# clovaai/assembled-cnn

Hardware: AMD Instinct MI355X
Metric: images/sec Assemble-ResNet-50 224^2 bf16 train (higher is better)
Workload: dtype bf16; 1 GPU; Assemble-ResNet-50 (BigLittle + SK + anti_alias sconv k=3 + resnet_d) bf16 train; per_gpu_batch=256, global_batch=256, image=224x224x3, num_classes=1001, parallelism=dp1

## Files before the change

### assembled_cnn_amd/csrc/sk_fused.hip

```cpp
#include "common.h"
#include "blur3s2.h"

namespace {

__device__ __forceinline__ u32x4 ldv(const bf16_t* p, size_t off) { return *reinterpret_cast<const u32x4*>(p + off); }
__device__ __forceinline__ float rbf(float x) { return bf2f(f2bf(x)); }

struct Coef8 {
  float sc[8], sh[8];
};
__device__ __forceinline__ void load_coef(const float* __restrict__ scale, const float* __restrict__ shift, int ch0, Coef8& k) {
  const f32x4 s0 = *reinterpret_cast<const f32x4*>(scale + ch0), s1 = *reinterpret_cast<const f32x4*>(scale + ch0 + 4);
  const f32x4 h0 = *reinterpret_cast<const f32x4*>(shift + ch0), h1 = *reinterpret_cast<const f32x4*>(shift + ch0 + 4);
#pragma unroll
  for (int e = 0; e < 4; ++e) {
    k.sc[e] = s0[e]; k.sc[e + 4] = s1[e];
    k.sh[e] = h0[e]; k.sh[e + 4] = h1[e];
  }
}
template <class K>
__device__ __forceinline__ void bnrelu8(const u32x4& vy, const K& k, float* f) {
  float y[8];
  unpack8(vy, y);
#pragma unroll
  for (int e = 0; e < 8; ++e) f[e] = rbf(fmaxf(y[e] * k.sc[e] + k.sh[e], 0.f));
}

__device__ __forceinline__ void gate8(const float* __restrict__ att, int n, int F, int c0, float* a0) {
#pragma unroll
  for (int e = 0; e < 8; ++e) {
    const float l0 = att[(size_t)n * 2 * F + c0 + e];
    const float l1 = att[(size_t)n * 2 * F + F + c0 + e];
    a0[e] = 1.0f / (1.0f + __expf(l1 - l0));
  }
}

template <int NT>
__device__ __forceinline__ void lane_sum8(float (*red)[9], const float* v, float* out, int vcb, int vcl, int nrl, bool leader) {
  if ((vcb & (vcb - 1)) == 0 && vcb <= 64) {
    float w[8];
#pragma unroll
    for (int e = 0; e < 8; ++e) w[e] = v[e];
    for (int off = vcb; off < 64; off <<= 1) {
#pragma unroll
      for (int e = 0; e < 8; ++e) w[e] += __shfl_xor(w[e], off, 64);
    }
    const int wave = threadIdx.x >> 6, lane = threadIdx.x & 63;
    __syncthreads();
    if (lane < vcb) {
#pragma unroll
      for (int e = 0; e < 8; ++e) red[wave * vcb + lane][e] = w[e];
    }
    __syncthreads();
    if (leader) {
#pragma unroll
      for (int e = 0; e < 8; ++e) {
        float t = 0.f;
#pragma unroll
        for (int r = 0; r < NT / 64; ++r) t += red[r * vcb + vcl][e];
        out[e] = t;
      }
    }
    return;
  }
  __syncthreads();
#pragma unroll
  for (int e = 0; e < 8; ++e) red[threadIdx.x][e] = v[e];
  __syncthreads();
  if (leader) {
#pragma unroll
    for (int e = 0; e < 8; ++e) {
      float t = 0.f;
      for (int r = 0; r < nrl; ++r) t += red[r * vcb + vcl][e];
      out[e] = t;
    }
  }
}

struct CoefLds {
  const float* sc;
  const float* sh;
};
template <class K>
__device__ __forceinline__ void bnrelu8m(const u32x4& vy, const K& k, float* f, float* m, float* my) {
  float y[8];
  unpack8(vy, y);
#pragma unroll
  for (int e = 0; e < 8; ++e) {
    const float t = y[e] * k.sc[e] + k.sh[e];
    f[e] = rbf(fmaxf(t, 0.f));
    m[e] = t > 0.f ? 1.f : 0.f;
    my[e] = t > 0.f ? y[e] : 0.f;
  }
}

template <int NT, bool ST>
__global__ __launch_bounds__(NT, NT == 256 ? 4 : 1) void sk_gap_bn_kernel(const bf16_t* __restrict__ y, const float* __restrict__ scale,
                                                       const float* __restrict__ shift, bf16_t* __restrict__ s, int HW,
                                                       int F, int vcb, const float* __restrict__ mean,
                                                       const float* __restrict__ invstd, float* __restrict__ stats) {
  __shared__ float red[NT][9];
  const int vcols = F >> 3;
  const int vcl = threadIdx.x % vcb, rl = threadIdx.x / vcb, nrl = NT / vcb;
  const int vc = blockIdx.x * vcb + vcl;
  const int n = blockIdx.y;
  float acc[8], c0[8], x0[8], c1[8], x1[8];
#pragma unroll
  for (int e = 0; e < 8; ++e) acc[e] = c0[e] = x0[e] = c1[e] = x1[e] = 0.f;
  if (vc < vcols && rl < nrl) {
    Coef8 k0, k1;
    load_coef(scale, shift, vc * 8, k0);
    load_coef(scale, shift, F + vc * 8, k1);
    auto consume = [&](const u32x4& v, const u32x4& w) {
      if (ST) {
        float f[8], m[8], my[8];
        bnrelu8m(v, k0, f, m, my);
#pragma unroll
        for (int e = 0; e < 8; ++e) { acc[e] += f[e]; c0[e] += m[e]; x0[e] += my[e]; }
        bnrelu8m(w, k1, f, m, my);
#pragma unroll
        for (int e = 0; e < 8; ++e) { acc[e] += f[e]; c1[e] += m[e]; x1[e] += my[e]; }
      } else {
        float f0[8], f1[8];
        bnrelu8(v, k0, f0);
        bnrelu8(w, k1, f1);
#pragma unroll
        for (int e = 0; e < 8; ++e) acc[e] += f0[e] + f1[e];
      }
    };
    constexpr int U = ST ? 2 : 4;
    const bf16_t* base = y + (size_t)n * HW * 2 * F + vc * 8;
    int r = rl;
    for (; r + (U - 1) * nrl < HW; r += U * nrl) {
      u32x4 v[U], w[U];
#pragma unroll
      for (int u = 0; u < U; ++u) {
        const size_t off = (size_t)(r + u * nrl) * 2 * F;
        v[u] = ldv(base, off);
        w[u] = ldv(base, off + F);
      }
#pragma unroll
      for (int u = 0; u < U; ++u) consume(v[u], w[u]);
    }
    for (; r < HW; r += nrl) {
      const size_t off = (size_t)r * 2 * F;
      consume(ldv(base, off), ldv(base, off + F));
    }
  }
  const bool leader = rl == 0 && vc < vcols;
  float o[8];
  lane_sum8<NT>(red, acc, o, vcb, vcl, nrl, leader);
  if (leader) {
    const float inv = 1.0f / (float)HW;
#pragma unroll
    for (int e = 0; e < 8; ++e) o[e] *= inv;
    *reinterpret_cast<u32x4*>(s + (size_t)n * F + vc * 8) = pack8(o);
  }
  if (ST) {
    float* st = stats + (size_t)n * 4 * F;
    const float* src[4] = {c0, c1, x0, x1};
#pragma unroll
    for (int q = 0; q < 4; ++q) {
      lane_sum8<NT>(red, src[q], o, vcb, vcl, nrl, leader);
      if (leader) {
        float* dst = st + (q >> 1) * 2 * F + (q & 1) * F + vc * 8;
        *reinterpret_cast<f32x4*>(dst) = f32x4{o[0], o[1], o[2], o[3]};
        *reinterpret_cast<f32x4*>(dst + 4) = f32x4{o[4], o[5], o[6], o[7]};
      }
    }
  }
}

struct PoolGeom {
  int W, Hh, Wh;
  FastDiv fd_w;
  float a0, a1, a2;
};

__device__ __forceinline__ u32x4 dv_from_pooled(const bf16_t* __restrict__ gimg, const PoolGeom& pg, int F, int r) {
  const int h = (int)fd_div((unsigned)r, pg.fd_w), w = r - h * pg.W;
  const int i = h >> 1, j = w >> 1;
  const bool u = h & 1, v = w & 1;
  const bool hv = i + 1 < pg.Hh, wv = j + 1 < pg.Wh;
  u32x4 g[2][2];
#pragma unroll
  for (int a = 0; a < 2; ++a)
#pragma unroll
    for (int b = 0; b < 2; ++b) {
      const bool ok = (a == 0 || (u && hv)) && (b == 0 || (v && wv));
      g[a][b] = ldv(gimg, ((size_t)(i + (ok ? a : 0)) * pg.Wh + j + (ok ? b : 0)) * F);
    }
  float acc[8];
  blur3s2_bwd_pixel([&](int a, int b, float* t) { unpack8(g[a][b], t); }, u, v, hv, wv, i == 0, j == 0, pg.a0, pg.a1, pg.a2,
                    acc);
  return pack8(acc);
}

__global__ __launch_bounds__(256) void sk_select_blur_fwd_kernel(const bf16_t* __restrict__ y, const float* __restrict__ scale,
                                                                 const float* __restrict__ shift,
                                                                 const float* __restrict__ att, bf16_t* __restrict__ out,
                                                                 int H, int W, int F, int fvb, int rpb, int bh,
                                                                 FastDiv fd_wo, float b0, float b1, float b2) {
  extern __shared__ u32x4 vband[];
  const int fv = F >> 3;
  const int vcl = threadIdx.x % fvb, rr = threadIdx.x / fvb;
  const int vc = blockIdx.z * fvb + vcl;
  const int n = blockIdx.y;
  const bool live = rr < rpb && vc < fv;
  const int Ho = H >> 1, Wo = W >> 1;
  const int ho0 = blockIdx.x * bh;
  const int nbh = min(bh, Ho - ho0);
  if (live) {
    Coef8 k0, k1;
    load_coef(scale, shift, vc * 8, k0);
    load_coef(scale, shift, F + vc * 8, k1);
    float a0[8];
    gate8(att, n, F, vc * 8, a0);
    const bf16_t* yn = y + (size_t)n * H * W * 2 * F + vc * 8;
    const int npix = (2 * nbh + 1) * W;
    const int first = (2 * ho0 - 1) * W;
    constexpr int U = 2;
    for (int p = rr; p < npix; p += U * rpb) {
      u32x4 y0[U], y1[U];
#pragma unroll
      for (int q = 0; q < U; ++q) {
        const int pq = p + q * rpb;
        int gp = first + (pq < npix ? pq : p);
        if (gp < 0) gp += 2 * W;
        y0[q] = ldv(yn, (size_t)gp * 2 * F);
        y1[q] = ldv(yn, (size_t)gp * 2 * F + F);
      }
#pragma unroll
      for (int q = 0; q < U; ++q) {
        const int pq = p + q * rpb;
        if (pq >= npix) break;
        float f0[8], f1[8], o[8];
        bnrelu8(y0[q], k0, f0);
        bnrelu8(y1[q], k1, f1);
#pragma unroll
        for (int e = 0; e < 8; ++e) o[e] = a0[e] * f0[e] + (1.0f - a0[e]) * f1[e];
        vband[pq * fvb + vcl] = pack8(o);
      }
    }
  }
  __syncthreads();
  if (live) {
    const float bw[3] = {b0, b1, b2};
    const int nout = nbh * Wo;
    for (int q = rr; q < nout; q += rpb) {
      const int oh = (int)fd_div((unsigned)q, fd_wo), ow = q - oh * Wo;
      float acc[8];
#pragma unroll
      for (int e = 0; e < 8; ++e) acc[e] = 0.f;
#pragma unroll
      for (int r = 0; r < 3; ++r) {
        const int lr = 2 * oh + r;
#pragma unroll
        for (int t = 0; t < 3; ++t) {
          int iw = 2 * ow + t - 1;
          if (iw < 0) iw = 1;
          float f[8];
          unpack8(vband[(lr * W + iw) * fvb + vcl], f);
          const float wgt = bw[r] * bw[t];
#pragma unroll
          for (int e = 0; e < 8; ++e) acc[e] += f[e] * wgt;
        }
      }
      *reinterpret_cast<u32x4*>(out + (((size_t)n * Ho + ho0 + oh) * Wo + ow) * F + vc * 8) = pack8(acc);
    }
  }
}

__global__ __launch_bounds__(256) void sk_select_bn_fwd_kernel(const bf16_t* __restrict__ y, const float* __restrict__ scale,
                                                               const float* __restrict__ shift,
                                                               const float* __restrict__ att, bf16_t* __restrict__ v,
                                                               int HW, int F, int rpb, int rows_per_chunk) {
  const int fv = F >> 3;
  const int vc = threadIdx.x % fv, rr = threadIdx.x / fv;
  if (rr >= rpb) return;
  const int n = blockIdx.y;
  Coef8 k0, k1;
  load_coef(scale, shift, vc * 8, k0);
  load_coef(scale, shift, F + vc * 8, k1);
  float a0[8];
  gate8(att, n, F, vc * 8, a0);
  const int r_begin = blockIdx.x * rows_per_chunk;
  const int r_end = min(HW, r_begin + rows_per_chunk);
  constexpr int U = 2;
  for (int r = r_begin + rr; r < r_end; r += U * rpb) {
    u32x4 y0[U], y1[U];
#pragma unroll
    for (int q = 0; q < U; ++q) {
      const int rq = r + q * rpb;
      const size_t m = (size_t)n * HW + (rq < r_end ? rq : r);
      y0[q] = ldv(y, m * 2 * F + vc * 8);
      y1[q] = ldv(y, m * 2 * F + F + vc * 8);
    }
#pragma unroll
    for (int q = 0; q < U; ++q) {
      const int rq = r + q * rpb;
      if (rq >= r_end) break;
      float f0[8], f1[8], o[8];
      bnrelu8(y0[q], k0, f0);
      bnrelu8(y1[q], k1, f1);
#pragma unroll
      for (int e = 0; e < 8; ++e) o[e] = a0[e] * f0[e] + (1.0f - a0[e]) * f1[e];
      *reinterpret_cast<u32x4*>(v + ((size_t)n * HW + rq) * F + vc * 8) = pack8(o);
    }
  }
}

template <int NT, bool ST, bool PG>
__global__ __launch_bounds__(NT, NT == 256 ? 4 : 1) void sk_bn_bwd_att_kernel(const bf16_t* __restrict__ y, const float* __restrict__ scale,
                                                           const float* __restrict__ shift, const bf16_t* __restrict__ dv,
                                                           const float* __restrict__ att, bf16_t* __restrict__ datt,
                                                           int HW, int F, int vcb, const float* __restrict__ mean,
                                                           const float* __restrict__ invstd, float* __restrict__ stats,
                                                           PoolGeom pg) {
  __shared__ float red[NT][9];
  __shared__ float cfl[PG ? 4 * 256 : 1];
  const int vcols = F >> 3;
  const int vcl = threadIdx.x % vcb, rl = threadIdx.x / vcb, nrl = NT / vcb;
  const int vc = blockIdx.x * vcb + vcl;
  const int n = blockIdx.y;
  float acc[8], g0[8], x0[8], g1[8], x1[8];
#pragma unroll
  for (int e = 0; e < 8; ++e) acc[e] = g0[e] = x0[e] = g1[e] = x1[e] = 0.f;
  if (PG) {
    if (rl == 0 && vc < vcols) {
#pragma unroll
      for (int e = 0; e < 8; ++e) {
        cfl[vcl * 8 + e] = scale[vc * 8 + e];
        cfl[256 + vcl * 8 + e] = shift[vc * 8 + e];
        cfl[512 + vcl * 8 + e] = scale[F + vc * 8 + e];
        cfl[768 + vcl * 8 + e] = shift[F + vc * 8 + e];
      }
    }
    __syncthreads();
  }
  if (vc < vcols && rl < nrl) {
    Coef8 r0, r1;
    if (!PG) {
      load_coef(scale, shift, vc * 8, r0);
      load_coef(scale, shift, F + vc * 8, r1);
    }
    const CoefLds l0 = {cfl + vcl * 8, cfl + 256 + vcl * 8}, l1 = {cfl + 512 + vcl * 8, cfl + 768 + vcl * 8};
    auto add_pixel = [&](const auto& k0, const auto& k1, const u32x4& v0, const u32x4& v1, const u32x4& vg) {
      float g[8];
      unpack8(vg, g);
      if (ST) {
        float f[8], m[8], my[8];
        bnrelu8m(v0, k0, f, m, my);
#pragma unroll
        for (int e = 0; e < 8; ++e) { acc[e] += f[e] * g[e]; g0[e] += m[e] * g[e]; x0[e] += my[e] * g[e]; }
        bnrelu8m(v1, k1, f, m, my);
#pragma unroll
        for (int e = 0; e < 8; ++e) { acc[e] -= f[e] * g[e]; g1[e] += m[e] * g[e]; x1[e] += my[e] * g[e]; }
      } else {
        float f0[8], f1[8];
        bnrelu8(v0, k0, f0);
        bnrelu8(v1, k1, f1);
#pragma unroll
        for (int e = 0; e < 8; ++e) acc[e] += (f0[e] - f1[e]) * g[e];
      }
    };
    auto consume = [&](const u32x4& v0, const u32x4& v1, const u32x4& vg) {
      if (PG) {
        __asm__ volatile("" ::: "memory");
        add_pixel(l0, l1, v0, v1, vg);
      } else {
        add_pixel(r0, r1, v0, v1, vg);
      }
    };
    const bf16_t* gimg = PG ? dv + (size_t)n * pg.Hh * pg.Wh * F + vc * 8 : nullptr;
    auto load_dv = [&](int rq) { return PG ? dv_from_pooled(gimg, pg, F, rq) : ldv(dv, ((size_t)n * HW + rq) * F + vc * 8); };
    constexpr int U = ST ? 1 : 2;
    int r = rl;
    for (; r + (U - 1) * nrl < HW; r += U * nrl) {
      u32x4 v0[U], v1[U], vg[U];
#pragma unroll
      for (int u = 0; u < U; ++u) {
        const size_t m = (size_t)n * HW + r + u * nrl;
        v0[u] = ldv(y, m * 2 * F + vc * 8);
        v1[u] = ldv(y, m * 2 * F + F + vc * 8);
        vg[u] = load_dv(r + u * nrl);
      }
#pragma unroll
      for (int u = 0; u < U; ++u) consume(v0[u], v1[u], vg[u]);
    }
    for (; r < HW; r += nrl) {
      const size_t m = (size_t)n * HW + r;
      consume(ldv(y, m * 2 * F + vc * 8), ldv(y, m * 2 * F + F + vc * 8), load_dv(r));
    }
  }
  const bool leader = rl == 0 && vc < vcols;
  float o[8];
  lane_sum8<NT>(red, acc, o, vcb, vcl, nrl, leader);
  if (leader) {
    float a0[8], d0[8], d1[8];
    gate8(att, n, F, vc * 8, a0);
#pragma unroll
    for (int e = 0; e < 8; ++e) {
      d0[e] = a0[e] * (1.0f - a0[e]) * o[e];
      d1[e] = -d0[e];
    }
    *reinterpret_cast<u32x4*>(datt + (size_t)n * 2 * F + vc * 8) = pack8(d0);
    *reinterpret_cast<u32x4*>(datt + (size_t)n * 2 * F + F + vc * 8) = pack8(d1);
  }
  if (ST) {
    float* st = stats + (size_t)n * 4 * F;
    const float* src[4] = {g0, g1, x0, x1};
#pragma unroll
    for (int q = 0; q < 4; ++q) {
      lane_sum8<NT>(red, src[q], o, vcb, vcl, nrl, leader);
      if (leader) {
        float* dst = st + (q >> 1) * 2 * F + (q & 1) * F + vc * 8;
        *reinterpret_cast<f32x4*>(dst) = f32x4{o[0], o[1], o[2], o[3]};
        *reinterpret_cast<f32x4*>(dst + 4) = f32x4{o[4], o[5], o[6], o[7]};
      }
    }
  }
}

struct SkBnGeom {
  int HW, F, vcols, rpb, rows_per_chunk, chunks;
};

__device__ __forceinline__ void sk_thread_setup(const SkBnGeom& g, int n, int vc, const float* __restrict__ att,
                                                const bf16_t* __restrict__ ds, float* ab, float* u) {
  const int fv = g.F >> 3;
  const int b = vc >= fv ? 1 : 0;
  const int c0 = (vc - b * fv) * 8;
  float a0[8], q[8];
  gate8(att, n, g.F, c0, a0);
  unpack8(ldv(ds, (size_t)n * g.F + c0), q);
  const float inv = 1.0f / (float)g.HW;
#pragma unroll
  for (int e = 0; e < 8; ++e) {
    ab[e] = b ? (1.0f - a0[e]) : a0[e];
    u[e] = q[e] * inv;
  }
}

__global__ __launch_bounds__(256) void sk_bn_bwd_reduce_kernel(const bf16_t* __restrict__ dv, const float* __restrict__ att,
                                                               const bf16_t* __restrict__ ds, const bf16_t* __restrict__ y,
                                                               const float* __restrict__ scale,
                                                               const float* __restrict__ shift,
                                                               const float* __restrict__ mean,
                                                               const float* __restrict__ invstd, SkBnGeom g,
                                                               float* __restrict__ partial) {
  __shared__ float red[4096];
  const int tid = threadIdx.x;
  const int vc = tid % g.vcols;
  const int rr = tid / g.vcols;
  const bool active = rr < g.rpb;
  const int n = blockIdx.y;
  const int C2 = 2 * g.F;
  const int fv = g.F >> 3;
  const int cv = vc >= fv ? vc - fv : vc;
  float acc[2][8];
#pragma unroll
  for (int e = 0; e < 8; ++e) acc[0][e] = acc[1][e] = 0.f;
  if (active) {
    Coef8 k;
    load_coef(scale, shift, vc * 8, k);
    float mu[8], is[8], ab[8], u[8];
#pragma unroll
    for (int e = 0; e < 8; ++e) {
      mu[e] = mean[vc * 8 + e];
      is[e] = invstd[vc * 8 + e];
    }
    sk_thread_setup(g, n, vc, att, ds, ab, u);
    const int r_begin = blockIdx.x * g.rows_per_chunk;
    const int r_end = min(g.HW, r_begin + g.rows_per_chunk);
    constexpr int U = 2;
    for (int r = r_begin + rr; r < r_end; r += U * g.rpb) {
      u32x4 vy[U], vg[U];
#pragma unroll
      for (int q = 0; q < U; ++q) {
        const int rq = r + q * g.rpb;
        const size_t m = (size_t)n * g.HW + (rq < r_end ? rq : r);
        vy[q] = *reinterpret_cast<const u32x4*>(y + m * C2 + vc * 8);
        vg[q] = ldv(dv, m * g.F + cv * 8);
      }
#pragma unroll
      for (int q = 0; q < U; ++q) {
        if (r + q * g.rpb >= r_end) break;
        float fy[8], fg[8];
        unpack8(vy[q], fy);
        unpack8(vg[q], fg);
#pragma unroll
        for (int e = 0; e < 8; ++e) {
          const float dz = (fy[e] * k.sc[e] + k.sh[e] > 0.f) ? (ab[e] * fg[e] + u[e]) : 0.f;
          acc[0][e] += dz;
          acc[1][e] += dz * ((fy[e] - mu[e]) * is[e]);
        }
      }
    }
  }
  const size_t prow = (size_t)n * g.chunks + blockIdx.x;
  row_lanes_sum<2>(red, acc, active, vc, rr, g.rpb, g.vcols * 8,
                   [&](int which, int col, float v) { partial[(prow * 2 + which) * C2 + col] = v; });
}

__global__ __launch_bounds__(1024) void sk_bn_bwd_finalize_kernel(const float* __restrict__ gst, const float* __restrict__ mst,
                                                                  const float* __restrict__ att, const bf16_t* __restrict__ ds,
                                                                  int N, int HW, int F, const float* __restrict__ gamma,
                                                                  const float* __restrict__ mean,
                                                                  const float* __restrict__ invstd, float* dgamma,
                                                                  float* dbeta, float* coefA, float* coefB, float* coefC) {
  __shared__ double red[2][64][16];
  const int cx = threadIdx.x & 15, ry = threadIdx.x >> 4;
  const int C2 = 2 * F;
  const int ch = blockIdx.x * 16 + cx;
  double s0 = 0.0, s1 = 0.0;
  if (ch < C2) {
    const int b = ch >= F ? 1 : 0, c = ch - b * F;
    const float inv = 1.0f / (float)HW;
    for (int n = ry; n < N; n += 64) {
      const float l0 = att[(size_t)n * C2 + c], l1 = att[(size_t)n * C2 + F + c];
      const float a0 = 1.0f / (1.0f + __expf(l1 - l0));
      const float ab = b ? (1.0f - a0) : a0;
      const float u = bf2f(ds[(size_t)n * F + c]) * inv;
      const float* gs = gst + (size_t)n * 2 * C2;
      const float* ms = mst + (size_t)n * 2 * C2;
      const double g0 = gs[ch], m0 = ms[ch];
      const double w = (double)ab * g0 + (double)u * m0;
      s0 += w;
      s1 += (double)ab * (double)gs[C2 + ch] + (double)u * (double)ms[C2 + ch];
      s1 -= (double)mean[ch] * w;
    }
    s1 *= (double)invstd[ch];
  }
  fl_stage(red, ry, cx, s0, s1);
  if (ry == 0 && ch < C2) {
    double db, dg;
    fl_sum2(red, cx, db, dg);
    dbeta[ch] = (float)db;
    dgamma[ch] = (float)dg;
    bn_bwd_coefs(gamma[ch], invstd[ch], mean[ch], db, dg, (double)N * (double)HW, coefA[ch], coefB[ch], coefC[ch]);
  }
}

template <bool PG>
__global__ __launch_bounds__(256) void sk_bn_bwd_apply_kernel(const bf16_t* __restrict__ dv, const float* __restrict__ att,
                                                              const bf16_t* __restrict__ ds, const bf16_t* __restrict__ y,
                                                              const float* __restrict__ scale,
                                                              const float* __restrict__ shift, const float* __restrict__ cA,
                                                              const float* __restrict__ cB, const float* __restrict__ cC,
                                                              bf16_t* __restrict__ dy, SkBnGeom g, PoolGeom pg) {
  const int tid = threadIdx.x;
  const int vc = tid % g.vcols;
  const int rr = tid / g.vcols;
  if (rr >= g.rpb) return;
  const int n = blockIdx.y;
  const int C2 = 2 * g.F;
  const int fv = g.F >> 3;
  const int cv = vc >= fv ? vc - fv : vc;
  Coef8 k;
  load_coef(scale, shift, vc * 8, k);
  float ab[8], u[8], kA[8], kB[8], kC[8];
#pragma unroll
  for (int e = 0; e < 8; ++e) {
    kA[e] = cA[vc * 8 + e];
    kB[e] = cB[vc * 8 + e];
    kC[e] = cC[vc * 8 + e];
  }
  sk_thread_setup(g, n, vc, att, ds, ab, u);
  const bf16_t* gimg = PG ? dv + (size_t)n * pg.Hh * pg.Wh * g.F + cv * 8 : nullptr;
  const int r_begin = blockIdx.x * g.rows_per_chunk;
  const int r_end = min(g.HW, r_begin + g.rows_per_chunk);
  constexpr int U = 2;
  for (int r = r_begin + rr; r < r_end; r += U * g.rpb) {
    u32x4 vy[U], vg[U];
#pragma unroll
    for (int q = 0; q < U; ++q) {
      const int rq = r + q * g.rpb;
      const int rc = rq < r_end ? rq : r;
      const size_t m = (size_t)n * g.HW + rc;
      vy[q] = __builtin_nontemporal_load(reinterpret_cast<const u32x4*>(y + m * C2 + vc * 8));
      vg[q] = PG ? dv_from_pooled(gimg, pg, g.F, rc) : ldv(dv, m * g.F + cv * 8);
    }
#pragma unroll
    for (int q = 0; q < U; ++q) {
      const int rq = r + q * g.rpb;
      if (rq >= r_end) break;
      float fy[8], fg[8], o[8];
      unpack8(vy[q], fy);
      unpack8(vg[q], fg);
#pragma unroll
      for (int e = 0; e < 8; ++e) {
        const float dz = (fy[e] * k.sc[e] + k.sh[e] > 0.f) ? (ab[e] * fg[e] + u[e]) : 0.f;
        o[e] = kA[e] * dz + kB[e] * fy[e] + kC[e];
      }
      const size_t m = (size_t)n * g.HW + rq;
      __builtin_nontemporal_store(pack8(o), reinterpret_cast<u32x4*>(dy + m * C2 + vc * 8));
    }
  }
}

int image_pass_vcb(int N, int F) {
  const int vcols = F / 8;
  int groups = cdiv(1024, N > 0 ? N : 1);
  if (groups < 1) groups = 1;
  int vcb = 32;
  while (vcb > 8 && cdiv(vcols, vcb) < groups) vcb >>= 1;
  return vcols < vcb ? vcols : vcb;
}

SkBnGeom make_geom(int N, int HW, int F) {
  SkBnGeom g;
  g.HW = HW;
  g.F = F;
  g.vcols = 2 * F / 8;
  g.rpb = 256 / g.vcols;
  int chunks = 1024 / N;
  if (chunks < 1) chunks = 1;
  int rows = cdiv(HW, chunks);
  rows = cdiv(rows, g.rpb) * g.rpb;
  if (rows < g.rpb * 4) rows = g.rpb * 4;
  g.rows_per_chunk = rows;
  g.chunks = cdiv(HW, rows);
  return g;
}

}

#define SKF_OK(name)                                                                                        \
  ASM_REQUIRE(N > 0 && HW > 0 && F > 0 && F % 8 == 0 && 2 * F / 8 <= 256, name ": bad shape (N=%d HW=%d F=%d)", N, HW, F); \
  ASM_REQUIRE((size_t)N * HW * (2 * F / 8) < 0x7fffffffull, name ": tensor too large for 32-bit indexing")

static int sk_gap_bn_impl(const void* y, const float* scale, const float* shift, void* s, int N, int HW, int F,
                          const float* mean, const float* invstd, float* stats, void* stream) {
  SKF_OK("sk_gap_bn");
  ASM_REQUIRE(y && scale && shift && s, "sk_gap_bn: null pointer");
  const int vcb = image_pass_vcb(N, F);
  const dim3 grid(cdiv(F / 8, vcb), N);
  hipStream_t st = (hipStream_t)stream;
#define LAUNCH_GAP(NT, ST)                                                                                       \
  ASM_LAUNCH((sk_gap_bn_kernel<NT, ST>), grid, dim3(NT), 0, st, (const bf16_t*)y, scale, shift, (bf16_t*)s, HW, F, \
                     vcb, mean, invstd, stats)
  if (stats) { if (HW >= 512) LAUNCH_GAP(1024, true); else LAUNCH_GAP(256, true); }
  else { if (HW >= 512) LAUNCH_GAP(1024, false); else LAUNCH_GAP(256, false); }
#undef LAUNCH_GAP
  ASM_CHECK_LAUNCH("sk_gap_bn");
  return ASM_OK;
}

extern "C" int asm_sk_gap_bn(const void* y, const float* scale, const float* shift, void* s, int N, int HW, int F,
                             void* stream) {
  return sk_gap_bn_impl(y, scale, shift, s, N, HW, F, nullptr, nullptr, nullptr, stream);
}

extern "C" int asm_sk_gap_bn_stats(const void* y, const float* scale, const float* shift, const float* mean,
                                   const float* invstd, void* s, float* mask_stats, int N, int HW, int F, void* stream) {
  ASM_REQUIRE(mean && invstd && mask_stats, "sk_gap_bn_stats: null pointer");
  return sk_gap_bn_impl(y, scale, shift, s, N, HW, F, mean, invstd, mask_stats, stream);
}

extern "C" int asm_sk_select_bn_fwd(const void* y, const float* scale, const float* shift, const float* att, void* v,
                                    int N, int HW, int F, void* stream) {
  SKF_OK("sk_select_bn_fwd");
  ASM_REQUIRE(y && scale && shift && att && v, "sk_select_bn_fwd: null pointer");
  const int fv = F / 8, rpb = 256 / fv;
  int chunks = 2048 / N;
  if (chunks < 1) chunks = 1;
  int rows = cdiv(HW, chunks);
  rows = cdiv(rows, rpb) * rpb;
  if (rows < rpb * 4) rows = rpb * 4;
  ASM_LAUNCH(sk_select_bn_fwd_kernel, dim3(cdiv(HW, rows), N), dim3(256), 0, (hipStream_t)stream,
                     (const bf16_t*)y, scale, shift, att, (bf16_t*)v, HW, F, rpb, rows);
  ASM_CHECK_LAUNCH("sk_select_bn_fwd");
  return ASM_OK;
}

#define SKB_OK(name)                                                                                                    \
  ASM_REQUIRE(k == 3 && stride == 2, name ": blur filter size %d / stride %d not supported (3 / 2 only)", k, stride);    \
  ASM_REQUIRE(H > 0 && W > 0 && H % 2 == 0 && W % 2 == 0, name ": H=%d W=%d must be even", H, W);                        \
  const int HW = H * W;                                                                                                 \
  SKF_OK(name)

static PoolGeom make_pool_geom(int H, int W) {
  const BlurCoef cf = blur_coef(3);
  return PoolGeom{W, H / 2, W / 2, make_fastdiv((unsigned)W), cf.a[0], cf.a[1], cf.a[2]};
}

constexpr int SKB_BAND = 2;
constexpr int SKB_MAX_W = 512;
constexpr size_t SKB_LDS = 40 * 1024;

extern "C" int asm_sk_select_bn_blur_fwd(const void* y, const float* scale, const float* shift, const float* att, void* out,
                                         int N, int H, int W, int F, int k, int stride, void* stream) {
  SKB_OK("sk_select_bn_blur_fwd");
  ASM_REQUIRE(y && scale && shift && att && out, "sk_select_bn_blur_fwd: null pointer");
  ASM_REQUIRE(W <= SKB_MAX_W, "sk_select_bn_blur_fwd: W=%d above %d", W, SKB_MAX_W);
  const int fv = F / 8, rows = 2 * SKB_BAND + 1;
  int fvb = fv < 32 ? fv : 32;
  while (fvb > 1 && (size_t)rows * W * fvb * 16 > SKB_LDS) fvb = cdiv(fvb, 2);
  const int groups = cdiv(fv, fvb);
  ASM_REQUIRE(groups <= 65535, "sk_select_bn_blur_fwd: too many column groups");
  const BlurCoef cf = blur_coef(3);
  const unsigned lds = (unsigned)((size_t)rows * W * fvb * 16);
  ASM_LAUNCH(sk_select_blur_fwd_kernel, dim3(cdiv(H / 2, SKB_BAND), N, groups), dim3(256), lds, (hipStream_t)stream,
                     (const bf16_t*)y, scale, shift, att, (bf16_t*)out, H, W, F, fvb, 256 / fvb, SKB_BAND,
                     make_fastdiv((unsigned)(W / 2)), cf.a[0], cf.a[1], cf.a[2]);
  ASM_CHECK_LAUNCH("sk_select_bn_blur_fwd");
  return ASM_OK;
}

static int sk_att_impl(const void* y, const float* scale, const float* shift, const void* dv, const float* att, void* datt,
                       int N, int HW, int F, const float* mean, const float* invstd, float* stats, void* stream,
                       const PoolGeom* pooled = nullptr) {
  SKF_OK("sk_select_bn_bwd_att");
  ASM_REQUIRE(y && scale && shift && dv && att && datt, "sk_select_bn_bwd_att: null pointer");
  const int vcb = image_pass_vcb(N, F);
  const dim3 grid(cdiv(F / 8, vcb), N);
  hipStream_t st = (hipStream_t)stream;
  const PoolGeom pg = pooled ? *pooled : PoolGeom{};
#define LAUNCH_ATT(NT, ST, PG)                                                                                          \
  ASM_LAUNCH((sk_bn_bwd_att_kernel<NT, ST, PG>), grid, dim3(NT), 0, st, (const bf16_t*)y, scale, shift, (const bf16_t*)dv, \
                     att, (bf16_t*)datt, HW, F, vcb, mean, invstd, stats, pg)
  if (pooled) { if (HW >= 512) LAUNCH_ATT(1024, true, true); else LAUNCH_ATT(256, true, true); }
  else if (stats) { if (HW >= 512) LAUNCH_ATT(1024, true, false); else LAUNCH_ATT(256, true, false); }
  else { if (HW >= 512) LAUNCH_ATT(1024, false, false); else LAUNCH_ATT(256, false, false); }
#undef LAUNCH_ATT
  ASM_CHECK_LAUNCH("sk_select_bn_bwd_att");
  return ASM_OK;
}

extern "C" int asm_sk_select_bn_bwd_att(const void* y, const float* scale, const float* shift, const void* dv,
                                        const float* att, void* datt, int N, int HW, int F, void* stream) {
  return sk_att_impl(y, scale, shift, dv, att, datt, N, HW, F, nullptr, nullptr, nullptr, stream);
}

extern "C" int asm_sk_select_bn_bwd_att_stats(const void* y, const float* scale, const float* shift, const float* mean,
                                              const float* invstd, const void* dv, const float* att, void* datt,
                                              float* grad_stats, int N, int HW, int F, void* stream) {
  ASM_REQUIRE(mean && invstd && grad_stats, "sk_select_bn_bwd_att_stats: null pointer");
  return sk_att_impl(y, scale, shift, dv, att, datt, N, HW, F, mean, invstd, grad_stats, stream);
}

extern "C" int asm_sk_select_bn_bwd_att_stats_blur(const void* y, const float* scale, const float* shift, const float* mean,
                                                   const float* invstd, const void* dpool, const float* att, void* datt,
                                                   float* grad_stats, int N, int H, int W, int F, int k, int stride,
                                                   void* stream) {
  SKB_OK("sk_select_bn_bwd_att_stats_blur");
  ASM_REQUIRE(mean && invstd && grad_stats, "sk_select_bn_bwd_att_stats_blur: null pointer");
  const PoolGeom pg = make_pool_geom(H, W);
  return sk_att_impl(y, scale, shift, dpool, att, datt, N, HW, F, mean, invstd, grad_stats, stream, &pg);
}

extern "C" int asm_sk_bn_bwd_finalize(const float* grad_stats, const float* mask_stats, const float* att, const void* ds,
                                      int N, int HW, int F, const float* gamma, const float* mean, const float* invstd,
                                      float* dgamma, float* dbeta, float* coefA, float* coefB, float* coefC, void* stream) {
  SKF_OK("sk_bn_bwd_finalize");
  ASM_REQUIRE(grad_stats && mask_stats && att && ds && gamma && mean && invstd && dgamma && dbeta && coefA && coefB && coefC,
              "sk_bn_bwd_finalize: null pointer");
  ASM_LAUNCH(sk_bn_bwd_finalize_kernel, dim3(cdiv(2 * F, 16)), dim3(1024), 0, (hipStream_t)stream, grad_stats,
                     mask_stats, att, (const bf16_t*)ds, N, HW, F, gamma, mean, invstd, dgamma, dbeta, coefA, coefB, coefC);
  ASM_CHECK_LAUNCH("sk_bn_bwd_finalize");
  return ASM_OK;
}

extern "C" int asm_sk_bn_bwd_blocks(int N, int HW, int F) {
  if (N <= 0 || HW <= 0 || F <= 0 || F % 8 || 2 * F / 8 > 256) return ASM_EINVAL;
  return N * make_geom(N, HW, F).chunks;
}

extern "C" int asm_sk_bn_bwd_reduce(const void* dv, const float* att, const void* ds, const void* y, const float* scale,
                                    const float* shift, const float* mean, const float* invstd, int N, int HW, int F,
                                    float* partial, void* stream) {
  SKF_OK("sk_bn_bwd_reduce");
  ASM_REQUIRE(dv && att && ds && y && scale && shift && mean && invstd && partial, "sk_bn_bwd_reduce: null pointer");
  const SkBnGeom g = make_geom(N, HW, F);
  ASM_LAUNCH(sk_bn_bwd_reduce_kernel, dim3(g.chunks, N), dim3(256), 0, (hipStream_t)stream, (const bf16_t*)dv, att,
                     (const bf16_t*)ds, (const bf16_t*)y, scale, shift, mean, invstd, g, partial);
  ASM_CHECK_LAUNCH("sk_bn_bwd_reduce");
  return ASM_OK;
}

extern "C" int asm_sk_bn_bwd_apply(const void* dv, const float* att, const void* ds, const void* y, const float* scale,
                                   const float* shift, const float* coefA, const float* coefB, const float* coefC,
                                   void* dy, int N, int HW, int F, void* stream) {
  SKF_OK("sk_bn_bwd_apply");
  ASM_REQUIRE(dv && att && ds && y && scale && shift && coefA && coefB && coefC && dy, "sk_bn_bwd_apply: null pointer");
  const SkBnGeom g = make_geom(N, HW, F);
  ASM_LAUNCH(sk_bn_bwd_apply_kernel<false>, dim3(g.chunks, N), dim3(256), 0, (hipStream_t)stream,
                     (const bf16_t*)dv, att, (const bf16_t*)ds, (const bf16_t*)y, scale, shift, coefA, coefB, coefC,
                     (bf16_t*)dy, g, PoolGeom{});
  ASM_CHECK_LAUNCH("sk_bn_bwd_apply");
  return ASM_OK;
}

extern "C" int asm_sk_bn_bwd_apply_blur(const void* dpool, const float* att, const void* ds, const void* y,
                                        const float* scale, const float* shift, const float* coefA, const float* coefB,
                                        const float* coefC, void* dy, int N, int H, int W, int F, int k, int stride,
                                        void* stream) {
  SKB_OK("sk_bn_bwd_apply_blur");
  ASM_REQUIRE(dpool && att && ds && y && scale && shift && coefA && coefB && coefC && dy, "sk_bn_bwd_apply_blur: null pointer");
  const SkBnGeom g = make_geom(N, HW, F);
  ASM_LAUNCH(sk_bn_bwd_apply_kernel<true>, dim3(g.chunks, N), dim3(256), 0, (hipStream_t)stream,
                     (const bf16_t*)dpool, att, (const bf16_t*)ds, (const bf16_t*)y, scale, shift, coefA, coefB, coefC,
                     (bf16_t*)dy, g, make_pool_geom(H, W));
  ASM_CHECK_LAUNCH("sk_bn_bwd_apply_blur");
  return ASM_OK;
}
```

### assembled_cnn_amd/lib.py

```python
from __future__ import annotations

import ctypes as C
import os

HERE = os.path.dirname(os.path.abspath(__file__))
LIB_PATH = os.environ.get('ASM_HIP_LIB') or os.path.join(HERE, 'libasm_hip.so')

ASM_OK, ASM_EINVAL, ASM_ENOTSUP, ASM_EHIP = 0, -1, -2, -3
ABI_VERSION = 11


class AsmError(RuntimeError):
  pass


class ImageDesc(C.Structure):
  _fields_ = [('src_offset', C.c_int64), ('Hs', C.c_int32), ('Ws', C.c_int32),
              ('crop_y', C.c_int32), ('crop_x', C.c_int32), ('crop_h', C.c_int32), ('crop_w', C.c_int32),
              ('resize_h', C.c_int32), ('resize_w', C.c_int32), ('out_y', C.c_int32), ('out_x', C.c_int32),
              ('flip', C.c_int32), ('reserved', C.c_int32)]


assert C.sizeof(ImageDesc) == 56

class AugmentOp(C.Structure):
  _fields_ = [('op', C.c_int32), ('a', C.c_int32), ('b', C.c_int32), ('reserved', C.c_int32), ('f', C.c_float * 6)]


class AugmentDesc(C.Structure):
  _fields_ = [('slot', AugmentOp * 2)]


assert C.sizeof(AugmentOp) == 40 and C.sizeof(AugmentDesc) == 80


class JpegDesc(C.Structure):
  _fields_ = [(n, C.c_int64) for n in ('scan_offset', 'scan_bytes', 'coef_offset', 'plane_offset', 'dst_offset')] + [
      (n, C.c_int32) for n in ('width', 'height', 'ncomp', 'hs', 'vs', 'mcus_x', 'mcus_y', 'restart_interval',
                               'first_interval', 'n_intervals')] + [
      ('qsel', C.c_uint8 * 4), ('dcsel', C.c_uint8 * 4), ('acsel', C.c_uint8 * 4), ('reserved', C.c_int32)]


class JpegHuff(C.Structure):
  _fields_ = [('bits', C.c_uint8 * 16), ('vals', C.c_uint8 * 256)]


class JpegTables(C.Structure):
  _fields_ = [('quant', (C.c_uint16 * 64) * 4), ('dc', JpegHuff * 2), ('ac', JpegHuff * 2)]


class JpegInterval(C.Structure):
  _fields_ = [('image', C.c_int32), ('first_mcu', C.c_int32), ('n_mcus', C.c_int32), ('rst', C.c_int32),
              ('byte_begin', C.c_int64), ('byte_end', C.c_int64)]


class JpegScan(C.Structure):
  _fields_ = [('image', C.c_int32), ('ncomp', C.c_int32), ('comp', C.c_uint8 * 4), ('ss', C.c_uint8), ('se', C.c_uint8),
              ('ah', C.c_uint8), ('al', C.c_uint8), ('huff', C.c_int32 * 3), ('restart_interval', C.c_int32),
              ('first_interval', C.c_int32), ('n_intervals', C.c_int32), ('byte_begin', C.c_int64), ('byte_end', C.c_int64)]


assert (C.sizeof(JpegDesc), C.sizeof(JpegHuff), C.sizeof(JpegTables), C.sizeof(JpegInterval)) == (96, 272, 1600, 32)
assert C.sizeof(JpegScan) == 56
JPEG_EBADCODE, JPEG_EOVERRUN, JPEG_ERESTART, JPEG_EDESC = 1, 2, 4, 8


class SpanDesc(C.Structure):
  _fields_ = [('offset', C.c_int64), ('length', C.c_int64), ('expect_masked', C.c_uint32), ('flags', C.c_uint32)]


assert C.sizeof(SpanDesc) == 24
SPAN_EDESC, SPAN_EMISMATCH = 1, 2


class ExampleRow(C.Structure):
  _fields_ = [('cls', C.c_int32), ('label', C.c_int32), ('enc_offset', C.c_int64), ('name_offset', C.c_int64),
              ('logit_offset', C.c_int64), ('enc_length', C.c_int32), ('name_length', C.c_int32),
              ('logit_count', C.c_int32), ('n_boxes', C.c_int32)]


assert C.sizeof(ExampleRow) == 48
EXAMPLE_WINDOW = 1024
EXAMPLE_PSPAN, EXAMPLE_PMALFORMED, EXAMPLE_PSCHEMA, EXAMPLE_PFORM = 1, 2, 4, 8
EXAMPLE_LSKIP, EXAMPLE_LRANGE = 1, 2


class JpegHead(C.Structure):
  _fields_ = [(n, C.c_int32) for n in ('cls', 'width', 'height', 'ncomp', 'hs', 'vs', 'restart_interval', 'n_intervals')] + [
      (n, C.c_int64) for n in ('scan_begin', 'scan_bytes', 'n_segments')] + [
      ('qsel', C.c_uint8 * 4), ('dcsel', C.c_uint8 * 4), ('acsel', C.c_uint8 * 4), ('reserved', C.c_int32)]


class JpegPlace(C.Structure):
  _fields_ = [('span', C.c_int32), ('first_interval', C.c_int32), ('first_segment', C.c_int32), ('reserved', C.c_int32),
              ('coef_offset', C.c_int64), ('dst_offset', C.c_int64)]


assert (C.sizeof(JpegHead), C.sizeof(JpegPlace)) == (72, 32)
JPEG_PNOTJPEG, JPEG_PHEADER, JPEG_PKIND, JPEG_PNOEOI, JPEG_PSPAN, JPEG_PLIMIT = 1, 2, 4, 8, 16, 32


class ConvDesc(C.Structure):
  _fields_ = [('N', C.c_int32), ('H', C.c_int32), ('W', C.c_int32), ('C', C.c_int32),
              ('K', C.c_int32), ('R', C.c_int32), ('S', C.c_int32),
              ('stride', C.c_int32), ('pad', C.c_int32),
              ('Ho', C.c_int32), ('Wo', C.c_int32),
              ('x_img_pitch', C.c_int64), ('x_row_pitch', C.c_int32), ('x_pix_pitch', C.c_int32),
              ('ldy', C.c_int32), ('out_f32', C.c_int32)]


class ModelCfg(C.Structure):
  _fields_ = [(n, C.c_int32) for n in (
      'resnet_size', 'resnet_version', 'num_classes', 'use_se_block', 'use_sk_block', 'use_resnet_d',
      'anti_alias_filter_size', 'anti_alias_type', 'bl_alpha', 'bl_beta', 'zero_gamma', 'no_downsample', 'pool_type',
      'embedding_size', 'dtype', 'mixup_type')] + [(n, C.c_float) for n in (
          'bn_momentum', 'bn_eps', 'loss_scale', 'label_smoothing', 'kd_temp', 'weight_decay', 'momentum')]


class PlanEntry(C.Structure):
  _fields_ = [(n, C.c_int32) for n in ('kind', 'N', 'H', 'W', 'C', 'K', 'R', 'S', 'stride', 'Ho', 'Wo', 'flags',
                                       'trainable', 'reserved')] + [
      ('param_offset', C.c_int64), ('param_elems', C.c_int64), ('name', C.c_char * 112)]


class PlanSummary(C.Structure):
  _fields_ = [('n_entries', C.c_int32), ('trainable_tensors', C.c_int32), ('trainable_elems', C.c_int64),
              ('forward_macs_per_image', C.c_int64), ('wgrad_workspace_bytes', C.c_int64)]


class Tuning(C.Structure):
  _fields_ = [(n, C.c_int32) for n in (
      'igemm_mode', 'igemm_tile', 'igemm_pfa', 'dgrad_parity', 'wgrad_halo', 'wgrad_big', 'wgrad_splits', 'bn_rows', 'igemm3',
      'gemm1', 'wgrad_ring', 'igemm8', 'dense_small')]


TUNING_ENV = {'ASM_IGEMM_MODE': 'igemm_mode', 'ASM_IGEMM_TILE': 'igemm_tile', 'ASM_IGEMM_PFA': 'igemm_pfa',
              'ASM_DGRAD_PARITY': 'dgrad_parity', 'ASM_WGRAD_HALO': 'wgrad_halo', 'ASM_WGRAD_BIG': 'wgrad_big',
              'ASM_WGRAD_SPLITS': 'wgrad_splits', 'ASM_BN_ROWS': 'bn_rows', 'ASM_IGEMM3': 'igemm3', 'ASM_GEMM1': 'gemm1',
              'ASM_WGRAD_RING': 'wgrad_ring', 'ASM_IGEMM8': 'igemm8', 'ASM_DENSE_SMALL': 'dense_small'}


def apply_env_tuning(lib) -> 'Tuning':
  t = Tuning()
  lib.asm_tuning_defaults(C.byref(t))
  for env, field in TUNING_ENV.items():
    v = os.environ.get(env)
    if v not in (None, ''):
      setattr(t, field, int(v))
  check_code = lib.asm_set_tuning(C.byref(t))
  if check_code != ASM_OK:
    raise ValueError('asm_set_tuning rejected the ASM_* overrides: %s' % (lib.asm_last_error() or b'').decode())
  return t


ASM_F32, ASM_BF16, ASM_F16 = 0, 1, 2
ASM_DGRAD_MASKED, ASM_DGRAD_POOLED, ASM_DGRAD_BNRED = 1, 2, 4
CONV_DGRAD_S2 = 5
CONV_DENSE = 6
ASM_AA_SCONV, ASM_AA_PROJ = 1, 2
POOL_TYPES = {'gap': 0, 'gem': 1, 'flatten': 2}
(PLAN_CONV, PLAN_BN, PLAN_DENSE, PLAN_MAXPOOL, PLAN_AVGPOOL, PLAN_BLURPOOL, PLAN_GAP, PLAN_GEM, PLAN_FLATTEN, PLAN_SK_GAP,
 PLAN_SK_SELECT, PLAN_SE_SCALE, PLAN_ADD) = range(13)

_P, _I, _F, _Z = C.c_void_p, C.c_int, C.c_float, C.c_size_t
_D = C.POINTER(ConvDesc)

SIGNATURES = {
    'asm_last_error': (C.c_char_p, []),
    'asm_abi_version': (_I, []),
    'asm_launch_count': (C.c_ulonglong, []),
    'asm_stream_join': (_I, [_P, _P]),
    'asm_memcpy_async': (_I, [_P, _P, _Z, _P]),
    'asm_allreduce_bucket': (_I, [_P, _Z, _I, _P, _P, _P]),
    'asm_tape_begin': (_I, []),
    'asm_tape_mark': (_I, []),
    'asm_tape_end': (_I, []),
    'asm_tape_info': (_I, [_I, C.POINTER(C.c_int64 * 6)]),
    'asm_tape_replay': (_I, [_I, _I]),
    'asm_tape_free': (_I, [_I]),
    'asm_tuning_defaults': (None, [C.POINTER(Tuning)]),
    'asm_set_tuning': (_I, [C.POINTER(Tuning)]),
    'asm_get_tuning': (None, [C.POINTER(Tuning)]),
    'asm_conv2d_fprop': (_I, [_D, _P, _P, _P, _P, _P]),
    'asm_conv2d_stats_blocks': (_I, [_D]),
    'asm_conv2d_dgrad': (_I, [_D, _P, _P, _P, _P, _P]),
    'asm_conv2d_dgrad_masked': (_I, [_D, _P, _P, _P, _P, _P, _P]),
    'asm_conv2d_dgrad_pooled': (_I, [_D, _P, _P, _P, _P, _P, _I, _I, _I, _I, _I, _I, _P, _P]),
    'asm_conv2d_dgrad_bnred_blocks': (_I, [_D]),
    'asm_conv2d_dgrad_bnred': (_I, [_D, _P, _P, _P, _P, _P, _P, _P, _P, _P]),
    'asm_conv2d_dgrad_kernel': (_I, [_D, _I]),
    'asm_conv2d_wgrad_workspace_bytes': (_Z, [_D]),
    'asm_conv2d_wgrad': (_I, [_D, _P, _P, _P, _P, _Z, _P]),
    'asm_filter_transpose': (_I, [_P, _P, _I, _I, _I, _I, _I, _P]),
    'asm_filter_transpose_batched': (_I, [_P, _P, _P, _I, C.c_longlong, _P]),
    'asm_filter_transpose_tiled': (_I, [_P, _P, _P, _I, _I, _P]),
    'asm_stem_pack_filter': (_I, [_P, _P, _I, _I, _P]),
    'asm_stem_unpack_grad': (_I, [_P, _P, _I, _I, _P]),
    'asm_stem_pad_input': (_I, [_P, _I, _P, _I, _I, _I, _P]),
    'asm_bn_stats_blocks': (_I, [_I, _I]),
    'asm_bn_stats': (_I, [_P, _I, _I, _P, _P]),
    'asm_bn_partials_compact': (_I, [_P, _I, _I, _P, _I, _P]),
    'asm_bn_finalize': (_I, [_P, _I, _I, _I, _P, _P, _F, _F, _P, _P, _P, _P, _P, _P, _P]),
    'asm_bn_infer_coeffs': (_I, [_I, _P, _P, _P, _P, _F, _P, _P, _P]),
    'asm_bn_apply': (_I, [_P, _P, _I, _I, _P, _P, _P, _I, _I, _I, _I, _P, _P]),
    'asm_bn_bwd_reduce': (_I, [_P, _P, _P, _I, _I, _I, _P, _P, _P, _P]),
    'asm_bn_bwd_finalize': (_I, [_P, _I, _I, _I, _P, _P, _P, _P, _P, _P, _P, _P, _P]),
    'asm_bn_bwd_finalize_raw': (_I, [_P, _I, _I, _I, _P, _P, _P, _P, _P, _P, _P, _P, _P]),
    'asm_bn_bwd_apply': (_I, [_P, _P, _P, _I, _I, _I, _P, _P, _P, _P, _P, _P]),
    'asm_bn_bwd_apply_blocksum': (_I, [_P, _P, _P, _I, _I, _I, _I, _P, _P, _P, _P, _P, _P]),
    'asm_maxpool3x3s2_fwd': (_I, [_P, _P, _P, _I, _I, _I, _I, _P]),
    'asm_maxpool3x3s2_bwd': (_I, [_P, _P, _P, _I, _I, _I, _I, _P]),
    'asm_avgpool_fwd': (_I, [_P, _P, _I, _I, _I, _I, _I, _I, _I, _I, _I, _I, _P]),
    'asm_avgpool_bwd': (_I, [_P, _P, _I, _I, _I, _I, _I, _I, _I, _I, _I, _I, _P, _P]),
    'asm_upsample2x_bwd': (_I, [_P, _P, _I, _I, _I, _I, _P]),
    'asm_upsample2x_bwd_masked': (_I, [_P, _P, _P, _I, _I, _I, _I, _P]),
    'asm_blurpool_fwd': (_I, [_P, _P, _I, _I, _I, _I, _I, _I, _P]),
    'asm_blurpool_bwd': (_I, [_P, _P, _I, _I, _I, _I, _I, _I, _P]),
    'asm_gap_fwd': (_I, [_P, _P, _I, _I, _I, _P]),
    'asm_gap_bwd': (_I, [_P, _P, _I, _I, _I, _P]),
    'asm_sk_gap': (_I, [_P, _P, _I, _I, _I, _P]),
    'asm_sk_select_fwd': (_I, [_P, _P, _P, _I, _I, _I, _P]),
    'asm_sk_select_bwd_att': (_I, [_P, _P, _P, _P, _I, _I, _I, _P]),
    'asm_sk_select_bwd_f': (_I, [_P, _P, _P, _P, _I, _I, _I, _P]),
    'asm_sk_gap_bn': (_I, [_P, _P, _P, _P, _I, _I, _I, _P]),
    'asm_sk_select_bn_fwd': (_I, [_P, _P, _P, _P, _P, _I, _I, _I, _P]),
    'asm_sk_select_bn_blur_fwd': (_I, [_P, _P, _P, _P, _P, _I, _I, _I, _I, _I, _I, _P]),
    'asm_sk_select_bn_bwd_att': (_I, [_P, _P, _P, _P, _P, _P, _I, _I, _I, _P]),
    'asm_sk_bn_bwd_blocks': (_I, [_I, _I, _I]),
    'asm_sk_bn_bwd_reduce': (_I, [_P, _P, _P, _P, _P, _P, _P, _P, _I, _I, _I, _P, _P]),
    'asm_sk_bn_bwd_apply': (_I, [_P, _P, _P, _P, _P, _P, _P, _P, _P, _P, _I, _I, _I, _P]),
    'asm_sk_bn_bwd_apply_blur': (_I, [_P, _P, _P, _P, _P, _P, _P, _P, _P, _P, _I, _I, _I, _I, _I, _I, _P]),
    'asm_sk_gap_bn_stats': (_I, [_P, _P, _P, _P, _P, _P, _P, _I, _I, _I, _P]),
    'asm_sk_select_bn_bwd_att_stats': (_I, [_P, _P, _P, _P, _P, _P, _P, _P, _P, _I, _I, _I, _P]),
    'asm_sk_select_bn_bwd_att_stats_blur': (_I, [_P, _P, _P, _P, _P, _P, _P, _P, _P, _I, _I, _I, _I, _I, _I, _P]),
    'asm_sk_bn_bwd_finalize': (_I, [_P, _P, _P, _P, _I, _I, _I, _P, _P, _P, _P, _P, _P, _P, _P, _P]),
    'asm_se_scale_fwd': (_I, [_P, _P, _P, _I, _I, _I, _P]),
    'asm_se_scale_bwd_e': (_I, [_P, _P, _P, _P, _I, _I, _I, _P]),
    'asm_se_scale_bwd_x': (_I, [_P, _P, _P, _P, _I, _I, _I, _P]),
    'asm_relu_fwd': (_I, [_P, _P, _Z, _P]),
    'asm_relu_bwd': (_I, [_P, _P, _P, _Z, _P]),
    'asm_add_bf16': (_I, [_P, _P, _P, _Z, _P]),
    'asm_mask_apply': (_I, [_P, _P, _P, _Z, _P]),
    'asm_bias_add_f32': (_I, [_P, _P, _I, _I, _I, _P]),
    'asm_bias_grad_bf16': (_I, [_P, _I, _I, _I, _P, _P]),
    'asm_cast_f32_to_bf16': (_I, [_P, _P, _Z, _P]),
    'asm_cast_bf16_to_f32': (_I, [_P, _P, _Z, _P]),
    'asm_softmax_ce': (_I, [_P, _I, _P, _P, _I, _I, _F, _F, _F, _P, _P, _I, _P]),
    'asm_onehot': (_I, [_P, _P, _I, _I, _P]),
    'asm_softmax_rows': (_I, [_P, _P, _I, _I, _F, _P]),
    'asm_mean_f32': (_I, [_P, _I, _P, _P]),
    'asm_mixup_meansub': (_I, [_P, _I, _I, _I, _I, _I, _P, _P, _P, _P]),
    'asm_mixup_labels': (_I, [_P, _I, _I, _I, _P, _P, _P, _P]),
    'asm_sigmoid_ce': (_I, [_P, _I, _P, _I, _I, _F, _P, _P, _P, _I, _P]),
    'asm_gem_fwd': (_I, [_P, _P, _P, _I, _I, _I, _F, _P]),
    'asm_gem_bwd': (_I, [_P, _P, _P, _P, _I, _I, _I, _F, _P]),
    'asm_dropblock_mask': (_I, [_P, _F, _I, _I, _I, _I, _P, _P, _P]),
    'asm_dropblock_mask_dev': (_I, [_P, _P, _I, _I, _I, _I, _P, _P, _P]),
    'asm_dropblock_apply': (_I, [_P, _P, _P, _P, _I, _P, _I, _I, _P]),
    'asm_eval_rows': (_I, [_P, _I, _P, _I, _I, _P, _P, _P, _P, _P]),
    'asm_eval_accumulate': (_I, [_P, _P, _P, _I, _P, _P]),
    'asm_eval_groups': (_I, [_P, _I, _P, _P, _I, _I, _I, _P, _P, _P]),
    'asm_embed_sqnorm': (_I, [_P, _I, _I, _I, _P, _P]),
    'asm_retrieval_topk_workspace_bytes': (_Z, [_I, _I, _I]),
    'asm_retrieval_topk': (_I, [_P, _I, _P, _I, _P, _P, _I, _I, _I, _I, _I, _I, _P, _P, _P, _Z, _P]),
    'asm_topk_merge': (_I, [_P, _P, _I, _I, _I, _P, _P, _P]),
    'asm_retrieval_topk_wide_workspace_bytes': (_Z, [_I, _I, _I]),
    'asm_retrieval_topk_wide': (_I, [_P, _I, _P, _I, _P, _P, _I, _I, _I, _I, _I, _I, _P, _P, _P, _Z, _P]),
    'asm_topk_merge_wide': (_I, [_P, _P, _I, _I, _I, _P, _P, _P]),
    'asm_recall_accumulate': (_I, [_P, _I, _I, _P, _P, _I, _I, _P, _I, _P, _P]),
    'asm_sgd_momentum': (_I, [_P, _P, _P, _P, _Z, _F, _F, _F, _F, _P]),
    'asm_conv2d_fprop_bn': (_I, [_P, _P, _P, _P, _P, _P, _P, _I, _P]),
    'asm_bn_apply2': (_I, [_P, _P, _P, _I, _I, _P, _P, _P, _P, _I, _P, _P]),
    'asm_bn_bwd_reduce2': (_I, [_P, _P, _P, _P, _I, _I, _P, _P, _P, _P, _P, _P, _P]),
    'asm_bn_bwd_apply2': (_I, [_P, _P, _P, _P, _I, _I, _P, _P, _P, _P]),
    'asm_bn_small_max_rows': (_I, []),
    'asm_bn_small_fwd': (_I, [_P, _P, _I, _I, _P, _P, _F, _F, _P, _P, _P, _P, _I, _P, _P]),
    'asm_bn_small_bwd': (_I, [_P, _P, _P, _I, _I, _P, _P, _P, _P, _P, _P, _P]),
    'asm_dense_small': (_I, [_P, _I, _P, _I, _I, _I, _I, _P, _I, _I, _P, _P]),
    'asm_dense_small_wgrad': (_I, [_P, _I, _P, _I, _I, _I, _I, _P, _I, _P]),
    'asm_resize_crop_flip': (_I, [_P, C.c_int64, _P, _I, _I, _I, _I, _P, _P]),
    'asm_preprocess_window': (_I, [_P, C.c_int64, _P, _I, _I, _I, _I, _I, _P, _P, _P]),
    'asm_autoaugment_workspace_bytes': (_I, [_I, _I, _I, C.POINTER(C.c_int64)]),
    'asm_autoaugment': (_I, [_P, _P, _I, _I, _I, _I, _P, _P, C.c_int64, _P]),
    'asm_jpeg_decode_workspace_bytes': (_I, [C.c_int64, C.POINTER(C.c_int64)]),
    'asm_jpeg_decode': (_I, [_P, C.c_int64, _P, _P, _P, _I, _I, C.c_int64, _I, _I, _P, C.c_int64, _P, _P, C.c_int64, _I, _P]),
    'asm_jpeg_decode_parallel_workspace_bytes': (_I, [C.c_int64, C.c_int64, C.POINTER(C.c_int64)]),
    'asm_jpeg_decode_parallel': (_I, [_P, C.c_int64, _P, _P, _P, _P, _I, _I, C.c_int64, _I, C.c_int64, _I, _I, _P, C.c_int64, _P,
                                      _P, _P, C.c_int64, _I, _P]),
    'asm_jpeg_decode_progressive': (_I, [_P, C.c_int64, _P, _P, _P, _P, _P, _I, _I, _I, _I, C.c_int64, _I, _I, _P, C.c_int64, _P,
                                         _P, C.c_int64, _I, _P]),
    'asm_crc32c_spans': (_I, [_P, C.c_int64, _P, _I, _P, _P, _P]),
    'asm_example_parse': (_I, [_P, C.c_int64, _P, _I, _P, _P]),
    'asm_example_label_rows': (_I, [_P, C.c_int64, _P, _I, _I, _P, _I, _P, _P]),
    'asm_jpeg_parse': (_I, [_P, C.c_int64, _P, _I, _I, _P, _P, _P]),
    'asm_jpeg_parse_fill': (_I, [_P, C.c_int64, _P, _I, _P, _P, _P, _I, _I, C.c_int64, _I, _P, _P, _P, _P, _P, _P]),
    'asm_model_plan': (_I, [C.POINTER(ModelCfg), _I, _I, _I, C.POINTER(PlanEntry), _I, C.POINTER(PlanSummary)]),
}

DEBUG_SIGNATURES = {
    'asm_conv2d_fprop_naive': (_I, [_D, _P, _P, _P, _P]),
    'asm_conv2d_dgrad_naive': (_I, [_D, _P, _P, _P, _P]),
    'asm_conv2d_wgrad_naive': (_I, [_D, _P, _P, _P, _P]),
    'asm_debug_tr_probe': (_I, [_P, _P]),
    'asm_conv2d_wgrad_plan': (_I, [_D, C.POINTER(C.c_int32 * 6)]),
    'asm_debug_last_conv_kernel': (_I, []),
    'asm_debug_retrieval_topk_wide_counted': (_I, [_P, _I, _P, _I, _P, _P, _I, _I, _I, _I, _I, _I, _P, _P, _P, _Z, _P, _P]),
    'asm_debug_retrieval_plan': (_I, [_I, _I, _I, _I, C.POINTER(C.c_int32 * 4)]),
}

_lib = None


def load(path: str = LIB_PATH) -> C.CDLL:
  global _lib
  if _lib is not None:
    return _lib
  if not os.path.exists(path):
    raise AsmError('%s not found -- build it with `python -m assembled_cnn_amd.build` '
                   '(there is no CPU fallback)' % path)
  import torch
  lib = C.CDLL(path)
  ver = getattr(lib, 'asm_abi_version', None)
  if ver is None:
    raise AsmError('%s does not export asm_abi_version: not a libasm_hip.so' % path)
  ver.restype, ver.argtypes = C.c_int, []
  if ver() != ABI_VERSION:
    raise AsmError('libasm_hip.so ABI version %d != %d (rebuild: python -m assembled_cnn_amd.build)' % (ver(), ABI_VERSION))
  for name, (res, args) in list(SIGNATURES.items()) + list(DEBUG_SIGNATURES.items()):
    fn = getattr(lib, name, None)
    if fn is None:
      raise AsmError('libasm_hip.so does not export %s' % name)
    fn.restype = res
    fn.argtypes = args
  apply_env_tuning(lib)
  _lib = lib
  return lib


CALLS = [0]


def check(code: int, what: str = ''):
  CALLS[0] += 1
  if code != ASM_OK:
    msg = load().asm_last_error()
    msg = msg.decode() if msg else ''
    if code == ASM_EINVAL:
      raise ValueError('%s: %s' % (what, msg))
    if code == ASM_ENOTSUP:
      raise NotImplementedError('%s: %s' % (what, msg))
    raise AsmError('%s: HIP error: %s' % (what, msg))
```

### assembled_cnn_amd/ops.py

```python
from __future__ import annotations

import ctypes as C
import os
from typing import Optional, Tuple

import torch

from . import lib as _lib
from .lib import ConvDesc, check

_L = None
_IS_DOUBLE = False


def set_library(obj, is_double: bool = False):
  global _L, _IS_DOUBLE
  _L = obj
  _IS_DOUBLE = is_double


def L():
  global _L
  if _L is None:
    _L = _lib.load()
  return _L


def abi_calls() -> int:
  return _lib.CALLS[0]


_KNOBS = {}


def knob(name: str, default: str) -> str:
  v = _KNOBS.get(name)
  if v is None:
    v = _KNOBS[name] = os.environ.get(name, default)
  return v


def refresh_tuning():
  _KNOBS.clear()
  if _IS_DOUBLE:
    return None
  return _lib.apply_env_tuning(L())


def _ptr(t: Optional[torch.Tensor]) -> int:
  if t is None:
    return 0
  if not _IS_DOUBLE and not t.is_cuda:
    raise _lib.AsmError('assembled_cnn_amd ops need GPU tensors (no CPU fallback)')
  if not t.is_contiguous():
    raise ValueError('tensor must be contiguous')
  return t.data_ptr()


_RAW_STREAM = getattr(torch._C, '_cuda_getCurrentRawStream', None)
_CUR_DEVICE = getattr(torch._C, '_cuda_getDevice', None)


import threading

_TLS = threading.local()


def launch_on(stream: Optional["torch.cuda.Stream"]):
  _TLS.stream = None if stream is None else stream.cuda_stream


def _stream() -> int:
  if _IS_DOUBLE:
    return 0
  ov = getattr(_TLS, 'stream', None)
  if ov is not None:
    return ov
  if _RAW_STREAM is not None and _CUR_DEVICE is not None:
    return _RAW_STREAM(_CUR_DEVICE())
  return torch.cuda.current_stream().cuda_stream


def stream_join(dst: "torch.cuda.Stream", src: "torch.cuda.Stream"):
  if dst is src:
    return
  if _IS_DOUBLE:
    dst.wait_stream(src)
    return
  check(L().asm_stream_join(dst.cuda_stream, src.cuda_stream), 'stream_join')


def tape_begin() -> int:
  rc = L().asm_tape_begin()
  if rc <= 0:
    check(rc, 'tape_begin')
  return rc


def tape_mark() -> int:
  rc = L().asm_tape_mark()
  if rc <= 0:
    check(rc, 'tape_mark')
  return rc


def tape_end() -> int:
  rc = L().asm_tape_end()
  if rc <= 0:
    check(rc, 'tape_end')
  return rc


def tape_info(tape: int) -> dict:
  import ctypes
  info = (ctypes.c_int64 * 6)()
  check(L().asm_tape_info(tape, ctypes.byref(info)), 'tape_info')
  return dict(zip(('nodes', 'launches', 'joins', 'fills', 'segments', 'arg_bytes'), [int(v) for v in info]))


def tape_replay(tape: int, segment: int = -1):
  check(L().asm_tape_replay(tape, segment), 'tape_replay')


def tape_free(tape: int):
  check(L().asm_tape_free(tape), 'tape_free')


def empty(shape, dtype, like: torch.Tensor) -> torch.Tensor:
  return torch.empty(shape, dtype=dtype, device=like.device)


BF16 = torch.bfloat16
F32 = torch.float32


def out_size(in_size: int, k: int, stride: int) -> int:
  if stride == 1:
    return in_size
  return (in_size - 1) // stride + 1


def make_conv_desc(N, H, W, Cin, K, R, S, stride, pad=None, Ho=None, Wo=None, ldy=0, out_f32=False,
                   img_pitch=0, row_pitch=0, pix_pitch=0) -> ConvDesc:
  d = ConvDesc()
  d.N, d.H, d.W, d.C = N, H, W, Cin
  d.K, d.R, d.S = K, R, S
  d.stride = stride
  d.pad = (R - 1) // 2 if pad is None else pad
  d.Ho = out_size(H, R, stride) if Ho is None else Ho
  d.Wo = out_size(W, S, stride) if Wo is None else Wo
  d.x_img_pitch, d.x_row_pitch, d.x_pix_pitch = img_pitch, row_pitch, pix_pitch
  d.ldy = ldy
  d.out_f32 = 1 if out_f32 else 0
  return d


class ConvTimer(object):

  def __init__(self, only=None, classes=False):
    self.only = only
    self.classes = classes
    self.events = {}
    self.class_events = {}

  @staticmethod
  def key(kind, d):
    return (kind, d.N, d.H, d.W, d.C, d.K, d.R, d.S, d.stride)

  def start(self, kind, d):
    k = self.key(kind, d)
    if self.only is not None and k != self.only:
      return None
    e0 = torch.cuda.Event(enable_timing=True)
    e1 = torch.cuda.Event(enable_timing=True)
    e0.record()
    self.events.setdefault(k, []).append((e0, e1))
    return e1

  def start_class(self, cls, work):
    e0 = torch.cuda.Event(enable_timing=True)
    e1 = torch.cuda.Event(enable_timing=True)
    e0.record()
    self.class_events.setdefault(cls, []).append((e0, e1, float(work)))
    return e1

  def summary(self):
    return {k: (len(v), sum(a.elapsed_time(b) for a, b in v)) for k, v in self.events.items()}

  def class_summary(self):
    return {k: (len(v), sum(a.elapsed_time(b) for a, b, _ in v), sum(w for _, _, w in v))
            for k, v in self.class_events.items()}


_TIMER: Optional[ConvTimer] = None


def set_conv_timer(t: Optional[ConvTimer]):
  global _TIMER
  _TIMER = t


def timer_on() -> bool:
  return _TIMER is not None


def _bn_ev(nbytes):
  return _TIMER.start_class('bn', nbytes) if (_TIMER is not None and _TIMER.classes) else None


def conv_fprop(d: ConvDesc, x: torch.Tensor, w: torch.Tensor, want_stats: bool = False
               ) -> Tuple[torch.Tensor, Optional[torch.Tensor]]:
  ldy = d.ldy if d.ldy else d.K
  y = empty((d.N, d.Ho, d.Wo, ldy), F32 if d.out_f32 else BF16, x)
  stats = None
  if want_stats:
    stats = empty((L().asm_conv2d_stats_blocks(C.byref(d)), 2, d.K), F32, x)
  ev = _TIMER.start('fprop', d) if _TIMER is not None else None
  check(L().asm_conv2d_fprop(C.byref(d), _ptr(x), _ptr(w), _ptr(y), _ptr(stats), _stream()), 'conv2d_fprop')
  if ev is not None:
    ev.record()
  return y, stats


def conv_fprop_bn(d: ConvDesc, x: torch.Tensor, w: torch.Tensor, scale, shift, residual=None, relu=False):
  y = empty((d.N, d.Ho, d.Wo, d.K), BF16, x)
  ev = _TIMER.start('fprop', d) if _TIMER is not None else None
  check(L().asm_conv2d_fprop_bn(C.byref(d), _ptr(x), _ptr(w), _ptr(y), _ptr(scale), _ptr(shift), _ptr(residual),
                                1 if relu else 0, _stream()), 'conv2d_fprop_bn')
  if ev is not None:
    ev.record()
  return y


def dgrad_kernel(d: ConvDesc, variant: int = 0) -> int:
  query = getattr(L(), 'asm_conv2d_dgrad_kernel', None)
  if query is None:
    return _lib.ASM_ENOTSUP
  return query(C.byref(d), variant)


def dgrad_pool_ok(d: ConvDesc) -> bool:
  return (knob('ASM_POOL_FUSE', '1') != '0' and d.K % 32 == 0
          and dgrad_kernel(d, _lib.ASM_DGRAD_POOLED) >= 0)


def dgrad_s2_ok(d: ConvDesc) -> bool:
  return dgrad_kernel(d) == _lib.CONV_DGRAD_S2


def dgrad_bnred_ok(d: ConvDesc) -> bool:
  mode = knob('ASM_BN_RED', '1')
  if mode == '0' or (mode == '1x1' and d.R != 1):
    return False
  return dgrad_kernel(d, _lib.ASM_DGRAD_BNRED) >= 0


def conv_dgrad_bnred(d: ConvDesc, dy: torch.Tensor, wt: torch.Tensor, addend, addend_mask, bn_y: torch.Tensor, bn_mask):
  dx = empty((d.N, d.H, d.W, d.C), BF16, dy)
  blocks = L().asm_conv2d_dgrad_bnred_blocks(C.byref(d))
  part = empty((blocks, 2, d.C), F32, dy)
  ev = _TIMER.start('dgrad', d) if _TIMER is not None else None
  check(L().asm_conv2d_dgrad_bnred(C.byref(d), _ptr(dy), _ptr(wt), _ptr(addend), _ptr(addend_mask), _ptr(bn_y), _ptr(bn_mask),
                                   _ptr(part), _ptr(dx), _stream()), 'conv2d_dgrad_bnred')
  if ev is not None:
    ev.record()
  return dx, part


def conv_dgrad(d: ConvDesc, dy: torch.Tensor, wt: torch.Tensor, addend: Optional[torch.Tensor] = None,
               addend_mask: Optional[torch.Tensor] = None, pool=None) -> torch.Tensor:
  dx = empty((d.N, d.H, d.W, d.C), BF16, dy)
  ev = None
  if _TIMER is not None:
    ev = _TIMER.start('dgrad+add' if (addend is not None and getattr(_TIMER, 'split_addend', False)) else 'dgrad', d)
  if pool is not None:
    pdy, pk, pst, ppad, pcv = pool
    check(L().asm_conv2d_dgrad_pooled(C.byref(d), _ptr(dy), _ptr(wt), _ptr(addend), _ptr(addend_mask), _ptr(pdy), pk, pst,
                                      ppad, pdy.shape[1], pdy.shape[2], 1 if pcv else 0, _ptr(dx), _stream()),
          'conv2d_dgrad_pooled')
    if ev is not None:
      ev.record()
    return dx
  if addend_mask is not None:
    check(L().asm_conv2d_dgrad_masked(C.byref(d), _ptr(dy), _ptr(wt), _ptr(addend), _ptr(addend_mask), _ptr(dx),
                                      _stream()), 'conv2d_dgrad_masked')
  else:
    check(L().asm_conv2d_dgrad(C.byref(d), _ptr(dy), _ptr(wt), _ptr(addend), _ptr(dx), _stream()), 'conv2d_dgrad')
  if ev is not None:
    ev.record()
  return dx


_ws_cache = {}
_ws_retired = []


def _workspace(nbytes: int, like: torch.Tensor) -> Optional[torch.Tensor]:
  if nbytes == 0:
    return None
  key = (str(like.device), _stream())
  buf = _ws_cache.get(key)
  if buf is None or buf.numel() < nbytes:
    if buf is not None:
      _ws_retired.append(buf)
    buf = torch.empty((nbytes,), dtype=torch.uint8, device=like.device)
    _ws_cache[key] = buf
  return buf


def conv_wgrad(d: ConvDesc, x: torch.Tensor, dy: torch.Tensor, dw: torch.Tensor):
  need = L().asm_conv2d_wgrad_workspace_bytes(C.byref(d))
  ws = _workspace(need, x)
  ev = _TIMER.start('wgrad', d) if _TIMER is not None else None
  check(L().asm_conv2d_wgrad(C.byref(d), _ptr(x), _ptr(dy), _ptr(dw), _ptr(ws), need, _stream()), 'conv2d_wgrad')
  if ev is not None:
    ev.record()


def filter_transpose(w: torch.Tensor, wt: torch.Tensor, K, R, S, Cin, ldk=0):
  check(L().asm_filter_transpose(_ptr(w), _ptr(wt), K, R, S, Cin, ldk, _stream()), 'filter_transpose')


def filter_transpose_batched(w_arena, wt_arena, table, nlayers, total):
  check(L().asm_filter_transpose_batched(_ptr(w_arena), _ptr(wt_arena), _ptr(table), nlayers, total, _stream()),
        'filter_transpose_batched')


def filter_transpose_tiled(w_arena, wt_arena, table, nlayers, total_tiles):
  check(L().asm_filter_transpose_tiled(_ptr(w_arena), _ptr(wt_arena), _ptr(table), nlayers, total_tiles, _stream()),
        'filter_transpose_tiled')


def stem_pack_filter(w32: torch.Tensor, wp: torch.Tensor, K: int, ksize: int):
  check(L().asm_stem_pack_filter(_ptr(w32), _ptr(wp), K, ksize, _stream()), 'stem_pack_filter')


def stem_unpack_grad(dwp: torch.Tensor, dw: torch.Tensor, K: int, ksize: int):
  check(L().asm_stem_unpack_grad(_ptr(dwp), _ptr(dw), K, ksize, _stream()), 'stem_unpack_grad')


def stem_pad_input(x: torch.Tensor) -> torch.Tensor:
  N, H, W, c = x.shape
  if c != 3:
    raise ValueError('stem input must have 3 channels')
  if x.dtype not in (F32, BF16):
    raise ValueError('stem input dtype must be float32 or bfloat16')
  xp = empty((N, H + 6, W + 6, 4), BF16, x)
  check(L().asm_stem_pad_input(_ptr(x), 1 if x.dtype == F32 else 0, _ptr(xp), N, H, W, _stream()), 'stem_pad_input')
  return xp


def bn_stats(x2d: torch.Tensor, M: int, Cn: int) -> torch.Tensor:
  blocks = L().asm_bn_stats_blocks(M, Cn)
  if blocks <= 0:
    raise ValueError('bn_stats: bad shape')
  part = empty((blocks, 2, Cn), F32, x2d)
  check(L().asm_bn_stats(_ptr(x2d), M, Cn, _ptr(part), _stream()), 'bn_stats')
  return part


def _compact(part: torch.Tensor, Cn: int) -> torch.Tensor:
  blocks = part.shape[0]
  if blocks <= 1024:
    return part
  per = -(-blocks // 32)
  groups = -(-blocks // per)
  out = empty((groups, 2, Cn), F32, part)
  check(L().asm_bn_partials_compact(_ptr(part), blocks, Cn, _ptr(out), groups, _stream()), 'bn_partials_compact')
  return out


def bn_finalize(part, M, Cn, gamma, beta, eps, momentum, mm, mv):
  ev = _bn_ev(part.numel() * 4.0)
  part = _compact(part, Cn)
  co = empty((4, Cn), F32, part)
  check(L().asm_bn_finalize(_ptr(part), part.shape[0], M, Cn, _ptr(gamma), _ptr(beta), eps, momentum,
                            _ptr(mm), _ptr(mv), _ptr(co[0]), _ptr(co[1]), _ptr(co[2]), _ptr(co[3]),
                            _stream()), 'bn_finalize')
  if ev is not None:
    ev.record()
  return co[0], co[1], co[2], co[3]


def bn_infer_coeffs(Cn, gamma, beta, mm, mv, eps):
  co = empty((2, Cn), F32, gamma)
  check(L().asm_bn_infer_coeffs(Cn, _ptr(gamma), _ptr(beta), _ptr(mm), _ptr(mv), eps, _ptr(co[0]), _ptr(co[1]),
                                _stream()), 'bn_infer_coeffs')
  return co[0], co[1]


def bn_apply(x, M, Cn, scale, shift, residual=None, res_mode=0, relu=False, H=0, W=0, want_mask=False):
  y = torch.empty_like(x)
  mask = empty((M, Cn // 8), torch.uint8, x) if (want_mask and relu) else None
  ev = _bn_ev(M * Cn * (4.0 + (2.0 if res_mode == 1 else 0.5 if res_mode == 2 else 0.0) + (0.125 if mask is not None else 0.0)))
  check(L().asm_bn_apply(_ptr(x), _ptr(y), M, Cn, _ptr(scale), _ptr(shift), _ptr(residual), res_mode,
                         1 if relu else 0, H, W, _ptr(mask), _stream()), 'bn_apply')
  if ev is not None:
    ev.record()
  return (y, mask) if want_mask else y


def _bn_bwd_coeffs(part, M, Cn, gamma, mean, invstd, dgamma, dbeta, co, raw=False):
  part = _compact(part, Cn)
  fin, what = (L().asm_bn_bwd_finalize_raw, 'bn_bwd_finalize_raw') if raw else (L().asm_bn_bwd_finalize, 'bn_bwd_finalize')
  check(fin(_ptr(part), part.shape[0], M, Cn, _ptr(gamma), _ptr(mean), _ptr(invstd), _ptr(dgamma), _ptr(dbeta),
            _ptr(co[0]), _ptr(co[1]), _ptr(co[2]), _stream()), what)


def bn_blocksum_ok(yout, relu, want_dz, H, W) -> bool:
  return (knob('ASM_BL_SUM', '1') != '0' and relu and not want_dz and yout is not None and yout.dtype == torch.uint8
          and H > 0 and W > 0 and H % 2 == 0 and W % 2 == 0 and getattr(L(), 'asm_bn_bwd_apply_blocksum', None) is not None)


def bn_bwd(dy, x, yout, relu, M, Cn, gamma, mean, invstd, dgamma, dbeta, want_dz, raw_part=None, block_sum=None):
  rk = 0 if not relu else (2 if yout.dtype == torch.uint8 else 1)
  red_bytes = 0.0 if raw_part is not None else (4.0 + (0.125 if rk == 2 else 2.0 if rk == 1 else 0.0))
  ev = _bn_ev(M * Cn * (red_bytes + 4.0 + 2.0 + (2.0 if want_dz else 0.0) + (0.125 if rk == 2 else 2.0 if rk == 1 else 0.0)
                        + (0.5 if block_sum is not None else 0.0)))
  co = empty((3, Cn), F32, dy)
  part = raw_part
  if part is None:
    part = empty((L().asm_bn_stats_blocks(M, Cn), 2, Cn), F32, dy)
    check(L().asm_bn_bwd_reduce(_ptr(dy), _ptr(x), _ptr(yout if relu else None), rk, M, Cn,
                                _ptr(mean), _ptr(invstd), _ptr(part), _stream()), 'bn_bwd_reduce')
  _bn_bwd_coeffs(part, M, Cn, gamma, mean, invstd, dgamma, dbeta, co, raw=raw_part is not None)
  dx = torch.empty_like(x)
  if block_sum is not None:
    H, W = block_sum
    Nb = M // (H * W)
    bsum = empty((Nb, H // 2, W // 2, Cn), BF16, dy)
    check(L().asm_bn_bwd_apply_blocksum(_ptr(dy), _ptr(x), _ptr(yout), Nb, H, W, Cn, _ptr(co[0]), _ptr(co[1]), _ptr(co[2]),
                                        _ptr(dx), _ptr(bsum), _stream()), 'bn_bwd_apply_blocksum')
    if ev is not None:
      ev.record()
    return dx, None, bsum
  dz = torch.empty_like(x) if want_dz else None
  check(L().asm_bn_bwd_apply(_ptr(dy), _ptr(x), _ptr(yout if relu else None), rk, M, Cn,
                             _ptr(co[0]), _ptr(co[1]), _ptr(co[2]), _ptr(dx), _ptr(dz), _stream()), 'bn_bwd_apply')
  if ev is not None:
    ev.record()
  return dx, dz


def bn_apply_dual(xa, xb, M, Cn, scale_a, shift_a, scale_b, shift_b, relu, want_mask=False):
  y = torch.empty_like(xa)
  mask = empty((M, Cn // 8), torch.uint8, xa) if (want_mask and relu) else None
  ev = _bn_ev(M * Cn * (6.0 + (0.125 if mask is not None else 0.0)))
  check(L().asm_bn_apply2(_ptr(xa), _ptr(xb), _ptr(y), M, Cn, _ptr(scale_a), _ptr(shift_a), _ptr(scale_b), _ptr(shift_b),
                          1 if relu else 0, _ptr(mask), _stream()), 'bn_apply2')
  if ev is not None:
    ev.record()
  return (y, mask) if want_mask else y


def bn_bwd_dual(dy, xa, xb, mask, M, Cn, bn_a, bn_b):
  ev = _bn_ev(M * Cn * (2 * 6.0 + 4.0 + 2 * 0.125))
  blocks = L().asm_bn_stats_blocks(M, Cn)
  pa, pb = empty((blocks, 2, Cn), F32, dy), empty((blocks, 2, Cn), F32, dy)
  check(L().asm_bn_bwd_reduce2(_ptr(dy), _ptr(xa), _ptr(xb), _ptr(mask), M, Cn, _ptr(bn_a[1]), _ptr(bn_a[2]),
                               _ptr(bn_b[1]), _ptr(bn_b[2]), _ptr(pa), _ptr(pb), _stream()), 'bn_bwd_reduce2')
  co = empty((6, Cn), F32, dy)
  for i, (part, (gamma, mean, invstd, dgamma, dbeta)) in enumerate(((pa, bn_a), (pb, bn_b))):
    _bn_bwd_coeffs(part, M, Cn, gamma, mean, invstd, dgamma, dbeta, co[3 * i:3 * i + 3])
  dxa, dxb = torch.empty_like(xa), torch.empty_like(xb)
  check(L().asm_bn_bwd_apply2(_ptr(dy), _ptr(xa), _ptr(xb), _ptr(mask), M, Cn, _ptr(co), _ptr(dxa), _ptr(dxb), _stream()),
        'bn_bwd_apply2')
  if ev is not None:
    ev.record()
  return dxa, dxb


_SMALL_BN_ROWS = None


def bn_small_ok(M: int) -> bool:
  global _SMALL_BN_ROWS
  if _SMALL_BN_ROWS is None:
    _SMALL_BN_ROWS = int(L().asm_bn_small_max_rows())
  return M <= _SMALL_BN_ROWS


def bn_small_fwd(x, M, Cn, gamma, beta, eps, momentum, mm, mv, relu, want_mask):
  y = torch.empty_like(x)
  co = empty((2, Cn), F32, x)
  mask = empty((M, Cn // 8), torch.uint8, x) if (want_mask and relu) else None
  check(L().asm_bn_small_fwd(_ptr(x), _ptr(y), M, Cn, _ptr(gamma), _ptr(beta), eps, momentum, _ptr(mm), _ptr(mv),
                             _ptr(co[0]), _ptr(co[1]), 1 if relu else 0, _ptr(mask), _stream()), 'bn_small_fwd')
  return y, mask, co[0], co[1]


def bn_small_bwd(dy, x, mask, M, Cn, gamma, mean, invstd, dgamma, dbeta):
  dx = torch.empty_like(x)
  check(L().asm_bn_small_bwd(_ptr(dy), _ptr(x), _ptr(mask), M, Cn, _ptr(gamma), _ptr(mean), _ptr(invstd),
                             _ptr(dgamma), _ptr(dbeta), _ptr(dx), _stream()), 'bn_small_bwd')
  return dx


def maxpool3x3s2_fwd(x):
  N, H, W, Cn = x.shape
  Ho, Wo = (H + 1) // 2, (W + 1) // 2
  y = empty((N, Ho, Wo, Cn), BF16, x)
  am = empty((N, Ho, Wo, Cn), torch.uint8, x)
  check(L().asm_maxpool3x3s2_fwd(_ptr(x), _ptr(y), _ptr(am), N, H, W, Cn, _stream()), 'maxpool_fwd')
  return y, am


def maxpool3x3s2_bwd(dy, am, in_shape):
  N, H, W, Cn = in_shape
  dx = empty(in_shape, BF16, dy)
  check(L().asm_maxpool3x3s2_bwd(_ptr(dy), _ptr(am), _ptr(dx), N, H, W, Cn, _stream()), 'maxpool_bwd')
  return dx


def avgpool_fwd(x, k, stride, pad, Ho, Wo, count_valid):
  N, H, W, Cn = x.shape
  y = empty((N, Ho, Wo, Cn), BF16, x)
  check(L().asm_avgpool_fwd(_ptr(x), _ptr(y), N, H, W, Cn, k, stride, pad, Ho, Wo, 1 if count_valid else 0,
                            _stream()), 'avgpool_fwd')
  return y


def avgpool_bwd(dy, in_shape, k, stride, pad, count_valid, addend=None):
  N, H, W, Cn = in_shape
  dx = addend if addend is not None else empty(in_shape, BF16, dy)
  check(L().asm_avgpool_bwd(_ptr(dy), _ptr(dx), N, H, W, Cn, k, stride, pad, dy.shape[1], dy.shape[2],
                            1 if count_valid else 0, _ptr(addend), _stream()), 'avgpool_bwd')
  return dx


def upsample2x_bwd(dy, mask=None):
  N, H, W, Cn = dy.shape
  dx = empty((N, H // 2, W // 2, Cn), BF16, dy)
  if mask is not None:
    check(L().asm_upsample2x_bwd_masked(_ptr(dy), _ptr(mask), _ptr(dx), N, H // 2, W // 2, Cn, _stream()),
          'upsample2x_bwd_masked')
  else:
    check(L().asm_upsample2x_bwd(_ptr(dy), _ptr(dx), N, H // 2, W // 2, Cn, _stream()), 'upsample2x_bwd')
  return dx


def blur_out_size(n, k, stride):
  return (n + 2 * ((k - 1) // 2) - k) // stride + 1


def blurpool_fwd(x, k, stride):
  N, H, W, Cn = x.shape
  y = empty((N, blur_out_size(H, k, stride), blur_out_size(W, k, stride), Cn), BF16, x)
  check(L().asm_blurpool_fwd(_ptr(x), _ptr(y), N, H, W, Cn, k, stride, _stream()), 'blurpool_fwd')
  return y


def blurpool_bwd(dy, in_shape, k, stride):
  N, H, W, Cn = in_shape
  dx = empty(in_shape, BF16, dy)
  check(L().asm_blurpool_bwd(_ptr(dy), _ptr(dx), N, H, W, Cn, k, stride, _stream()), 'blurpool_bwd')
  return dx


def gap_fwd(x):
  N, H, W, Cn = x.shape
  y = empty((N, 1, 1, Cn), BF16, x)
  check(L().asm_gap_fwd(_ptr(x), _ptr(y), N, H * W, Cn, _stream()), 'gap_fwd')
  return y


def gap_bwd(dy, in_shape):
  N, H, W, Cn = in_shape
  dx = empty(in_shape, BF16, dy)
  check(L().asm_gap_bwd(_ptr(dy), _ptr(dx), N, H * W, Cn, _stream()), 'gap_bwd')
  return dx


def sk_gap(f, F_):
  N, H, W, _ = f.shape
  s = empty((N, 1, 1, F_), BF16, f)
  check(L().asm_sk_gap(_ptr(f), _ptr(s), N, H * W, F_, _stream()), 'sk_gap')
  return s


def sk_select_fwd(f, att, F_):
  N, H, W, _ = f.shape
  v = empty((N, H, W, F_), BF16, f)
  check(L().asm_sk_select_fwd(_ptr(f), _ptr(att), _ptr(v), N, H * W, F_, _stream()), 'sk_select_fwd')
  return v


def sk_select_bwd_att(f, dv, att, F_):
  N, H, W, _ = f.shape
  datt = empty((N, 1, 1, 2 * F_), BF16, f)
  check(L().asm_sk_select_bwd_att(_ptr(f), _ptr(dv), _ptr(att), _ptr(datt), N, H * W, F_, _stream()),
        'sk_select_bwd_att')
  return datt


def sk_select_bwd_f(dv, att, ds, F_):
  N, H, W, _ = dv.shape
  df = empty((N, H, W, 2 * F_), BF16, dv)
  check(L().asm_sk_select_bwd_f(_ptr(dv), _ptr(att), _ptr(ds), _ptr(df), N, H * W, F_, _stream()), 'sk_select_bwd_f')
  return df


def sk_gap_bn(y, scale, shift, F_, mean=None, invstd=None):
  N, H, W, _ = y.shape
  s = empty((N, 1, 1, F_), BF16, y)
  if mean is not None:
    st = empty((N, 2, 2 * F_), F32, y)
    check(L().asm_sk_gap_bn_stats(_ptr(y), _ptr(scale), _ptr(shift), _ptr(mean), _ptr(invstd), _ptr(s), _ptr(st), N, H * W,
                                  F_, _stream()), 'sk_gap_bn_stats')
    return s, st
  check(L().asm_sk_gap_bn(_ptr(y), _ptr(scale), _ptr(shift), _ptr(s), N, H * W, F_, _stream()), 'sk_gap_bn')
  return s


def sk_select_bn_fwd(y, scale, shift, att, F_):
  N, H, W, _ = y.shape
  v = empty((N, H, W, F_), BF16, y)
  check(L().asm_sk_select_bn_fwd(_ptr(y), _ptr(scale), _ptr(shift), _ptr(att), _ptr(v), N, H * W, F_, _stream()),
        'sk_select_bn_fwd')
  return v


_SK_BLUR_ENTRIES = ('asm_sk_select_bn_blur_fwd', 'asm_sk_select_bn_bwd_att_stats_blur', 'asm_sk_bn_bwd_apply_blur')


def sk_blur_ok(H, W, k, stride) -> bool:
  return (knob('ASM_SK_BLUR', '1') != '0' and k == 3 and stride == 2 and H > 0 and W > 0 and H % 2 == 0 and W % 2 == 0
          and W <= 512 and all(getattr(L(), e, None) is not None for e in _SK_BLUR_ENTRIES))


def sk_select_bn_blur_fwd(y, scale, shift, att, F_, k, stride):
  N, H, W, _ = y.shape
  out = empty((N, H // 2, W // 2, F_), BF16, y)
  check(L().asm_sk_select_bn_blur_fwd(_ptr(y), _ptr(scale), _ptr(shift), _ptr(att), _ptr(out), N, H, W, F_, k, stride,
                                      _stream()), 'sk_select_bn_blur_fwd')
  return out


def sk_select_bn_bwd_att(y, scale, shift, dv, att, F_, mean=None, invstd=None, blur=None):
  N, H, W, _ = y.shape
  datt = empty((N, 1, 1, 2 * F_), BF16, y)
  if blur is not None:
    st = empty((N, 2, 2 * F_), F32, y)
    check(L().asm_sk_select_bn_bwd_att_stats_blur(_ptr(y), _ptr(scale), _ptr(shift), _ptr(mean), _ptr(invstd), _ptr(dv),
                                                  _ptr(att), _ptr(datt), _ptr(st), N, H, W, F_, blur[0], blur[1], _stream()),
          'sk_select_bn_bwd_att_stats_blur')
    return datt, st
  if mean is not None:
    st = empty((N, 2, 2 * F_), F32, y)
    check(L().asm_sk_select_bn_bwd_att_stats(_ptr(y), _ptr(scale), _ptr(shift), _ptr(mean), _ptr(invstd), _ptr(dv), _ptr(att),
                                             _ptr(datt), _ptr(st), N, H * W, F_, _stream()), 'sk_select_bn_bwd_att_stats')
    return datt, st
  check(L().asm_sk_select_bn_bwd_att(_ptr(y), _ptr(scale), _ptr(shift), _ptr(dv), _ptr(att), _ptr(datt), N, H * W, F_,
                                     _stream()), 'sk_select_bn_bwd_att')
  return datt


def sk_bn_bwd(dv, att, ds, y, scale, shift, gamma, mean, invstd, dgamma, dbeta, F_, grad_stats=None, mask_stats=None,
              blur=None):
  N, H, W, C2 = y.shape
  HW, M = H * W, N * H * W
  co = empty((3, C2), F32, y)
  if grad_stats is not None and mask_stats is not None:
    ev = _bn_ev(M * (2.0 * C2 + (0.5 if blur is not None else 2.0) * F_ + 2.0 * C2))
    check(L().asm_sk_bn_bwd_finalize(_ptr(grad_stats), _ptr(mask_stats), _ptr(att), _ptr(ds), N, HW, F_, _ptr(gamma),
                                     _ptr(mean), _ptr(invstd), _ptr(dgamma), _ptr(dbeta), _ptr(co[0]), _ptr(co[1]),
                                     _ptr(co[2]), _stream()), 'sk_bn_bwd_finalize')
  else:
    blocks = L().asm_sk_bn_bwd_blocks(N, HW, F_)
    if blocks <= 0:
      raise ValueError('sk_bn_bwd: bad shape')
    ev = _bn_ev(M * (2 * (2.0 * C2 + 2.0 * F_) + 2.0 * C2))
    part = empty((blocks, 2, C2), F32, y)
    check(L().asm_sk_bn_bwd_reduce(_ptr(dv), _ptr(att), _ptr(ds), _ptr(y), _ptr(scale), _ptr(shift), _ptr(mean),
                                   _ptr(invstd), N, HW, F_, _ptr(part), _stream()), 'sk_bn_bwd_reduce')
    _bn_bwd_coeffs(part, M, C2, gamma, mean, invstd, dgamma, dbeta, co)
  dy = torch.empty_like(y)
  if blur is not None:
    if grad_stats is None or mask_stats is None:
      raise ValueError('sk_bn_bwd: the pooled-gradient form needs the per-image statistics')
    check(L().asm_sk_bn_bwd_apply_blur(_ptr(dv), _ptr(att), _ptr(ds), _ptr(y), _ptr(scale), _ptr(shift), _ptr(co[0]),
                                       _ptr(co[1]), _ptr(co[2]), _ptr(dy), N, H, W, F_, blur[0], blur[1], _stream()),
          'sk_bn_bwd_apply_blur')
    if ev is not None:
      ev.record()
    return dy
  check(L().asm_sk_bn_bwd_apply(_ptr(dv), _ptr(att), _ptr(ds), _ptr(y), _ptr(scale), _ptr(shift), _ptr(co[0]),
                                _ptr(co[1]), _ptr(co[2]), _ptr(dy), N, HW, F_, _stream()), 'sk_bn_bwd_apply')
  if ev is not None:
    ev.record()
  return dy


def se_scale_fwd(x, e):
  N, H, W, Cn = x.shape
  y = torch.empty_like(x)
  check(L().asm_se_scale_fwd(_ptr(x), _ptr(e), _ptr(y), N, H * W, Cn, _stream()), 'se_scale_fwd')
  return y


def se_scale_bwd_e(x, dy, e):
  N, H, W, Cn = x.shape
  de = empty((N, 1, 1, Cn), BF16, x)
  check(L().asm_se_scale_bwd_e(_ptr(x), _ptr(dy), _ptr(e), _ptr(de), N, H * W, Cn, _stream()), 'se_scale_bwd_e')
  return de


def se_scale_bwd_x(dy, e, dsq):
  N, H, W, Cn = dy.shape
  dx = torch.empty_like(dy)
  check(L().asm_se_scale_bwd_x(_ptr(dy), _ptr(e), _ptr(dsq), _ptr(dx), N, H * W, Cn, _stream()), 'se_scale_bwd_x')
  return dx


def relu_fwd(x):
  y = torch.empty_like(x)
  check(L().asm_relu_fwd(_ptr(x), _ptr(y), x.numel(), _stream()), 'relu_fwd')
  return y


def relu_bwd(dy, y):
  dx = torch.empty_like(dy)
  check(L().asm_relu_bwd(_ptr(dy), _ptr(y), _ptr(dx), dy.numel(), _stream()), 'relu_bwd')
  return dx


def mask_apply(dy, mask):
  dx = torch.empty_like(dy)
  check(L().asm_mask_apply(_ptr(dy), _ptr(mask), _ptr(dx), dy.numel(), _stream()), 'mask_apply')
  return dx


def add_bf16(a, b, out=None):
  if out is None:
    out = torch.empty_like(a)
  check(L().asm_add_bf16(_ptr(a), _ptr(b), _ptr(out), a.numel(), _stream()), 'add_bf16')
  return out


def bias_add_f32(y, bias, M, Cn, ldy):
  check(L().asm_bias_add_f32(_ptr(y), _ptr(bias), M, Cn, ldy, _stream()), 'bias_add')


def bias_grad_bf16(dz, M, Cn, ld, dbias):
  check(L().asm_bias_grad_bf16(_ptr(dz), M, Cn, ld, _ptr(dbias), _stream()), 'bias_grad')


def cast_f32_to_bf16(x, y):
  check(L().asm_cast_f32_to_bf16(_ptr(x), _ptr(y), x.numel(), _stream()), 'cast')


def cast_bf16_to_f32(x, y):
  check(L().asm_cast_bf16_to_f32(_ptr(x), _ptr(y), x.numel(), _stream()), 'cast_bf16_to_f32')


def softmax_ce(logits, ld, targets, teacher, B, Cn, label_smoothing, kd_temp, loss_scale, ld_out, want_grad=True):
  loss_rows = empty((B,), F32, logits)
  dlogits = empty((B, 1, 1, ld_out), BF16, logits) if want_grad else None
  check(L().asm_softmax_ce(_ptr(logits), ld, _ptr(targets), _ptr(teacher), B, Cn, label_smoothing, kd_temp,
                           loss_scale, _ptr(loss_rows), _ptr(dlogits), ld_out, _stream()), 'softmax_ce')
  return loss_rows, dlogits


def onehot(labels_i32, B, Cn):
  out = empty((B, Cn), F32, labels_i32)
  check(L().asm_onehot(_ptr(labels_i32), _ptr(out), B, Cn, _stream()), 'onehot')
  return out


def softmax_rows(x, B, Cn, inv_temp):
  y = torch.empty_like(x)
  check(L().asm_softmax_rows(_ptr(x), _ptr(y), B, Cn, inv_temp, _stream()), 'softmax_rows')
  return y


def mean_f32(x):
  out = empty((1,), F32, x)
  check(L().asm_mean_f32(_ptr(x), x.numel(), _ptr(out), _stream()), 'mean')
  return out


def mixup_meansub(images, mixup_type, lam1, lam2):
  Bin, H, W, c = images.shape
  if c != 3:
    raise ValueError('images must be [B,H,W,3]')
  if images.dtype == torch.uint8:
    is_u8 = 1
  elif images.dtype == F32:
    is_u8 = 0
  else:
    raise ValueError('images must be uint8 or float32 (0..255)')
  Bout = Bin // 2 if mixup_type == 1 else Bin
  out = empty((Bout, H + 6, W + 6, 4), BF16, images)
  check(L().asm_mixup_meansub(_ptr(images), is_u8, Bin, H, W, mixup_type, _ptr(lam1), _ptr(lam2), _ptr(out),
                              _stream()), 'mixup_meansub')
  return out


def mixup_labels(y, mixup_type, lam1, lam2):
  Bin, Cn = y.shape
  Bout = Bin // 2 if mixup_type == 1 else Bin
  out = empty((Bout, Cn), F32, y)
  check(L().asm_mixup_labels(_ptr(y), Bin, Cn, mixup_type, _ptr(lam1), _ptr(lam2), _ptr(out), _stream()),
        'mixup_labels')
  return out


def sgd_momentum(w, accum, grad, w_bf16, lr, momentum, weight_decay, grad_scale):
  check(L().asm_sgd_momentum(_ptr(w), _ptr(accum), _ptr(grad), _ptr(w_bf16), w.numel(), lr, momentum, weight_decay,
                             grad_scale, _stream()), 'sgd_momentum')


def sigmoid_ce(logits, ld, targets, B, Cn, loss_scale, ld_out, want_grad=True):
  rows = empty((B, 2), F32, logits)
  out = empty((2,), F32, logits)
  dz = empty((B, 1, 1, ld_out), BF16, logits) if want_grad else None
  check(L().asm_sigmoid_ce(_ptr(logits), ld, _ptr(targets), B, Cn, loss_scale, _ptr(rows), _ptr(out), _ptr(dz), ld_out,
                           _stream()), 'sigmoid_ce')
  return out, dz


def gem_fwd(x, p=3.0):
  N, H, W, Cn = x.shape
  y = empty((N, 1, 1, Cn), BF16, x)
  ssum = empty((N, Cn), F32, x)
  check(L().asm_gem_fwd(_ptr(x), _ptr(y), _ptr(ssum), N, H * W, Cn, p, _stream()), 'gem_fwd')
  return y, ssum


def gem_bwd(x, dy, ssum, p=3.0):
  N, H, W, Cn = x.shape
  dx = torch.empty_like(x)
  check(L().asm_gem_bwd(_ptr(x), _ptr(dy), _ptr(ssum), _ptr(dx), N, H * W, Cn, p, _stream()), 'gem_bwd')
  return dx


def dropblock_mask(uniform, gamma, H, W, Cn, block_size, gamma_dev=None):
  keep = empty((H, W, Cn), F32, uniform)
  scale = empty((1,), F32, uniform)
  if gamma_dev is not None:
    check(L().asm_dropblock_mask_dev(_ptr(uniform), _ptr(gamma_dev), H, W, Cn, block_size, _ptr(keep), _ptr(scale),
                                     _stream()), 'dropblock_mask_dev')
  else:
    check(L().asm_dropblock_mask(_ptr(uniform), gamma, H, W, Cn, block_size, _ptr(keep), _ptr(scale), _stream()),
          'dropblock_mask')
  return keep, scale


def memcpy(dst: torch.Tensor, src: torch.Tensor):
  nb = src.numel() * src.element_size()
  if not (dst.is_contiguous() and src.is_contiguous()) or dst.numel() * dst.element_size() != nb:
    raise ValueError('memcpy needs two contiguous tensors of the same byte size')
  check(L().asm_memcpy_async(_ptr(dst), _ptr(src), nb, _stream()), 'memcpy_async')
  return dst


def dropblock_apply(x, keep, scale, relu=False, relu_mask_from=None):
  N = x.shape[0]
  y = torch.empty_like(x)
  check(L().asm_dropblock_apply(_ptr(x), _ptr(keep), _ptr(scale), _ptr(relu_mask_from), 1 if relu else 0, _ptr(y), N,
                                x.numel() // N, _stream()), 'dropblock_apply')
  return y


def eval_rows(logits, ld, labels_i32, B, Cn):
  pred = empty((B,), torch.int32, logits)
  vals = empty((3, B), F32, logits)
  check(L().asm_eval_rows(_ptr(logits), ld, _ptr(labels_i32), B, Cn, _ptr(pred), _ptr(vals[0]), _ptr(vals[1]),
                          _ptr(vals[2]), _stream()), 'eval_rows')
  return pred, vals[0], vals[1], vals[2]


def eval_accumulate(conf, top1, top5, state33):
  check(L().asm_eval_accumulate(_ptr(conf), _ptr(top1), _ptr(top5), conf.numel(), _ptr(state33), _stream()),
        'eval_accumulate')


def eval_groups(logits, ld, labels_i32, groups_i32, B, Cn, G, counts, want_pred=False):
  if counts.dtype != torch.int32 or counts.numel() != (G + 1) * 3:
    raise ValueError('counts must be int32 [%d, 3]' % (G + 1))
  if labels_i32.dtype != torch.int32 or groups_i32.dtype != torch.int32 or labels_i32.numel() < B or groups_i32.numel() < B:
    raise ValueError('labels and groups must be int32 [%d]' % B)
  if logits.dtype != F32 or logits.numel() < (B - 1) * ld + Cn:
    raise ValueError('logits must be float32 with %d rows of stride %d' % (B, ld))
  pred = empty((B,), torch.int32, logits) if want_pred else None
  check(L().asm_eval_groups(_ptr(logits), ld, _ptr(labels_i32), _ptr(groups_i32), B, Cn, G, _ptr(counts), _ptr(pred),
                            _stream()), 'eval_groups')
  return pred


def resize_crop_flip(src_u8, descs_dev, n, out_h, out_w, subtract_mean):
  if descs_dev.numel() != C.sizeof(_lib.ImageDesc) * n:
    raise ValueError('descriptor table must hold %d bytes' % (C.sizeof(_lib.ImageDesc) * n))
  out = torch.empty((n, out_h, out_w, 3), dtype=torch.float32, device=src_u8.device)
  if n:
    check(L().asm_resize_crop_flip(_ptr(src_u8), src_u8.numel(), _ptr(descs_dev), n, out_h, out_w,
                                   1 if subtract_mean else 0, _ptr(out), _stream()), 'resize_crop_flip')
  return out


SOURCE_BYTES, SOURCE_UNIT = 0, 1
TAIL_NONE, TAIL_MEANS, TAIL_ADD_CLAMP = 0, 1, 2


def preprocess_window(src_u8, descs_dev, n, out_h, out_w, source=SOURCE_BYTES, tail=TAIL_NONE, add=None):
  if descs_dev.numel() != C.sizeof(_lib.ImageDesc) * n:
    raise ValueError('descriptor table must hold %d bytes' % (C.sizeof(_lib.ImageDesc) * n))
  if source not in (SOURCE_BYTES, SOURCE_UNIT) or tail not in (TAIL_NONE, TAIL_MEANS, TAIL_ADD_CLAMP):
    raise ValueError('unknown source mode %r or tail mode %r' % (source, tail))
  if add is not None:
    if tail != TAIL_ADD_CLAMP:
      raise ValueError('an add table needs the add-and-clamp tail')
    if add.dtype != F32 or tuple(add.shape) != (n, 3) or not add.is_contiguous() or add.device != src_u8.device:
      raise ValueError('add must be contiguous float32 [%d, 3] on the device of the source' % n)
  out = torch.empty((n, out_h, out_w, 3), dtype=torch.float32, device=src_u8.device)
  if n:
    check(L().asm_preprocess_window(_ptr(src_u8), src_u8.numel(), _ptr(descs_dev), n, out_h, out_w, source, tail,
                                    _ptr(add) if add is not None else None, _ptr(out), _stream()), 'preprocess_window')
  return out


def autoaugment(images_f32, descs_dev, subtract_mean):
  if images_f32.dim() != 4 or images_f32.shape[3] != 3 or images_f32.dtype != F32:
    raise ValueError('images must be float32 [n, H, W, 3]')
  n, H, W = int(images_f32.shape[0]), int(images_f32.shape[1]), int(images_f32.shape[2])
  if descs_dev.numel() != C.sizeof(_lib.AugmentDesc) * n or descs_dev.dtype != torch.uint8:
    raise ValueError('descriptor table must hold %d bytes' % (C.sizeof(_lib.AugmentDesc) * n))
  out = torch.empty_like(images_f32)
  if n:
    need = C.c_int64(0)
    check(L().asm_autoaugment_workspace_bytes(n, H, W, C.byref(need)), 'autoaugment_workspace_bytes')
    ws = _workspace(need.value, images_f32)
    check(L().asm_autoaugment(_ptr(images_f32), _ptr(descs_dev), n, H, W, 1 if subtract_mean else 0, _ptr(out), _ptr(ws),
                              need.value, _stream()), 'autoaugment')
  return out


def _check_tables(text, *tables, uint8=False):
  if any((uint8 and t.dtype != torch.uint8) or t.numel() * t.element_size() != size * count for t, size, count in tables):
    raise ValueError(text)


def _rows(n, device, dtype=torch.int32, *row):
  return torch.empty((max(n, 1),) + row, dtype=dtype, device=device)[:n]


def _struct_rows(n, device, struct):
  return _rows(n, device, torch.uint8, C.sizeof(struct)).flatten()


def _jpeg_begin(name, counts, descs_dev, tables_dev, rows, dst, workspace_fn, *workspace_args):
  n = counts['n']
  _check_tables('%s: table sizes do not match %s' % (name, ', '.join('%s = %d' % kv for kv in counts.items())),
                (descs_dev, C.sizeof(_lib.JpegDesc), n), (tables_dev, C.sizeof(_lib.JpegTables), n),
                *((t, size, counts[c]) for t, size, c in rows))
  status = _rows(n, dst.device)
  if n == 0:
    return status, None
  need = C.c_int64(0)
  check(getattr(L(), 'asm_' + workspace_fn)(*workspace_args, C.byref(need)), workspace_fn)
  return status, _workspace(max(need.value, 16), dst)


def jpeg_decode(files_u8, descs_dev, tables_dev, intervals_dev, n, n_intervals, total_blocks, max_blocks, max_pixels, dst,
                stages=3):
  rows = ((intervals_dev, C.sizeof(_lib.JpegInterval), 'n_intervals'),)
  status, ws = _jpeg_begin('jpeg_decode', dict(n=n, n_intervals=n_intervals), descs_dev, tables_dev, rows, dst,
                           'jpeg_decode_workspace_bytes', total_blocks)
  if n:
    check(L().asm_jpeg_decode(_ptr(files_u8), files_u8.numel(), _ptr(descs_dev), _ptr(tables_dev), _ptr(intervals_dev), n,
                              n_intervals, total_blocks, max_blocks, max_pixels, _ptr(dst), dst.numel(), _ptr(status),
                              _ptr(ws), ws.numel(), stages, _stream()), 'jpeg_decode')
  return status, ws


def jpeg_decode_parallel(files_u8, descs_dev, tables_dev, intervals_dev, segment_first_dev, n, n_intervals, total_segments,
                         segment_bytes, total_blocks, max_blocks, max_pixels, dst, stages=3, info=False):
  rows = ((intervals_dev, C.sizeof(_lib.JpegInterval), 'n_intervals'), (segment_first_dev, 4, 'n_intervals'))
  status, ws = _jpeg_begin('jpeg_decode_parallel', dict(n=n, n_intervals=n_intervals), descs_dev, tables_dev, rows, dst,
                           'jpeg_decode_parallel_workspace_bytes', total_blocks, total_segments)
  info_dev = _rows(n, dst.device, torch.int32, 2).zero_() if info else None
  if n:
    check(L().asm_jpeg_decode_parallel(_ptr(files_u8), files_u8.numel(), _ptr(descs_dev), _ptr(tables_dev),
                                       _ptr(intervals_dev), _ptr(segment_first_dev), n, n_intervals, total_segments,
                                       segment_bytes, total_blocks, max_blocks, max_pixels, _ptr(dst), dst.numel(),
                                       _ptr(status), _ptr(info_dev), _ptr(ws), ws.numel(), stages, _stream()),
          'jpeg_decode_parallel')
  return (status, ws, info_dev) if info else (status, ws)


def jpeg_decode_progressive(files_u8, descs_dev, tables_dev, scans_dev, huff_dev, intervals_dev, n, n_scans, n_huff,
                            n_intervals, total_blocks, max_blocks, max_pixels, dst, stages=3):
  rows = ((scans_dev, C.sizeof(_lib.JpegScan), 'n_scans'), (huff_dev, C.sizeof(_lib.JpegHuff), 'n_huff'),
          (intervals_dev, C.sizeof(_lib.JpegInterval), 'n_intervals'))
  status, ws = _jpeg_begin('jpeg_decode_progressive', dict(n=n, n_scans=n_scans, n_huff=n_huff, n_intervals=n_intervals),
                           descs_dev, tables_dev, rows, dst, 'jpeg_decode_workspace_bytes', total_blocks)
  if n:
    check(L().asm_jpeg_decode_progressive(_ptr(files_u8), files_u8.numel(), _ptr(descs_dev), _ptr(tables_dev),
                                          _ptr(scans_dev), _ptr(huff_dev), _ptr(intervals_dev), n, n_scans, n_huff,
                                          n_intervals, total_blocks, max_blocks, max_pixels, _ptr(dst), dst.numel(),
                                          _ptr(status), _ptr(ws), ws.numel(), stages, _stream()), 'jpeg_decode_progressive')
  return status, ws


def crc32c_spans(buf_u8, spans_dev, n):
  if buf_u8.dim() != 1 or buf_u8.dtype != torch.uint8 or spans_dev.dtype != torch.uint8:
    raise ValueError('crc32c_spans: buffer and descriptor table are 1-D uint8 tensors')
  _check_tables('crc32c_spans: descriptor table must hold %d bytes' % (C.sizeof(_lib.SpanDesc) * max(n, 0)),
                (spans_dev, C.sizeof(_lib.SpanDesc), n))
  crc, status = _rows(n, buf_u8.device), _rows(n, buf_u8.device)
  if n:
    check(L().asm_crc32c_spans(_ptr(buf_u8), buf_u8.numel(), _ptr(spans_dev), n, _ptr(crc), _ptr(status), _stream()),
          'crc32c_spans')
  return crc, status


def example_parse(buf_u8, spans_dev, n):
  if buf_u8.dim() != 1 or buf_u8.dtype != torch.uint8 or spans_dev.dtype != torch.uint8:
    raise ValueError('example_parse: buffer and descriptor table are 1-D uint8 tensors')
  _check_tables('example_parse: descriptor table must hold %d bytes' % (C.sizeof(_lib.SpanDesc) * max(n, 0)),
                (spans_dev, C.sizeof(_lib.SpanDesc), n))
  rows = _struct_rows(n, buf_u8.device, _lib.ExampleRow)
  if n:
    check(L().asm_example_parse(_ptr(buf_u8), buf_u8.numel(), _ptr(spans_dev), n, _ptr(rows), _stream()), 'example_parse')
  return rows


def example_label_rows(buf_u8, rows_dev, n, num_classes, out=None):
  if buf_u8.dim() != 1 or buf_u8.dtype != torch.uint8:
    raise ValueError('example_label_rows: the buffer is a 1-D uint8 tensor')
  _check_tables('example_label_rows: the row table must hold %d bytes' % (C.sizeof(_lib.ExampleRow) * max(n, 0)),
                (rows_dev, C.sizeof(_lib.ExampleRow), n), uint8=True)
  if num_classes < 1:
    raise ValueError('example_label_rows: num_classes = %d' % num_classes)
  if out is None:
    out = _rows(n, buf_u8.device, torch.float32, 2 * num_classes)
  if out.dim() != 2 or out.dtype != torch.float32 or out.shape[0] != n or out.stride(1) != 1 or out.stride(0) < 2 * num_classes:
    raise ValueError('example_label_rows: out is float32 [n, >= 2 * num_classes] with unit column stride')
  status = _rows(n, buf_u8.device)
  if n:
    if not out.is_cuda and not _IS_DOUBLE:
      raise _lib.AsmError('assembled_cnn_amd ops need GPU tensors (no CPU fallback)')
    check(L().asm_example_label_rows(_ptr(buf_u8), buf_u8.numel(), _ptr(rows_dev), n, num_classes, out.data_ptr(),
                                     out.stride(0), _ptr(status), _stream()), 'example_label_rows')
  return out, status


def _segment_bytes_arg(segment_bytes) -> int:
  return 0 if segment_bytes is None else int(segment_bytes)


def jpeg_parse(buf_u8, spans_dev, n, segment_bytes=None):
  if buf_u8.dim() != 1 or buf_u8.dtype != torch.uint8 or spans_dev.dtype != torch.uint8:
    raise ValueError('jpeg_parse: buffer and descriptor table are 1-D uint8 tensors')
  _check_tables('jpeg_parse: descriptor table must hold %d bytes' % (C.sizeof(_lib.SpanDesc) * max(n, 0)),
                (spans_dev, C.sizeof(_lib.SpanDesc), n))
  heads, tables = _struct_rows(n, buf_u8.device, _lib.JpegHead), _struct_rows(n, buf_u8.device, _lib.JpegTables)
  if n:
    check(L().asm_jpeg_parse(_ptr(buf_u8), buf_u8.numel(), _ptr(spans_dev), n, _segment_bytes_arg(segment_bytes), _ptr(heads),
                             _ptr(tables), _stream()), 'jpeg_parse')
  return heads, tables


def jpeg_parse_fill(buf_u8, spans_dev, n_spans, heads_dev, tables_dev, place_dev, n_rows, n_intervals, total_segments,
                    segment_bytes=None):
  _check_tables('jpeg_parse_fill: table sizes do not match n_spans = %d' % n_spans,
                (spans_dev, C.sizeof(_lib.SpanDesc), n_spans), (heads_dev, C.sizeof(_lib.JpegHead), n_spans),
                (tables_dev, C.sizeof(_lib.JpegTables), n_spans), uint8=True)
  _check_tables('jpeg_parse_fill: table sizes do not match n_rows = %d' % n_rows,
                (place_dev, C.sizeof(_lib.JpegPlace), n_rows), uint8=True)
  if n_intervals < 0 or total_segments < 0:
    raise ValueError('jpeg_parse_fill: n_intervals = %d, total_segments = %d' % (n_intervals, total_segments))
  dev = buf_u8.device
  descs, tables = _struct_rows(n_rows, dev, _lib.JpegDesc), _struct_rows(n_rows, dev, _lib.JpegTables)
  intervals = _struct_rows(n_intervals, dev, _lib.JpegInterval)
  first = _rows(n_intervals, dev) if segment_bytes is not None else None
  status = _rows(n_rows, dev)
  if n_rows:
    check(L().asm_jpeg_parse_fill(_ptr(buf_u8), buf_u8.numel(), _ptr(spans_dev), n_spans, _ptr(heads_dev), _ptr(tables_dev),
                                  _ptr(place_dev), n_rows, n_intervals, total_segments, _segment_bytes_arg(segment_bytes),
                                  _ptr(descs), _ptr(tables), _ptr(intervals), _ptr(first), _ptr(status), _stream()),
          'jpeg_parse_fill')
  return descs, tables, intervals, first, status


SIMILARITIES = {'cosine': 0, 'euclidean': 1}
TOPK_LIST_MAX = 64
TOPK_WIDE_MAX = 1024


def _emb(x, D):
  if x.dim() != 2 or x.dtype != BF16 or x.stride(1) != 1 or (x.shape[0] > 1 and x.stride(0) != x.shape[1]):
    raise ValueError('embeddings must be a contiguous 2-D bfloat16 tensor')
  ld = x.shape[1]
  return x.shape[0], (ld if D is None else D), ld


def embed_sqnorm(x, D=None):
  n, D, ld = _emb(x, D)
  sq = empty((n,), F32, x)
  check(L().asm_embed_sqnorm(_ptr(x), n, D, ld, _ptr(sq), _stream()), 'embed_sqnorm')
  return sq


def topk_selection(K, selection='auto'):
  if selection not in ('auto', 'list', 'wide'):
    raise ValueError("selection %r (auto | list | wide)" % (selection,))
  if selection == 'auto':
    selection = 'list' if K <= TOPK_LIST_MAX else 'wide'
  cap = TOPK_LIST_MAX if selection == 'list' else TOPK_WIDE_MAX
  if K > cap:
    raise NotImplementedError('max(k_list) + 1 = %d is above the cap of %d of the %s selection' % (K, cap, selection))
  return selection


def _retrieval_topk(name, queries, index, sq_queries, sq_index, K, similarity, index_base, D):
  if similarity not in SIMILARITIES:
    raise NotImplementedError('eval_similarity %r (cosine | euclidean)' % (similarity,))
  Q, Dq, ldq = _emb(queries, D)
  N, Di, ldi = _emb(index, D)
  if Dq != Di:
    raise ValueError('queries have %d channels, the index %d' % (Dq, Di))
  need = int(getattr(L(), 'asm_%s_workspace_bytes' % name)(Q, N, K))
  ws = _workspace(need, queries)
  val = empty((Q, K), F32, queries)
  idx = empty((Q, K), torch.int32, queries)
  check(getattr(L(), 'asm_' + name)(_ptr(queries), ldq, _ptr(index), ldi, _ptr(sq_queries), _ptr(sq_index), Q, N, Dq,
                                    SIMILARITIES[similarity], K, index_base, _ptr(val), _ptr(idx), _ptr(ws), need, _stream()),
        name)
  return val, idx


def _topk_merge(name, vals, idxs):
  rows, P, K = vals.shape
  if tuple(idxs.shape) != (rows, P, K):
    raise ValueError('values and indices differ in shape')
  val = empty((rows, K), F32, vals)
  idx = empty((rows, K), torch.int32, vals)
  check(getattr(L(), 'asm_' + name)(_ptr(vals), _ptr(idxs), rows, P, K, _ptr(val), _ptr(idx), _stream()), name)
  return val, idx


def retrieval_topk_workspace_bytes(Q, N, K) -> int:
  return int(L().asm_retrieval_topk_workspace_bytes(Q, N, K))


def retrieval_topk_wide_workspace_bytes(Q, N, K) -> int:
  return int(L().asm_retrieval_topk_wide_workspace_bytes(Q, N, K))


def retrieval_topk(queries, index, sq_queries, sq_index, K, similarity='cosine', index_base=0, D=None):
  return _retrieval_topk('retrieval_topk', queries, index, sq_queries, sq_index, K, similarity, index_base, D)


def retrieval_topk_wide(queries, index, sq_queries, sq_index, K, similarity='cosine', index_base=0, D=None):
  return _retrieval_topk('retrieval_topk_wide', queries, index, sq_queries, sq_index, K, similarity, index_base, D)


def topk_merge(vals, idxs):
  return _topk_merge('topk_merge', vals, idxs)


def topk_merge_wide(vals, idxs):
  return _topk_merge('topk_merge_wide', vals, idxs)


def recall_accumulate(top_idx, query_labels, index_labels, query_base, k_list_dev, hits):
  Q, K = top_idx.shape
  check(L().asm_recall_accumulate(_ptr(top_idx), Q, K, _ptr(query_labels), _ptr(index_labels), index_labels.numel(),
                                  query_base, _ptr(k_list_dev), k_list_dev.numel(), _ptr(hits), _stream()),
        'recall_accumulate')
```

### assembled_cnn_amd/train.py

```python
from __future__ import annotations

import ctypes
import math
import os
from dataclasses import dataclass, field
from typing import Callable, List, Optional

import torch

from . import nn, ops
from .model import Model

IMAGENET_NUM_CLASSES = 1001
IMAGENET_NUM_TRAIN_IMAGES = 1281167


@dataclass
class HParams(object):
  resnet_size: int = 50
  resnet_version: int = 1
  use_resnet_d: bool = False
  use_se_block: bool = False
  use_sk_block: bool = False
  anti_alias_filter_size: int = 0
  anti_alias_type: str = ""
  bl_alpha: int = 2
  bl_beta: int = 4
  no_downsample: bool = False
  pool_type: str = 'gap'
  embedding_size: int = 0
  zero_gamma: bool = False
  bn_momentum: float = 0.997
  num_classes: int = IMAGENET_NUM_CLASSES
  label_smoothing: float = 0.0
  kd_temp: float = 0.0
  mixup_type: int = 0
  weight_decay: float = 4e-5
  use_dropblock: bool = False
  dropblock_kp: List[float] = field(default_factory=lambda: [1.0, 0.9])
  cls_loss_type: str = 'softmax'
  base_learning_rate: float = 0.01
  learning_rate_decay_type: str = 'exponential'
  lr_warmup_epochs: int = 0
  momentum: float = 0.9
  num_epochs_per_decay: float = 2.0
  learning_rate_decay_factor: float = 0.94
  end_learning_rate: float = 1e-4
  piecewise_lr_boundary_epochs: List[int] = field(default_factory=lambda: [30, 60, 80, 90])
  piecewise_lr_decay_rates: List[float] = field(default_factory=lambda: [1, 0.1, 0.01, 0.001, 1e-4])
  train_epochs: int = 90
  batch_size: int = 32
  dtype: str = 'bf16'
  loss_scale: Optional[float] = None
  num_images_train: int = IMAGENET_NUM_TRAIN_IMAGES

  def get_loss_scale(self) -> float:
    if self.loss_scale is not None:
      return float(self.loss_scale)
    return 128.0 if self.dtype == 'fp16' else 1.0

  def to_cfg(self):
    from . import lib
    aa = (lib.ASM_AA_SCONV if 'sconv' in self.anti_alias_type else 0) | (lib.ASM_AA_PROJ if 'proj' in self.anti_alias_type else 0)
    if self.pool_type not in lib.POOL_TYPES:
      raise NotImplementedError(self.pool_type)
    dt = {'bf16': lib.ASM_BF16, 'fp16': lib.ASM_F16, 'fp32': lib.ASM_F32}[self.dtype]
    return lib.ModelCfg(resnet_size=self.resnet_size, resnet_version=self.resnet_version, num_classes=self.num_classes,
                        use_se_block=int(self.use_se_block), use_sk_block=int(self.use_sk_block),
                        use_resnet_d=int(self.use_resnet_d), anti_alias_filter_size=self.anti_alias_filter_size,
                        anti_alias_type=aa, bl_alpha=self.bl_alpha, bl_beta=self.bl_beta, zero_gamma=int(self.zero_gamma),
                        no_downsample=int(self.no_downsample), pool_type=lib.POOL_TYPES[self.pool_type],
                        embedding_size=self.embedding_size, dtype=dt, mixup_type=self.mixup_type,
                        bn_momentum=self.bn_momentum, bn_eps=1e-5, loss_scale=self.get_loss_scale(),
                        label_smoothing=self.label_smoothing, kd_temp=self.kd_temp, weight_decay=self.weight_decay,
                        momentum=self.momentum)

  def make_model(self, seed=0, device='cuda') -> Model:
    if self.resnet_size < 50:
      assert not (self.use_dropblock or self.use_se_block or self.use_sk_block or self.use_resnet_d)
    return Model(self.resnet_size, None, num_classes=self.num_classes, resnet_version=self.resnet_version,
                 dtype=self.dtype, no_downsample=self.no_downsample, zero_gamma=self.zero_gamma,
                 use_se_block=self.use_se_block, use_sk_block=self.use_sk_block, bn_momentum=self.bn_momentum,
                 embedding_size=self.embedding_size, anti_alias_filter_size=self.anti_alias_filter_size,
                 anti_alias_type=self.anti_alias_type, pool_type=self.pool_type, loss_type=self.cls_loss_type,
                 bl_alpha=self.bl_alpha, bl_beta=self.bl_beta, seed=seed, device=device)


def learning_rate_with_decay(learning_rate_decay_type, batch_size, batch_denom, num_images, num_epochs_per_decay,
                             learning_rate_decay_factor, end_learning_rate, piecewise_lr_boundary_epochs,
                             piecewise_lr_decay_rates, base_lr, warmup_epochs=0, train_epochs=None
                             ) -> Callable[[int], float]:
  initial_learning_rate = base_lr * batch_size / batch_denom
  batches_per_epoch = num_images / batch_size
  decay_steps = int(batches_per_epoch * num_epochs_per_decay)
  kind = learning_rate_decay_type
  if kind not in ('exponential', 'fixed', 'polynomial', 'piecewise', 'cosine'):
    raise NotImplementedError(kind)

  def learning_rate_fn(global_step: int) -> float:
    warmup_steps = int(batches_per_epoch * warmup_epochs)
    if warmup_steps > 0 and global_step < warmup_steps:
      return initial_learning_rate * float(global_step) / float(warmup_steps)
    step = global_step - warmup_steps
    if kind == 'exponential':
      return initial_learning_rate * learning_rate_decay_factor ** (step // decay_steps)
    if kind == 'fixed':
      return base_lr
    if kind == 'polynomial':
      s = min(step, decay_steps)
      return (initial_learning_rate - end_learning_rate) * (1.0 - s / decay_steps) + end_learning_rate
    if kind == 'piecewise':
      boundaries = [int(batches_per_epoch * e) for e in piecewise_lr_boundary_epochs]
      values = [initial_learning_rate * float(d) for d in piecewise_lr_decay_rates]
      for b, v in zip(boundaries, values):
        if global_step <= b:
          return v
      return values[-1]
    total_batches = int(batches_per_epoch * train_epochs) - warmup_steps
    s = min(step, total_batches)
    return 0.5 * (1.0 + math.cos(math.pi * s / total_batches)) * initial_learning_rate
  return learning_rate_fn


def keep_prob_decay(starter_kp: float, end_kp: float, decay_steps: int) -> Callable[[int], float]:
  def keep_prob_decay_fn(global_step: int) -> float:
    s = min(global_step, decay_steps)
    return (starter_kp - end_kp) * (1.0 - s / decay_steps) + end_kp
  return keep_prob_decay_fn


def keep_prob_fn_from_hparams(p: "HParams") -> Optional[Callable[[int], float]]:
  if not p.use_dropblock:
    return None
  batches_per_epoch = p.num_images_train / p.batch_size
  return keep_prob_decay(p.dropblock_kp[0], p.dropblock_kp[1], int(p.train_epochs * batches_per_epoch))


def lr_fn_from_hparams(p: HParams) -> Callable[[int], float]:
  return learning_rate_with_decay(p.learning_rate_decay_type, p.batch_size, p.batch_size, p.num_images_train,
                                  p.num_epochs_per_decay, p.learning_rate_decay_factor, p.end_learning_rate,
                                  p.piecewise_lr_boundary_epochs, p.piecewise_lr_decay_rates, p.base_learning_rate,
                                  warmup_epochs=p.lr_warmup_epochs, train_epochs=p.train_epochs)


def _compare_tape_with_graph(g, tape):
  info = ops.tape_info(tape)
  try:
    hip = ctypes.CDLL(os.path.join(os.path.dirname(torch.__file__), 'lib', 'libamdhip64.so'),
                      mode=os.RTLD_NOLOAD | os.RTLD_NOW)
    get_nodes, get_type = hip.hipGraphGetNodes, hip.hipGraphNodeGetType
    raw = ctypes.c_void_p(g.raw_cuda_graph())
  except (AttributeError, OSError, RuntimeError) as e:
    return repr(e)
  n = ctypes.c_size_t(0)
  rc = get_nodes(raw, None, ctypes.byref(n))
  nodes = (ctypes.c_void_p * n.value)()
  rc = rc or get_nodes(raw, nodes, ctypes.byref(n))
  if rc != 0:
    return 'hipGraphGetNodes: error %d' % rc
  kernels = copies = 0
  for h in nodes[:n.value]:
    ty = ctypes.c_int(-1)
    rc = get_type(ctypes.c_void_p(h), ctypes.byref(ty))
    if rc != 0:
      return 'hipGraphNodeGetType: error %d' % rc
    kernels += ty.value == 0
    copies += ty.value in (1, 2)
  if kernels + copies != info['launches'] + info['fills']:
    raise RuntimeError('the captured step holds %d kernels and %d copies, the launch tape %d and %d: a framework kernel '
                       'ran inside the recorded region and would be missing from every replay'
                       % (kernels, copies, info['launches'], info['fills']))
  return kernels + copies


@dataclass
class Recording(object):
  graph: object = None
  tape: object = None
  static: tuple = ()
  out: tuple = None
  stream: object = None
  sig: tuple = None
  baked: tuple = None
  own: bool = False
  checked: object = None

  def fit(self, *inputs):
    for dst, src in zip(self.static, inputs):
      if (dst is None) != (src is None) or (dst is not None and (dst.shape != src.shape or dst.dtype != src.dtype)):
        raise ValueError('the captured step takes inputs of the shapes / dtypes it was captured with')

  def load(self, *inputs):
    for dst, src in zip(self.static, inputs):
      if dst is not None and dst.data_ptr() != src.data_ptr():
        dst.copy_(src, non_blocking=True)

  def replay(self, grad_sync):
    gs = grad_sync
    if self.tape is not None and gs is not None:
      try:
        for k in range(len(gs.recorded)):
          ops.tape_replay(self.tape, k)
          gs.launch_recorded(k)
        ops.tape_replay(self.tape, len(gs.recorded))
      except BaseException:
        gs.abort()
        raise
    elif self.tape is not None:
      ops.tape_replay(self.tape)
    else:
      self.graph.replay()

  def free(self):
    if self.tape is not None:
      torch.cuda.synchronize()
      ops.tape_free(self.tape)
      self.tape = None


class Trainer(object):

  AUTO_WARMUP = 3

  def __init__(self, hparams: HParams, seed: int = 0, device='cuda', grad_sync=None, world_size: int = 1,
               recorded: Optional[bool] = None):
    self.p = hparams
    self.model = hparams.make_model(seed, device)
    self.lr_fn = lr_fn_from_hparams(hparams)
    self.keep_prob_fn = keep_prob_fn_from_hparams(hparams)
    self.global_step = 0
    self.eval_state = None
    self.grad_sync = grad_sync
    self.world_size = world_size
    self.last = {}
    self._rec: Optional[Recording] = None
    dev = torch.device(device)
    self._step_stream = torch.cuda.Stream(device=dev) if dev.type == 'cuda' else None
    self.recorded = recorded
    self._auto = dev.type == 'cuda' and recorded is not False and ops.knob('ASM_STEP_TAPE', '1') != '0'
    self._auto_sig, self._auto_n = None, 0
    self._auto_error = None
    self._capturing = False
    self._db = nn.DropBlockState(dev) if (self.keep_prob_fn is not None and recorded is not False and
                                          (dev.type == 'cuda' or recorded is True)) else None

  @property
  def stream(self):
    return self._step_stream

  @property
  def step_mode(self):
    failed = ' (recording failed: %s)' % self._auto_error if self._auto_error else ''
    return 'recorded' if self._rec is not None else 'eager' + failed

  _tape = property(lambda self: self._rec.tape if self._rec is not None else None)
  _graph = property(lambda self: self._rec.graph if self._rec is not None else None)

  def _drop_stale(self, why):
    if not self._rec.own:
      raise RuntimeError(why)
    self.release_graph()

  def set_streams(self, on: bool, fresh: bool = False):
    if self._rec is not None:
      self._drop_stale('the stream setting is frozen into the captured step: release_graph() first')
    self.model.side_streams = bool(on)
    a = self.model.arena
    if a.finalized:
      if on:
        if fresh:
          a.disable_side_stream()
          old = self.model._bl_stream
          if old is not None:
            ops.stream_join(torch.cuda.current_stream(), old)
            a.extra_streams = [s_ for s_ in a.extra_streams if s_ is not old]
          self.model._bl_stream = None
        a.enable_side_stream(fresh=fresh)
      else:
        a.disable_side_stream()

  def calibrate_streams(self, step_fn, steps: int = 3, margin: float = 0.03, redraws: int = 0):
    import time

    def timed(on, fresh=False):
      self.set_streams(on, fresh=fresh)
      step_fn()
      torch.cuda.synchronize()
      t0 = time.time()
      for _ in range(steps):
        step_fn()
      torch.cuda.synchronize()
      return round(1000.0 * (time.time() - t0) / steps, 3)

    auto = self._auto
    self._auto = False
    try:
      res = {'side_streams_ms': timed(True), 'single_stream_ms': timed(False), 'redraws': 0}
      keep = res['side_streams_ms'] <= res['single_stream_ms'] * (1.0 + margin)
      while not keep and res['redraws'] < redraws:
        res['redraws'] += 1
        res['side_streams_ms'] = timed(True, fresh=True)
        keep = res['side_streams_ms'] <= res['single_stream_ms'] * (1.0 + margin)
      self.set_streams(keep)
    finally:
      self._auto = auto
      self._auto_n = 0
    if self._rec is not None:
      raise RuntimeError('calibrate_streams: a step was recorded while eager steps were being timed')
    res['chosen'] = 'side streams' if keep else 'single stream'
    return res

  def split_labels(self, labels):
    p = self.p
    C = p.num_classes
    if p.kd_temp > 0:
      if labels.dim() != 2 or labels.shape[1] != 2 * C:
        raise ValueError('kd_temp > 0 expects labels [B, 2*num_classes]')
      return labels[:, :C].contiguous(), labels[:, C:].contiguous()
    return labels.to(torch.int32).contiguous(), None

  def prepare_inputs(self, images, labels, lam1=None, lam2=None):
    hard, tlogits = self.split_labels(labels)
    return self._prepare(images, hard, tlogits, lam1, lam2)

  def _prepare(self, images, hard, tlogits, lam1, lam2):
    p = self.p
    C = p.num_classes
    Bin = images.shape[0]
    if p.kd_temp > 0:
      onehot = hard
      teacher = ops.softmax_rows(tlogits, Bin, C, 1.0 / p.kd_temp)
    else:
      onehot = ops.onehot(hard, Bin, C)
      teacher = None
    mt = p.mixup_type
    if mt not in (0, 1, 2):
      raise ValueError('mixup_type must be 0, 1 or 2')
    if mt and lam1 is None:
      raise ValueError('mixup needs the Beta(0.2, 0.2) draws (lam1 [, lam2])')
    x = ops.mixup_meansub(images if images.is_contiguous() else images.contiguous(), mt, lam1, lam2)
    if mt:
      onehot_src = onehot
      onehot = ops.mixup_labels(onehot, mt, lam1, lam2)
      if teacher is not None:
        if mt == 2:
          half = Bin // 2
          first = ops.mixup_labels(teacher, 1, lam1, None)
          src2 = ops.empty((Bin, C), torch.float32, teacher)
          ops.memcpy(src2[:half], onehot_src[:half])
          ops.memcpy(src2[half:], teacher[half:])
          second = ops.mixup_labels(src2, 2, lam1, lam2)
          teacher = ops.empty((Bin, C), torch.float32, second)
          ops.memcpy(teacher[:half], first)
          ops.memcpy(teacher[half:], second[half:])
        else:
          teacher = ops.mixup_labels(teacher, mt, lam1, lam2)
    return x, onehot, teacher

  def sample_mixup_lambdas(self, n: int, alpha: float = 0.2, rng=None):
    import numpy as np
    rng = rng if rng is not None else np.random.default_rng()
    lam = rng.beta(alpha, alpha, size=n).astype(np.float32)
    return torch.from_numpy(lam).to(self.model.device)

  def train_step(self, images, labels, lam1=None, lam2=None, lr: Optional[float] = None,
                 dropblock_uniforms=None):
    if self._rec is not None and self._baked_state() != self._rec.baked:
      self._drop_stale('grad_sync or a by-value hyper-parameter (loss scale, label smoothing, KD temperature, weight '
                       'decay, momentum, mixup type) changed after capture(): release_graph() and capture again')
    if self._rec is not None and self._rec.own and self._signature(images, labels, lam1, lam2) != self._rec.sig:
      self._drop_stale('other shapes')
    if self._rec is not None and not (dropblock_uniforms is not None and self._db is None):
      return self._replay(images, labels, lam1, lam2, lr, dropblock_uniforms)
    loss_rows, loss_scale, keep_prob = self._forward_backward(images, labels, lam1, lam2, dropblock_uniforms)
    out = self._apply(loss_rows, loss_scale, keep_prob, lr)
    if self._auto and self._rec is None and not self._capturing:
      self._auto_step(images, labels, lam1, lam2)
    return out

  @staticmethod
  def _signature(images, labels, lam1, lam2):
    return tuple((tuple(t.shape), t.dtype if t.dim() != 1 or t.dtype.is_floating_point else torch.int32, t.device)
                 if t is not None else None for t in (images, labels, lam1, lam2))

  def _auto_step(self, images, labels, lam1, lam2):
    if not images.is_cuda or (self.grad_sync is not None and not hasattr(self.grad_sync, 'launch_recorded')):
      return
    sig = self._signature(images, labels, lam1, lam2)
    if sig != self._auto_sig:
      self._auto_sig, self._auto_n = sig, 0
    self._auto_n += 1
    if self._auto_n < self.AUTO_WARMUP:
      return
    try:
      self.capture(images, labels, lam1, lam2, warmup=0)
      self._rec.own = True
    except Exception as e:
      if self.recorded is True:
        raise
      import warnings
      self._auto = False
      self._auto_error = str(e).splitlines()[0][:200] if str(e) else type(e).__name__
      warnings.warn('assembled_cnn_amd.Trainer: recording the training step failed, staying with the eager step '
                    '(14 ms of host time per step instead of 3): %r' % (e,), RuntimeWarning)

  def _forward_backward(self, images, labels, lam1, lam2, dropblock_uniforms=None):
    hard, tlogits = self.split_labels(labels)
    return self._forward_backward_split(images, hard, tlogits, lam1, lam2, dropblock_uniforms)

  def _forward_backward_split(self, images, hard, tlogits, lam1, lam2, dropblock_uniforms=None, db_prepared=False):
    p = self.p
    m = self.model
    keep_prob = self.keep_prob_fn(self.global_step) if self.keep_prob_fn else 1.0
    db = self._db
    if db is not None and not db_prepared:
      db.begin(keep_prob, dropblock_uniforms, self._db_rng())
    elif db is not None:
      db.rewind()
    x, onehot, teacher = self._prepare(images, hard, tlogits, lam1, lam2)
    B = x.shape[0]
    m(x, True, use_resnet_d=p.use_resnet_d, prepadded=True, keep_prob=keep_prob,
      dropblock_uniforms=dropblock_uniforms if db is None else None, db_static=db)
    if db is not None:
      db.end()
    loss_scale = p.get_loss_scale()
    if p.cls_loss_type == 'softmax':
      loss_rows, dlogits = ops.softmax_ce(m.logits_padded, m.ldc, onehot, teacher, B, p.num_classes,
                                          p.label_smoothing, p.kd_temp, loss_scale, m.ldc)
    elif p.cls_loss_type == 'sigmoid':
      if teacher is not None:
        raise NotImplementedError('KD on top of the sigmoid loss is not implemented on the HIP path')
      sig, dlogits = ops.sigmoid_ce(m.logits_padded, m.ldc, onehot, B, p.num_classes, loss_scale, m.ldc)
      loss_rows = sig[:1]
    else:
      raise AssertionError('cross_entropy is None')
    m.backward(dlogits)
    return loss_rows, loss_scale, keep_prob

  def _db_rng(self):
    m = self.model
    if m._db_rng is None:
      m._db_rng = torch.Generator(device=m.device)
      m._db_rng.manual_seed(m.seed + 12345)
    return m._db_rng

  def _apply(self, loss_rows, loss_scale, keep_prob, lr=None):
    p = self.p
    a = self.model.arena
    if self.grad_sync is not None:
      self.grad_sync(a.g32)
    lr = self.lr_fn(self.global_step) if lr is None else lr
    gs = 1.0 / (loss_scale * self.world_size)
    nd = a.decay_elems
    if nd:
      ops.sgd_momentum(a.w32[:nd], a.m32[:nd], a.g32[:nd], a.w16[:nd], lr, p.momentum, p.weight_decay, gs)
    if a.total_elems > nd:
      ops.sgd_momentum(a.w32[nd:], a.m32[nd:], a.g32[nd:], a.w16[nd:], lr, p.momentum, 0.0, gs)
    a.refresh_derived()
    self.global_step += 1
    self.last = {'loss_rows': loss_rows, 'lr': lr, 'keep_prob': keep_prob}
    return loss_rows

  def capture(self, images, labels, lam1=None, lam2=None, warmup: int = 2, capture_error_mode: str = 'global',
              replay: str = 'tape'):
    self._refuse_capture(images, replay)
    hard, tlogits = self.split_labels(labels)
    static = [t.clone() if t is not None else None for t in (images, hard, tlogits, lam1, lam2)]
    sig = self._signature(images, labels, lam1, lam2)
    cap = self._capture_stream(images.device)
    self._warm_up(cap, warmup, images, labels, lam1, lam2)
    g, tape, out, checked = self._record(static, cap, replay, capture_error_mode)
    self._rec = Recording(g, tape, static, out, cap, sig, self._baked_state(), checked=checked)
    return self

  def _refuse_capture(self, images, replay):
    if self._rec is not None:
      raise RuntimeError('a step is already captured: release_graph() first')
    if replay not in ('tape', 'graph'):
      raise ValueError("replay must be 'tape' or 'graph'")
    if self.keep_prob_fn is not None and self._db is None:
      raise NotImplementedError('DropBlock changes keep_prob and its draws every step: recording needs the static DropBlock '
                                'buffers (a Trainer made with recorded=False has none)')
    if self.grad_sync is not None and replay != 'tape':
      raise NotImplementedError('with a gradient exchange attached the bucket launches are host-driven: a HIP graph cannot '
                                'hold them; the launch tape is cut into segments at the bucket launches instead')
    if self.grad_sync is not None and not hasattr(self.grad_sync, 'launch_recorded'):
      raise NotImplementedError('capture needs a dp.GradSync as the gradient exchange (segmented replay)')
    if not images.is_cuda:
      raise RuntimeError('capture needs device tensors')

  def _capture_stream(self, device):
    cur = torch.cuda.current_stream(device)
    if cur != torch.cuda.default_stream(device):
      return cur
    cap = self._step_stream if self._step_stream is not None else torch.cuda.Stream(device=device)
    ops.stream_join(cap, cur)
    return cap

  def _warm_up(self, cap, warmup, *inputs):
    with torch.cuda.stream(cap):
      self._capturing = True
      try:
        for _ in range(warmup):
          self.train_step(*inputs)
      finally:
        self._capturing = False
      if self._db is not None and not self._db.known:
        raise RuntimeError('capture with DropBlock needs one eager step first (warmup >= 1): it discovers the DropBlock calls')
    torch.cuda.synchronize()

  def _record(self, static, cap, replay, capture_error_mode):
    g = torch.cuda.CUDAGraph(keep_graph=(replay == 'tape'))
    tape = None
    gs = self.grad_sync
    if gs is not None and capture_error_mode == 'global':
      capture_error_mode = 'thread_local'
    try:
      with torch.cuda.graph(g, stream=cap, capture_error_mode=capture_error_mode):
        if replay == 'tape':
          tape = ops.tape_begin()
        if gs is not None:
          gs.begin_recording()
        try:
          out = self._forward_backward_split(*static, db_prepared=True)
        finally:
          if gs is not None:
            gs.end_recording()
          if tape is not None:
            ops.tape_end()
      if gs is not None and ops.tape_info(tape)['segments'] != len(gs.recorded) + 1:
        raise RuntimeError('tape segments and recorded bucket launches disagree')
      checked = _compare_tape_with_graph(g, tape) if tape is not None else "replay='graph': there is no tape"
    except BaseException:
      if tape is not None:
        ops.tape_free(tape)
      raise
    return g, tape, out, checked

  @staticmethod
  def _check_tape_against_graph(g, tape):
    seen = _compare_tape_with_graph(g, tape)
    return seen if isinstance(seen, int) else None

  def _baked_state(self):
    p = self.p
    return (id(self.grad_sync), float(p.get_loss_scale()), float(p.label_smoothing), float(p.kd_temp), float(p.weight_decay),
            float(p.momentum), int(p.mixup_type))

  def release_graph(self):
    if self._rec is not None:
      self._rec.free()
    self._rec = None
    self._auto_n = 0
    self._auto_error = None

  def _replay(self, images, labels, lam1, lam2, lr, dropblock_uniforms=None):
    rec = self._rec
    inputs = (images,) + self.split_labels(labels) + (lam1, lam2)
    rec.fit(*inputs)
    cur = torch.cuda.current_stream()
    cap = rec.stream
    same = cap == cur
    if not same:
      ops.stream_join(cap, cur)
      torch.cuda.set_stream(cap)
    try:
      rec.load(*inputs)
      if self._db is not None:
        self._db.begin(self.keep_prob_fn(self.global_step), dropblock_uniforms, self._db_rng())
      rec.replay(self.grad_sync)
      loss_rows, loss_scale, keep_prob = rec.out
      if self.keep_prob_fn is not None:
        keep_prob = self.keep_prob_fn(self.global_step)
      out = self._apply(loss_rows, loss_scale, keep_prob, lr)
    finally:
      if not same:
        torch.cuda.set_stream(cur)
    if not same:
      ops.stream_join(cur, cap)
    return out

  def cross_entropy(self) -> torch.Tensor:
    return ops.mean_f32(self.last['loss_rows'])

  def l2_loss(self) -> torch.Tensor:
    a = self.model.arena
    return 0.5 * self.p.weight_decay * (a.w32[:a.decay_elems].double() ** 2).sum()

  def eval_logits(self, images_meansub_nhwc: torch.Tensor) -> torch.Tensor:
    return self.model(images_meansub_nhwc, False, use_resnet_d=self.p.use_resnet_d)

  def embed(self, images_meansub_nhwc: torch.Tensor) -> torch.Tensor:
    self.model(images_meansub_nhwc, False, use_resnet_d=self.p.use_resnet_d, return_embedding=True)
    return self.model.embedding_bf16

  def eval_reset(self):
    self.eval_state = torch.zeros((33,), dtype=torch.float32, device=self.model.device)

  def eval_step(self, images_meansub_nhwc: torch.Tensor, labels: torch.Tensor):
    if self.eval_state is None:
      self.eval_reset()
    m = self.model
    self.eval_logits(images_meansub_nhwc)
    B = images_meansub_nhwc.shape[0]
    pred, conf, top1, top5 = ops.eval_rows(m.logits_padded, m.ldc, labels.to(torch.int32).contiguous(), B,
                                           self.p.num_classes)
    ops.eval_accumulate(conf, top1, top5, self.eval_state)
    return pred

  def eval_result(self, reduce: bool = True) -> dict:
    st = self.eval_state.clone()
    if reduce:
      import torch.distributed as dist
      if dist.is_available() and dist.is_initialized() and dist.get_world_size() > 1:
        dist.all_reduce(st, op=dist.ReduceOp.SUM)
    st = st.double().cpu()
    n = float(st[2])
    correct, conf, cnt = st[3:13], st[13:23], st[23:33]
    eps = 1e-7
    ece = float(((cnt / cnt.sum()) * ((correct / (eps + cnt)) - (conf / (eps + cnt))).abs()).sum()) if n else 0.0
    return {'accuracy': float(st[0]) / n if n else 0.0, 'accuracy_top_5': float(st[1]) / n if n else 0.0, 'ece': ece,
            'count': n}
```

### include/asm_hip.h

```cpp
#ifndef ASM_HIP_H_
#define ASM_HIP_H_

#include <stddef.h>
#include <stdint.h>

#ifdef __cplusplus
extern "C" {
#endif

#define ASM_OK 0
#define ASM_EINVAL (-1)
#define ASM_ENOTSUP (-2)
#define ASM_EHIP (-3)

#define ASM_ABI_VERSION 11

const char* asm_last_error(void);
int asm_abi_version(void);
unsigned long long asm_launch_count(void);

int asm_stream_join(void* dst_stream, void* src_stream);
int asm_memcpy_async(void* dst, const void* src, size_t bytes, void* stream);

int asm_allreduce_bucket(void* buf, size_t count, int dtype, void* nccl_comm, void* comm_stream, void* producer_stream);
int asm_tape_begin(void);
int asm_tape_mark(void);
int asm_tape_end(void);
int asm_tape_info(int tape, int64_t info[6]);
int asm_tape_replay(int tape, int segment);
int asm_tape_free(int tape);

typedef struct asm_tuning {
  int32_t igemm_mode;
  int32_t igemm_tile;
  int32_t igemm_pfa;
  int32_t dgrad_parity;
  int32_t wgrad_halo;
  int32_t wgrad_big;
  int32_t wgrad_splits;
  int32_t bn_rows;
  int32_t igemm3;
  int32_t gemm1;
  int32_t wgrad_ring;
  int32_t igemm8;
  int32_t dense_small;
} asm_tuning;
void asm_tuning_defaults(asm_tuning* t);
int asm_set_tuning(const asm_tuning* t);
void asm_get_tuning(asm_tuning* t);

typedef struct asm_conv_desc {
  int32_t N, H, W, C;
  int32_t K, R, S;
  int32_t stride, pad;
  int32_t Ho, Wo;
  int64_t x_img_pitch;
  int32_t x_row_pitch;
  int32_t x_pix_pitch;
  int32_t ldy;
  int32_t out_f32;
} asm_conv_desc;

int asm_conv2d_fprop(const asm_conv_desc* d, const void* x, const void* w, void* y,
                     float* stats_partial, void* stream);
int asm_conv2d_stats_blocks(const asm_conv_desc* d);

int asm_conv2d_fprop_bn(const asm_conv_desc* d, const void* x, const void* w, void* y, const float* scale,
                        const float* shift, const void* residual, int relu, void* stream);

int asm_conv2d_dgrad(const asm_conv_desc* d, const void* dy, const void* wt, const void* addend, void* dx,
                     void* stream);

int asm_conv2d_dgrad_masked(const asm_conv_desc* d, const void* dy, const void* wt, const void* addend,
                            const uint8_t* addend_mask, void* dx, void* stream);
int asm_conv2d_dgrad_pooled(const asm_conv_desc* d, const void* dy, const void* wt, const void* addend,
                            const uint8_t* addend_mask, const void* pool_dy, int pool_k, int pool_stride, int pool_pad,
                            int pool_Ho, int pool_Wo, int count_valid, void* dx, void* stream);

int asm_conv2d_dgrad_bnred_blocks(const asm_conv_desc* d);
int asm_conv2d_dgrad_bnred(const asm_conv_desc* d, const void* dy, const void* wt, const void* addend,
                           const uint8_t* addend_mask, const void* bn_y, const uint8_t* bn_relu_mask, float* partial,
                           void* dx, void* stream);

#define ASM_DGRAD_MASKED 1
#define ASM_DGRAD_POOLED 2
#define ASM_DGRAD_BNRED 4
int asm_conv2d_dgrad_kernel(const asm_conv_desc* d, int variant);

size_t asm_conv2d_wgrad_workspace_bytes(const asm_conv_desc* d);
int asm_conv2d_wgrad(const asm_conv_desc* d, const void* x, const void* dy, float* dw,
                     void* workspace, size_t workspace_bytes, void* stream);

int asm_filter_transpose(const void* w_krsc, void* w_crsk, int K, int R, int S, int C, int ldk, void* stream);

int asm_filter_transpose_batched(const void* w_arena, void* wt_arena, const int32_t* table, int nlayers,
                                 long long total_elems, void* stream);
int asm_filter_transpose_tiled(const void* w_arena, void* wt_arena, const int32_t* table, int nlayers,
                               int total_tiles, void* stream);

int asm_stem_pack_filter(const float* w_krsc3, void* w_packed, int K, int ksize, void* stream);
int asm_stem_unpack_grad(const float* dw_packed, float* dw_krsc3, int K, int ksize, void* stream);
int asm_stem_pad_input(const void* x, int x_is_f32, void* xp, int N, int H, int W, void* stream);

int asm_bn_stats_blocks(int M, int C);
int asm_bn_stats(const void* x, int M, int C, float* stats_partial, void* stream);
int asm_bn_partials_compact(const float* partial, int blocks, int C, float* out, int groups, void* stream);
int asm_bn_finalize(const float* stats_partial, int blocks, int M, int C, const float* gamma,
                    const float* beta, float eps, float momentum, float* moving_mean,
                    float* moving_var, float* mean, float* invstd, float* scale, float* shift,
                    void* stream);
int asm_bn_infer_coeffs(int C, const float* gamma, const float* beta, const float* moving_mean,
                        const float* moving_var, float eps, float* scale, float* shift, void* stream);
int asm_bn_apply(const void* x, void* y, int M, int C, const float* scale, const float* shift,
                 const void* residual, int res_mode, int relu, int H, int W, uint8_t* relu_mask_out,
                 void* stream);
int asm_bn_bwd_reduce(const void* dy, const void* x, const void* yout, int relu, int M, int C,
                      const float* mean, const float* invstd, float* partial, void* stream);
int asm_bn_bwd_finalize(const float* partial, int blocks, int M, int C, const float* gamma,
                        const float* mean, const float* invstd, float* dgamma, float* dbeta,
                        float* coefA, float* coefB, float* coefC, void* stream);
int asm_bn_bwd_finalize_raw(const float* partial, int blocks, int M, int C, const float* gamma,
                            const float* mean, const float* invstd, float* dgamma, float* dbeta,
                            float* coefA, float* coefB, float* coefC, void* stream);
int asm_bn_bwd_apply(const void* dy, const void* x, const void* yout, int relu, int M, int C,
                     const float* coefA, const float* coefB, const float* coefC, void* dx,
                     void* dz_out, void* stream);
int asm_bn_bwd_apply_blocksum(const void* dy, const void* x, const uint8_t* relu_mask, int N, int H, int W, int C,
                              const float* coefA, const float* coefB, const float* coefC, void* dx, void* block_sum,
                              void* stream);

int asm_bn_apply2(const void* xa, const void* xb, void* y, int M, int C, const float* scale_a, const float* shift_a,
                  const float* scale_b, const float* shift_b, int relu, uint8_t* relu_mask_out, void* stream);
int asm_bn_bwd_reduce2(const void* dy, const void* xa, const void* xb, const uint8_t* relu_mask, int M, int C,
                       const float* mean_a, const float* invstd_a, const float* mean_b, const float* invstd_b,
                       float* partial_a, float* partial_b, void* stream);
int asm_bn_bwd_apply2(const void* dy, const void* xa, const void* xb, const uint8_t* relu_mask, int M, int C,
                      const float* coef6, void* dxa, void* dxb, void* stream);

int asm_bn_small_max_rows(void);
int asm_bn_small_fwd(const void* x, void* y, int M, int C, const float* gamma, const float* beta, float eps,
                     float momentum, float* moving_mean, float* moving_var, float* mean, float* invstd, int relu,
                     uint8_t* relu_mask_out, void* stream);
int asm_bn_small_bwd(const void* dy, const void* x, const uint8_t* relu_mask, int M, int C, const float* gamma,
                     const float* mean, const float* invstd, float* dgamma, float* dbeta, void* dx, void* stream);

int asm_dense_small(const void* p, int ldp, const void* q, int ldq, int M, int N, int K, void* out, int ldo,
                    int out_f32, const void* addend, void* stream);
int asm_dense_small_wgrad(const void* x, int ldx, const void* dy, int ldy, int M, int Cin, int Cout, float* dw, int ldw,
                          void* stream);

int asm_maxpool3x3s2_fwd(const void* x, void* y, uint8_t* argmax, int N, int H, int W, int C, void* stream);
int asm_maxpool3x3s2_bwd(const void* dy, const uint8_t* argmax, void* dx, int N, int H, int W, int C, void* stream);
int asm_avgpool_fwd(const void* x, void* y, int N, int H, int W, int C, int k, int stride, int pad,
                    int Ho, int Wo, int count_valid, void* stream);
int asm_avgpool_bwd(const void* dy, void* dx, int N, int H, int W, int C, int k, int stride, int pad,
                    int Ho, int Wo, int count_valid, const void* addend, void* stream);
int asm_upsample2x_bwd(const void* dy, void* dx, int N, int Hs, int Ws, int C, void* stream);
int asm_upsample2x_bwd_masked(const void* dy, const uint8_t* relu_mask, void* dx, int N, int Hs, int Ws, int C,
                              void* stream);
int asm_blurpool_fwd(const void* x, void* y, int N, int H, int W, int C, int k, int stride, void* stream);
int asm_blurpool_bwd(const void* dy, void* dx, int N, int H, int W, int C, int k, int stride, void* stream);
int asm_gap_fwd(const void* x, void* y, int N, int HW, int C, void* stream);
int asm_gap_bwd(const void* dy, void* dx, int N, int HW, int C, void* stream);

int asm_sk_gap(const void* f, void* s, int N, int HW, int F, void* stream);
int asm_sk_select_fwd(const void* f, const float* att, void* v, int N, int HW, int F, void* stream);
int asm_sk_select_bwd_att(const void* f, const void* dv, const float* att, void* datt, int N, int HW, int F, void* stream);
int asm_sk_select_bwd_f(const void* dv, const float* att, const void* ds, void* df, int N, int HW, int F, void* stream);
int asm_sk_gap_bn(const void* y, const float* scale, const float* shift, void* s, int N, int HW, int F, void* stream);
int asm_sk_select_bn_fwd(const void* y, const float* scale, const float* shift, const float* att, void* v, int N,
                         int HW, int F, void* stream);
int asm_sk_select_bn_bwd_att(const void* y, const float* scale, const float* shift, const void* dv, const float* att,
                             void* datt, int N, int HW, int F, void* stream);
int asm_sk_bn_bwd_blocks(int N, int HW, int F);
int asm_sk_bn_bwd_reduce(const void* dv, const float* att, const void* ds, const void* y, const float* scale,
                         const float* shift, const float* mean, const float* invstd, int N, int HW, int F,
                         float* partial, void* stream);
int asm_sk_bn_bwd_apply(const void* dv, const float* att, const void* ds, const void* y, const float* scale,
                        const float* shift, const float* coefA, const float* coefB, const float* coefC, void* dy,
                        int N, int HW, int F, void* stream);
int asm_sk_gap_bn_stats(const void* y, const float* scale, const float* shift, const float* mean, const float* invstd,
                        void* s, float* mask_stats, int N, int HW, int F, void* stream);
int asm_sk_select_bn_bwd_att_stats(const void* y, const float* scale, const float* shift, const float* mean,
                                   const float* invstd, const void* dv, const float* att, void* datt, float* grad_stats,
                                   int N, int HW, int F, void* stream);
int asm_sk_bn_bwd_finalize(const float* grad_stats, const float* mask_stats, const float* att, const void* ds, int N,
                           int HW, int F, const float* gamma, const float* mean, const float* invstd, float* dgamma,
                           float* dbeta, float* coefA, float* coefB, float* coefC, void* stream);
int asm_sk_select_bn_blur_fwd(const void* y, const float* scale, const float* shift, const float* att, void* out, int N,
                              int H, int W, int F, int k, int stride, void* stream);
int asm_sk_select_bn_bwd_att_stats_blur(const void* y, const float* scale, const float* shift, const float* mean,
                                        const float* invstd, const void* dpool, const float* att, void* datt,
                                        float* grad_stats, int N, int H, int W, int F, int k, int stride, void* stream);
int asm_sk_bn_bwd_apply_blur(const void* dpool, const float* att, const void* ds, const void* y, const float* scale,
                             const float* shift, const float* coefA, const float* coefB, const float* coefC, void* dy,
                             int N, int H, int W, int F, int k, int stride, void* stream);
int asm_se_scale_fwd(const void* x, const float* e, void* y, int N, int HW, int C, void* stream);
int asm_se_scale_bwd_e(const void* x, const void* dy, const float* e, void* de, int N, int HW, int C, void* stream);
int asm_se_scale_bwd_x(const void* dy, const float* e, const void* dsq, void* dx, int N, int HW, int C, void* stream);

int asm_relu_fwd(const void* x, void* y, size_t n, void* stream);
int asm_relu_bwd(const void* dy, const void* y, void* dx, size_t n, void* stream);
int asm_add_bf16(const void* a, const void* b, void* out, size_t n, void* stream);
int asm_mask_apply(const void* dy, const uint8_t* mask, void* dx, size_t n, void* stream);
int asm_bias_add_f32(float* y, const float* bias, int M, int C, int ldy, void* stream);
int asm_bias_grad_bf16(const void* dz, int M, int C, int ld, float* dbias, void* stream);
int asm_cast_f32_to_bf16(const float* x, void* y, size_t n, void* stream);
int asm_cast_bf16_to_f32(const void* x, float* y, size_t n, void* stream);

int asm_softmax_ce(const float* logits, int ld, const float* targets, const float* teacher, int B,
                   int C, float label_smoothing, float kd_temp, float loss_scale, float* loss_rows,
                   void* dlogits, int ld_out, void* stream);
int asm_onehot(const int32_t* labels, float* out, int B, int C, void* stream);
int asm_softmax_rows(const float* x, float* y, int B, int C, float inv_temp, void* stream);
int asm_mean_f32(const float* x, int n, float* out, void* stream);

int asm_mixup_meansub(const void* images, int is_u8, int Bin, int H, int W, int mixup_type,
                      const float* lam1, const float* lam2, void* out, void* stream);
int asm_mixup_labels(const float* y, int Bin, int C, int mixup_type, const float* lam1,
                     const float* lam2, float* out, void* stream);

int asm_sgd_momentum(float* w, float* accum, const float* grad, void* w_bf16, size_t n, float lr,
                     float momentum, float weight_decay, float grad_scale, void* stream);

int asm_sigmoid_ce(const float* logits, int ld, const float* targets, int B, int C, float loss_scale,
                   float* rows_ws, float* loss_out, void* dlogits, int ld_out, void* stream);
int asm_gem_fwd(const void* x, void* y, float* ssum, int N, int HW, int C, float p, void* stream);
int asm_gem_bwd(const void* x, const void* dy, const float* ssum, void* dx, int N, int HW, int C, float p,
                void* stream);
int asm_dropblock_mask(const float* uniform, float gamma, int H, int W, int C, int block_size, float* keep,
                       float* scale, void* stream);
int asm_dropblock_mask_dev(const float* uniform, const float* gamma_dev, int H, int W, int C, int block_size, float* keep,
                           float* scale, void* stream);
int asm_dropblock_apply(const void* x, const float* keep, const float* scale, const void* relu_mask_from, int relu,
                        void* y, int N, int HWC, void* stream);
int asm_eval_rows(const float* logits, int ld, const int32_t* labels, int B, int C, int32_t* pred, float* conf,
                  float* top1, float* top5, void* stream);
int asm_eval_accumulate(const float* conf, const float* top1, const float* top5, int B, float* state33,
                        void* stream);
int asm_eval_groups(const float* logits, int ld, const int32_t* labels, const int32_t* groups, int B, int C, int G,
                    int32_t* counts, int32_t* pred, void* stream);

int asm_embed_sqnorm(const void* x, int N, int D, int ld, float* sq, void* stream);
size_t asm_retrieval_topk_workspace_bytes(int Q, int N, int K);
int asm_retrieval_topk(const void* queries, int ldq, const void* index, int ldi, const float* sq_queries,
                       const float* sq_index, int Q, int N, int D, int similarity, int K, int index_base,
                       float* top_val, int32_t* top_idx, void* workspace, size_t workspace_bytes, void* stream);
int asm_topk_merge(const float* in_val, const int32_t* in_idx, int rows, int P, int K, float* out_val, int32_t* out_idx,
                   void* stream);
#define ASM_TOPK_WIDE_MAX 1024
size_t asm_retrieval_topk_wide_workspace_bytes(int Q, int N, int K);
int asm_retrieval_topk_wide(const void* queries, int ldq, const void* index, int ldi, const float* sq_queries,
                            const float* sq_index, int Q, int N, int D, int similarity, int K, int index_base,
                            float* top_val, int32_t* top_idx, void* workspace, size_t workspace_bytes, void* stream);
int asm_topk_merge_wide(const float* in_val, const int32_t* in_idx, int rows, int P, int K, float* out_val, int32_t* out_idx,
                        void* stream);
int asm_recall_accumulate(const int32_t* top_idx, int Q, int K, const int32_t* query_labels, const int32_t* index_labels,
                          int N, int query_base, const int32_t* k_list, int nk, int32_t* hits, void* stream);

typedef struct asm_image_desc {
  int64_t src_offset;
  int32_t Hs, Ws;
  int32_t crop_y, crop_x, crop_h, crop_w;
  int32_t resize_h, resize_w;
  int32_t out_y, out_x;
  int32_t flip;
  int32_t reserved;
} asm_image_desc;
int asm_resize_crop_flip(const uint8_t* src, int64_t src_bytes, const asm_image_desc* descs, int N,
                         int out_h, int out_w, int subtract_mean, float* out, void* stream);

#define ASM_FLIP_NONE 0
#define ASM_FLIP_BEFORE 1
#define ASM_FLIP_AFTER 2
#define ASM_SOURCE_BYTES 0
#define ASM_SOURCE_UNIT 1
#define ASM_TAIL_NONE 0
#define ASM_TAIL_MEANS 1
#define ASM_TAIL_ADD_CLAMP 2
int asm_preprocess_window(const uint8_t* src, int64_t src_bytes, const asm_image_desc* descs, int N, int out_h, int out_w,
                          int source, int tail, const float* add, float* out, void* stream);

typedef struct asm_augment_op {
  int32_t op, a, b, reserved;
  float f[6];
} asm_augment_op;
typedef struct asm_augment_desc {
  asm_augment_op slot[2];
} asm_augment_desc;
int asm_autoaugment_workspace_bytes(int N, int H, int W, int64_t* bytes);
int asm_autoaugment(const float* in, const asm_augment_desc* descs, int N, int H, int W, int subtract_mean, float* out,
                    void* workspace, int64_t workspace_bytes, void* stream);

#define ASM_JPEG_EBADCODE 1
#define ASM_JPEG_EOVERRUN 2
#define ASM_JPEG_ERESTART 4
#define ASM_JPEG_EDESC 8
typedef struct asm_jpeg_desc {
  int64_t scan_offset, scan_bytes;
  int64_t coef_offset;
  int64_t plane_offset;
  int64_t dst_offset;
  int32_t width, height;
  int32_t ncomp;
  int32_t hs, vs;
  int32_t mcus_x, mcus_y;
  int32_t restart_interval;
  int32_t first_interval, n_intervals;
  uint8_t qsel[4], dcsel[4], acsel[4];
  int32_t reserved;
} asm_jpeg_desc;
typedef struct asm_jpeg_huff {
  uint8_t bits[16];
  uint8_t vals[256];
} asm_jpeg_huff;
typedef struct asm_jpeg_tables {
  uint16_t quant[4][64];
  asm_jpeg_huff dc[2], ac[2];
} asm_jpeg_tables;
typedef struct asm_jpeg_interval {
  int32_t image;
  int32_t first_mcu, n_mcus;
  int32_t rst;
  int64_t byte_begin, byte_end;
} asm_jpeg_interval;
int asm_jpeg_decode_workspace_bytes(int64_t total_blocks, int64_t* bytes);
int asm_jpeg_decode(const uint8_t* files, int64_t files_bytes, const asm_jpeg_desc* descs, const asm_jpeg_tables* tables,
                    const asm_jpeg_interval* intervals, int N, int n_intervals, int64_t total_blocks, int max_blocks,
                    int max_pixels, uint8_t* dst, int64_t dst_bytes, int32_t* status, void* workspace,
                    int64_t workspace_bytes, int stages, void* stream);

int asm_jpeg_decode_parallel_workspace_bytes(int64_t total_blocks, int64_t total_segments, int64_t* bytes);
int asm_jpeg_decode_parallel(const uint8_t* files, int64_t files_bytes, const asm_jpeg_desc* descs,
                             const asm_jpeg_tables* tables, const asm_jpeg_interval* intervals, const int32_t* segment_first,
                             int N, int n_intervals, int64_t total_segments, int segment_bytes, int64_t total_blocks,
                             int max_blocks, int max_pixels, uint8_t* dst, int64_t dst_bytes, int32_t* status, int32_t* info,
                             void* workspace, int64_t workspace_bytes, int stages, void* stream);

typedef struct asm_jpeg_scan {
  int32_t image;
  int32_t ncomp;
  uint8_t comp[4];
  uint8_t ss, se, ah, al;
  int32_t huff[3];
  int32_t restart_interval;
  int32_t first_interval, n_intervals;
  int64_t byte_begin, byte_end;
} asm_jpeg_scan;
int asm_jpeg_decode_progressive(const uint8_t* files, int64_t files_bytes, const asm_jpeg_desc* descs,
                                const asm_jpeg_tables* tables, const asm_jpeg_scan* scans, const asm_jpeg_huff* huff,
                                const asm_jpeg_interval* intervals, int N, int n_scans, int n_huff, int n_intervals,
                                int64_t total_blocks, int max_blocks, int max_pixels, uint8_t* dst, int64_t dst_bytes,
                                int32_t* status, void* workspace, int64_t workspace_bytes, int stages, void* stream);

#define ASM_SPAN_EDESC 1
#define ASM_SPAN_EMISMATCH 2
typedef struct asm_span_desc {
  int64_t offset, length;
  uint32_t expect_masked;
  uint32_t flags;
} asm_span_desc;
int asm_crc32c_spans(const uint8_t* buf, int64_t buf_bytes, const asm_span_desc* spans, int n, uint32_t* crc,
                     int32_t* status, void* stream);

#define ASM_JPEG_PNOTJPEG 1
#define ASM_JPEG_PHEADER 2
#define ASM_JPEG_PKIND 4
#define ASM_JPEG_PNOEOI 8
#define ASM_JPEG_PSPAN 16
#define ASM_JPEG_PLIMIT 32
typedef struct asm_jpeg_head {
  int32_t cls;
  int32_t width, height, ncomp, hs, vs;
  int32_t restart_interval;
  int32_t n_intervals;
  int64_t scan_begin, scan_bytes;
  int64_t n_segments;
  uint8_t qsel[4], dcsel[4], acsel[4];
  int32_t reserved;
} asm_jpeg_head;
typedef struct asm_jpeg_place {
  int32_t span;
  int32_t first_interval;
  int32_t first_segment;
  int32_t reserved;
  int64_t coef_offset;
  int64_t dst_offset;
} asm_jpeg_place;
int asm_jpeg_parse(const uint8_t* buf, int64_t buf_bytes, const asm_span_desc* spans, int n, int segment_bytes,
                   asm_jpeg_head* heads, asm_jpeg_tables* tables, void* stream);
int asm_jpeg_parse_fill(const uint8_t* buf, int64_t buf_bytes, const asm_span_desc* spans, int n_spans,
                        const asm_jpeg_head* heads, const asm_jpeg_tables* tables, const asm_jpeg_place* place, int n_rows,
                        int n_intervals, int64_t total_segments, int segment_bytes, asm_jpeg_desc* descs,
                        asm_jpeg_tables* tables_out, asm_jpeg_interval* intervals, int32_t* segment_first, int32_t* status,
                        void* stream);

#define ASM_EXAMPLE_WINDOW 1024
#define ASM_EXAMPLE_PSPAN 1
#define ASM_EXAMPLE_PMALFORMED 2
#define ASM_EXAMPLE_PSCHEMA 4
#define ASM_EXAMPLE_PFORM 8
#define ASM_EXAMPLE_LSKIP 1
#define ASM_EXAMPLE_LRANGE 2
typedef struct asm_example_row {
  int32_t cls, label;
  int64_t enc_offset, name_offset, logit_offset;
  int32_t enc_length, name_length;
  int32_t logit_count, n_boxes;
} asm_example_row;
int asm_example_parse(const uint8_t* buf, int64_t buf_bytes, const asm_span_desc* spans, int n, asm_example_row* rows,
                      void* stream);
int asm_example_label_rows(const uint8_t* buf, int64_t buf_bytes, const asm_example_row* rows, int n, int num_classes,
                           float* out, int ld, int32_t* status, void* stream);

#define ASM_F32 0
#define ASM_BF16 1
#define ASM_F16 2
#define ASM_AA_SCONV 1
#define ASM_AA_PROJ 2
#define ASM_POOL_GAP 0
#define ASM_POOL_GEM 1
#define ASM_POOL_FLATTEN 2
typedef struct asm_model_cfg {
  int32_t resnet_size, resnet_version, num_classes;
  int32_t use_se_block, use_sk_block, use_resnet_d;
  int32_t anti_alias_filter_size, anti_alias_type;
  int32_t bl_alpha, bl_beta;
  int32_t zero_gamma, no_downsample, pool_type, embedding_size;
  int32_t dtype;
  int32_t mixup_type;
  float bn_momentum, bn_eps, loss_scale, label_smoothing, kd_temp, weight_decay, momentum;
} asm_model_cfg;

#define ASM_PLAN_CONV 0
#define ASM_PLAN_BN 1
#define ASM_PLAN_DENSE 2
#define ASM_PLAN_MAXPOOL 3
#define ASM_PLAN_AVGPOOL 4
#define ASM_PLAN_BLURPOOL 5
#define ASM_PLAN_GAP 6
#define ASM_PLAN_GEM 7
#define ASM_PLAN_FLATTEN 8
#define ASM_PLAN_SK_GAP 9
#define ASM_PLAN_SK_SELECT 10
#define ASM_PLAN_SE_SCALE 11
#define ASM_PLAN_ADD 12
#define ASM_PLAN_RELU 1
#define ASM_PLAN_RESIDUAL 2
#define ASM_PLAN_UPSAMPLED_RESIDUAL 4
#define ASM_PLAN_ZERO_GAMMA 8
#define ASM_PLAN_COUNT_VALID 16
typedef struct asm_plan_entry {
  int32_t kind;
  int32_t N, H, W, C;
  int32_t K, R, S, stride;
  int32_t Ho, Wo;
  int32_t flags;
  int32_t trainable;
  int32_t reserved;
  int64_t param_offset;
  int64_t param_elems;
  char name[112];
} asm_plan_entry;
typedef struct asm_plan_summary {
  int32_t n_entries, trainable_tensors;
  int64_t trainable_elems;
  int64_t forward_macs_per_image;
  int64_t wgrad_workspace_bytes;
} asm_plan_summary;
int asm_model_plan(const asm_model_cfg* cfg, int N, int H, int W, asm_plan_entry* entries, int capacity,
                   asm_plan_summary* summary);

#ifdef __cplusplus
}
#endif
#endif
```

Measured before the change: 10940 images/sec.

## Split SK image-pass reductions across row chunks with last-block combine

Adds a chunked form of the SK global-average-pool/BN-stats and attention-backward reduction kernels. Each image's spatial rows are split across several workgroups, and each chunk writes partial sums to a workspace. An atomic ticket elects the last-arriving block, which combines the partials and writes the final outputs. The aim is to fill more CUs when N×groups workgroups underfill the GPU at large HW. The cost is workspace traffic, an atomic per slot, and persistent counters that must be managed for graph capture.

```diff
diff --git a/assembled_cnn_amd/csrc/sk_fused.hip b/assembled_cnn_amd/csrc/sk_fused.hip
--- a/assembled_cnn_amd/csrc/sk_fused.hip
+++ b/assembled_cnn_amd/csrc/sk_fused.hip
@@ -94,16 +94,77 @@
   }
 }
 
-template <int NT, bool ST>
+struct ChunkGeom {
+  int rows, chunks;
+  float* ws;
+  unsigned ws_bytes;
+  unsigned* count;
+};
+constexpr int BUF_SC1 = 16;
+
+__device__ __forceinline__ unsigned chunk_row(const ChunkGeom& cg, int NS, int slot, int chunk, int q, int vcb, int vcl) {
+  return (unsigned)((((slot * cg.chunks + chunk) * NS + q) * vcb + vcl) * 32);
+}
+__device__ __forceinline__ void chunk_store(const ChunkGeom& cg, unsigned off, const float* o) {
+  const __amdgpu_buffer_rsrc_t rs = make_rsrc(cg.ws, cg.ws_bytes);
+  const u32x4 a = {__float_as_uint(o[0]), __float_as_uint(o[1]), __float_as_uint(o[2]), __float_as_uint(o[3])};
+  const u32x4 b = {__float_as_uint(o[4]), __float_as_uint(o[5]), __float_as_uint(o[6]), __float_as_uint(o[7])};
+  __builtin_amdgcn_raw_buffer_store_b128(a, rs, off, 0, BUF_SC1);
+  __builtin_amdgcn_raw_buffer_store_b128(b, rs, off + 16, 0, BUF_SC1);
+}
+__device__ __forceinline__ bool chunk_arrive(float (*red)[9], const ChunkGeom& cg, int slot) {
+  __asm__ volatile("s_waitcnt vmcnt(0)" ::: "memory");
+  __syncthreads();
+  if (threadIdx.x == 0) {
+    const unsigned ticket = atomicInc(cg.count + slot, (unsigned)cg.chunks - 1u);
+    red[0][8] = ticket == (unsigned)cg.chunks - 1u ? 1.f : 0.f;
+  }
+  __syncthreads();
+  return red[0][8] != 0.f;
+}
+__device__ __forceinline__ void chunk_combine(const ChunkGeom& cg, int NS, int slot, int q, int vcb, int vcl, float* t) {
+#pragma unroll
+  for (int e = 0; e < 8; ++e) t[e] = 0.f;
+  const __amdgpu_buffer_rsrc_t rs = make_rsrc(cg.ws, cg.ws_bytes);
+  const unsigned base = chunk_row(cg, NS, slot, 0, q, vcb, vcl), step = (unsigned)(NS * vcb * 32);
+  constexpr int U = 4;
+  for (int c = 0; c < cg.chunks; c += U) {
+    u32x4 a[U], b[U];
+#pragma unroll
+    for (int u = 0; u < U; ++u) {
+      const unsigned off = base + (unsigned)min(c + u, cg.chunks - 1) * step;
+      a[u] = __builtin_amdgcn_raw_buffer_load_b128(rs, off, 0, BUF_SC1);
+      b[u] = __builtin_amdgcn_raw_buffer_load_b128(rs, off + 16, 0, BUF_SC1);
+    }
+#pragma unroll
+    for (int u = 0; u < U; ++u) {
+      if (c + u >= cg.chunks) break;
+#pragma unroll
+      for (int e = 0; e < 4; ++e) { t[e] += __uint_as_float(a[u][e]); t[e + 4] += __uint_as_float(b[u][e]); }
+    }
+  }
+}
+__device__ __forceinline__ void stats_row_store(float* stats, int n, int F, int q, int vc, const float* o) {
+  float* dst = stats + (size_t)n * 4 * F + (q >> 1) * 2 * F + (q & 1) * F + vc * 8;
+  *reinterpret_cast<f32x4*>(dst) = f32x4{o[0], o[1], o[2], o[3]};
+  *reinterpret_cast<f32x4*>(dst + 4) = f32x4{o[4], o[5], o[6], o[7]};
+}
+
+template <int NT, bool ST, bool CH = false>
 __global__ __launch_bounds__(NT, NT == 256 ? 4 : 1) void sk_gap_bn_kernel(const bf16_t* __restrict__ y, const float* __restrict__ scale,
                                                        const float* __restrict__ shift, bf16_t* __restrict__ s, int HW,
                                                        int F, int vcb, const float* __restrict__ mean,
-                                                       const float* __restrict__ invstd, float* __restrict__ stats) {
+                                                       const float* __restrict__ invstd, float* __restrict__ stats,
+                                                       ChunkGeom cg) {
+  static_assert(!CH || NT == 256, "the chunked form is a 256-thread workgroup");
   __shared__ float red[NT][9];
   const int vcols = F >> 3;
   const int vcl = threadIdx.x % vcb, rl = threadIdx.x / vcb, nrl = NT / vcb;
-  const int vc = blockIdx.x * vcb + vcl;
+  const int grp = CH ? blockIdx.z : blockIdx.x;
+  const int vc = grp * vcb + vcl;
   const int n = blockIdx.y;
+  const int r_begin = CH ? blockIdx.x * cg.rows : 0;
+  const int r_end = CH ? min(HW, r_begin + cg.rows) : HW;
   float acc[8], c0[8], x0[8], c1[8], x1[8];
 #pragma unroll
   for (int e = 0; e < 8; ++e) acc[e] = c0[e] = x0[e] = c1[e] = x1[e] = 0.f;
@@ -130,8 +191,8 @@
     };
     constexpr int U = ST ? 2 : 4;
     const bf16_t* base = y + (size_t)n * HW * 2 * F + vc * 8;
-    int r = rl;
-    for (; r + (U - 1) * nrl < HW; r += U * nrl) {
+    int r = r_begin + rl;
+    for (; r + (U - 1) * nrl < r_end; r += U * nrl) {
       u32x4 v[U], w[U];
 #pragma unroll
       for (int u = 0; u < U; ++u) {
@@ -142,31 +203,43 @@
 #pragma unroll
       for (int u = 0; u < U; ++u) consume(v[u], w[u]);
     }
-    for (; r < HW; r += nrl) {
+    for (; r < r_end; r += nrl) {
       const size_t off = (size_t)r * 2 * F;
       consume(ldv(base, off), ldv(base, off + F));
     }
   }
   const bool leader = rl == 0 && vc < vcols;
+  constexpr int NS = ST ? 5 : 1;
+  const int slot = n * (int)gridDim.z + grp;
+  auto finish_s = [&](float* o) {
+    const float inv = 1.0f / (float)HW;
+#pragma unroll
+    for (int e = 0; e < 8; ++e) o[e] *= inv;
+    *reinterpret_cast<u32x4*>(s + (size_t)n * F + vc * 8) = pack8(o);
+  };
   float o[8];
   lane_sum8<NT>(red, acc, o, vcb, vcl, nrl, leader);
   if (leader) {
-    const float inv = 1.0f / (float)HW;
-#pragma unroll
-    for (int e = 0; e < 8; ++e) o[e] *= inv;
-    *reinterpret_cast<u32x4*>(s + (size_t)n * F + vc * 8) = pack8(o);
+    if (CH) chunk_store(cg, chunk_row(cg, NS, slot, blockIdx.x, 0, vcb, vcl), o);
+    else finish_s(o);
   }
   if (ST) {
-    float* st = stats + (size_t)n * 4 * F;
     const float* src[4] = {c0, c1, x0, x1};
 #pragma unroll
     for (int q = 0; q < 4; ++q) {
       lane_sum8<NT>(red, src[q], o, vcb, vcl, nrl, leader);
       if (leader) {
-        float* dst = st + (q >> 1) * 2 * F + (q & 1) * F + vc * 8;
-        *reinterpret_cast<f32x4*>(dst) = f32x4{o[0], o[1], o[2], o[3]};
-        *reinterpret_cast<f32x4*>(dst + 4) = f32x4{o[4], o[5], o[6], o[7]};
-      }
+        if (CH) chunk_store(cg, chunk_row(cg, NS, slot, blockIdx.x, q + 1, vcb, vcl), o);
+        else stats_row_store(stats, n, F, q, vc, o);
+      }
+    }
+  }
+  if (CH) {
+    if (!chunk_arrive(red, cg, slot)) return;
+    if (rl < NS && vc < vcols) {
+      chunk_combine(cg, NS, slot, rl, vcb, vcl, o);
+      if (rl == 0) finish_s(o);
+      else stats_row_store(stats, n, F, rl - 1, vc, o);
     }
   }
 }
@@ -310,19 +383,23 @@
   }
 }
 
-template <int NT, bool ST, bool PG>
+template <int NT, bool ST, bool PG, bool CH = false>
 __global__ __launch_bounds__(NT, NT == 256 ? 4 : 1) void sk_bn_bwd_att_kernel(const bf16_t* __restrict__ y, const float* __restrict__ scale,
                                                            const float* __restrict__ shift, const bf16_t* __restrict__ dv,
                                                            const float* __restrict__ att, bf16_t* __restrict__ datt,
                                                            int HW, int F, int vcb, const float* __restrict__ mean,
                                                            const float* __restrict__ invstd, float* __restrict__ stats,
-                                                           PoolGeom pg) {
+                                                           PoolGeom pg, ChunkGeom cg) {
+  static_assert(!CH || NT == 256, "the chunked form is a 256-thread workgroup");
   __shared__ float red[NT][9];
   __shared__ float cfl[PG ? 4 * 256 : 1];
   const int vcols = F >> 3;
   const int vcl = threadIdx.x % vcb, rl = threadIdx.x / vcb, nrl = NT / vcb;
-  const int vc = blockIdx.x * vcb + vcl;
+  const int grp = CH ? blockIdx.z : blockIdx.x;
+  const int vc = grp * vcb + vcl;
   const int n = blockIdx.y;
+  const int r_begin = CH ? blockIdx.x * cg.rows : 0;
+  const int r_end = CH ? min(HW, r_begin + cg.rows) : HW;
   float acc[8], g0[8], x0[8], g1[8], x1[8];
 #pragma unroll
   for (int e = 0; e < 8; ++e) acc[e] = g0[e] = x0[e] = g1[e] = x1[e] = 0.f;
@@ -375,8 +452,8 @@
     const bf16_t* gimg = PG ? dv + (size_t)n * pg.Hh * pg.Wh * F + vc * 8 : nullptr;
     auto load_dv = [&](int rq) { return PG ? dv_from_pooled(gimg, pg, F, rq) : ldv(dv, ((size_t)n * HW + rq) * F + vc * 8); };
     constexpr int U = ST ? 1 : 2;
-    int r = rl;
-    for (; r + (U - 1) * nrl < HW; r += U * nrl) {
+    int r = r_begin + rl;
+    for (; r + (U - 1) * nrl < r_end; r += U * nrl) {
       u32x4 v0[U], v1[U], vg[U];
 #pragma unroll
       for (int u = 0; u < U; ++u) {
@@ -388,36 +465,48 @@
 #pragma unroll
       for (int u = 0; u < U; ++u) consume(v0[u], v1[u], vg[u]);
     }
-    for (; r < HW; r += nrl) {
+    for (; r < r_end; r += nrl) {
       const size_t m = (size_t)n * HW + r;
       consume(ldv(y, m * 2 * F + vc * 8), ldv(y, m * 2 * F + F + vc * 8), load_dv(r));
     }
   }
   const bool leader = rl == 0 && vc < vcols;
+  constexpr int NS = ST ? 5 : 1;
+  const int slot = n * (int)gridDim.z + grp;
+  auto finish_datt = [&](const float* o) {
+    float a0[8], d0[8], d1[8];
+    gate8(att, n, F, vc * 8, a0);
+#pragma unroll
+    for (int e = 0; e < 8; ++e) {
+      d0[e] = a0[e] * (1.0f - a0[e]) * o[e];
+      d1[e] = -d0[e];
+    }
+    *reinterpret_cast<u32x4*>(datt + (size_t)n * 2 * F + vc * 8) = pack8(d0);
+    *reinterpret_cast<u32x4*>(datt + (size_t)n * 2 * F + F + vc * 8) = pack8(d1);
+  };
   float o[8];
   lane_sum8<NT>(red, acc, o, vcb, vcl, nrl, leader);
   if (leader) {
-    float a0[8], d0[8], d1[8];
-    gate8(att, n, F, vc * 8, a0);
-#pragma unroll
-    for (int e = 0; e < 8; ++e) {
-      d0[e] = a0[e] * (1.0f - a0[e]) * o[e];
-      d1[e] = -d0[e];
-    }
-    *reinterpret_cast<u32x4*>(datt + (size_t)n * 2 * F + vc * 8) = pack8(d0);
-    *reinterpret_cast<u32x4*>(datt + (size_t)n * 2 * F + F + vc * 8) = pack8(d1);
+    if (CH) chunk_store(cg, chunk_row(cg, NS, slot, blockIdx.x, 0, vcb, vcl), o);
+    else finish_datt(o);
   }
   if (ST) {
-    float* st = stats + (size_t)n * 4 * F;
     const float* src[4] = {g0, g1, x0, x1};
 #pragma unroll
     for (int q = 0; q < 4; ++q) {
       lane_sum8<NT>(red, src[q], o, vcb, vcl, nrl, leader);
       if (leader) {
-        float* dst = st + (q >> 1) * 2 * F + (q & 1) * F + vc * 8;
-        *reinterpret_cast<f32x4*>(dst) = f32x4{o[0], o[1], o[2], o[3]};
-        *reinterpret_cast<f32x4*>(dst + 4) = f32x4{o[4], o[5], o[6], o[7]};
-      }
+        if (CH) chunk_store(cg, chunk_row(cg, NS, slot, blockIdx.x, q + 1, vcb, vcl), o);
+        else stats_row_store(stats, n, F, q, vc, o);
+      }
+    }
+  }
+  if (CH) {
+    if (!chunk_arrive(red, cg, slot)) return;
+    if (rl < NS && vc < vcols) {
+      chunk_combine(cg, NS, slot, rl, vcb, vcl, o);
+      if (rl == 0) finish_datt(o);
+      else stats_row_store(stats, n, F, rl - 1, vc, o);
     }
   }
 }
@@ -608,6 +697,38 @@
   return vcols < vcb ? vcols : vcb;
 }
 
+struct ImagePassPlan {
+  int vcb, groups, chunks, rows;
+  size_t ws_bytes;
+};
+constexpr int SK_IMAGE_PASS_SUMS = 5;
+int g_sk_chunks = 0;
+
+int image_pass_rule(long long wgs, int HW) {
+  const int cus = asm_num_cus();
+  if (HW < 512 || wgs == cus || wgs >= 4LL * cus) return 1;
+  return (int)(4LL * cus / wgs);
+}
+
+ImagePassPlan image_pass_plan(int N, int HW, int F) {
+  ImagePassPlan p;
+  p.vcb = image_pass_vcb(N, F);
+  p.groups = cdiv(F / 8, p.vcb);
+  const int nrl = 256 / p.vcb;
+  const int forced = g_sk_chunks;
+  const long long wgs = (long long)N * p.groups;
+  int want = forced > 0 ? forced : image_pass_rule(wgs, HW);
+  if (want < 1) want = 1;
+  if (want > HW) want = HW;
+  int rows = cdiv(HW, want);
+  rows = cdiv(rows, nrl) * nrl;
+  if (forced <= 0 && rows < 4 * nrl) rows = 4 * nrl;
+  p.rows = rows;
+  p.chunks = cdiv(HW, rows);
+  p.ws_bytes = p.chunks > 1 ? (size_t)N * p.groups * p.chunks * SK_IMAGE_PASS_SUMS * p.vcb * 8 * sizeof(float) : 0;
+  return p;
+}
+
 SkBnGeom make_geom(int N, int HW, int F) {
   SkBnGeom g;
   g.HW = HW;
@@ -630,21 +751,82 @@
   ASM_REQUIRE(N > 0 && HW > 0 && F > 0 && F % 8 == 0 && 2 * F / 8 <= 256, name ": bad shape (N=%d HW=%d F=%d)", N, HW, F); \
   ASM_REQUIRE((size_t)N * HW * (2 * F / 8) < 0x7fffffffull, name ": tensor too large for 32-bit indexing")
 
+struct ImagePassScratch {
+  void* workspace;
+  size_t workspace_bytes;
+  uint32_t* counters;
+};
+#define SK_SCRATCH_OK(name, sc, plan)                                                                                  \
+  ASM_REQUIRE((sc)->counters, name ": null counters");                                                                 \
+  ASM_REQUIRE((sc)->workspace_bytes >= (plan).ws_bytes && ((sc)->workspace || (plan).ws_bytes == 0),                   \
+              name ": workspace of %zu bytes, the plan needs %zu", (sc)->workspace_bytes, (plan).ws_bytes);            \
+  ASM_REQUIRE(((uintptr_t)(sc)->workspace & 15) == 0, name ": workspace not 16-byte aligned");                          \
+  ASM_REQUIRE((plan).groups <= 65535 && N <= 65535 && (plan).ws_bytes <= 0x7fffffffull, name ": grid or workspace too large")
+
 static int sk_gap_bn_impl(const void* y, const float* scale, const float* shift, void* s, int N, int HW, int F,
-                          const float* mean, const float* invstd, float* stats, void* stream) {
+                          const float* mean, const float* invstd, float* stats, void* stream,
+                          const ImagePassScratch* scratch = nullptr) {
   SKF_OK("sk_gap_bn");
   ASM_REQUIRE(y && scale && shift && s, "sk_gap_bn: null pointer");
+  hipStream_t st = (hipStream_t)stream;
+  if (scratch) {
+    const ImagePassPlan p = image_pass_plan(N, HW, F);
+    SK_SCRATCH_OK("sk_gap_bn_ws", scratch, p);
+    if (p.chunks > 1) {
+      const ChunkGeom cg = {p.rows, p.chunks, (float*)scratch->workspace, (unsigned)p.ws_bytes, scratch->counters};
+      const dim3 grid(p.chunks, N, p.groups);
+      if (stats)
+        ASM_LAUNCH((sk_gap_bn_kernel<256, true, true>), grid, dim3(256), 0, st, (const bf16_t*)y, scale, shift, (bf16_t*)s, HW,
+                   F, p.vcb, mean, invstd, stats, cg);
+      else
+        ASM_LAUNCH((sk_gap_bn_kernel<256, false, true>), grid, dim3(256), 0, st, (const bf16_t*)y, scale, shift, (bf16_t*)s,
+                   HW, F, p.vcb, mean, invstd, stats, cg);
+      ASM_CHECK_LAUNCH("sk_gap_bn_ws");
+      return ASM_OK;
+    }
+  }
   const int vcb = image_pass_vcb(N, F);
   const dim3 grid(cdiv(F / 8, vcb), N);
-  hipStream_t st = (hipStream_t)stream;
 #define LAUNCH_GAP(NT, ST)                                                                                       \
   ASM_LAUNCH((sk_gap_bn_kernel<NT, ST>), grid, dim3(NT), 0, st, (const bf16_t*)y, scale, shift, (bf16_t*)s, HW, F, \
-                     vcb, mean, invstd, stats)
+                     vcb, mean, invstd, stats, ChunkGeom{})
   if (stats) { if (HW >= 512) LAUNCH_GAP(1024, true); else LAUNCH_GAP(256, true); }
   else { if (HW >= 512) LAUNCH_GAP(1024, false); else LAUNCH_GAP(256, false); }
 #undef LAUNCH_GAP
   ASM_CHECK_LAUNCH("sk_gap_bn");
   return ASM_OK;
+}
+
+extern "C" int asm_sk_image_pass_chunks(int n) {
+  ASM_REQUIRE(n >= 0, "sk_image_pass_chunks: %d < 0", n);
+  g_sk_chunks = n;
+  return ASM_OK;
+}
+
+extern "C" int asm_sk_image_pass_plan(int N, int HW, int F, int32_t plan[4]) {
+  SKF_OK("sk_image_pass_plan");
+  ASM_REQUIRE(plan, "sk_image_pass_plan: null pointer");
+  const ImagePassPlan p = image_pass_plan(N, HW, F);
+  ASM_REQUIRE(p.ws_bytes <= 0x7fffffffull, "sk_image_pass_plan: workspace above 2 GiB");
+  plan[0] = p.chunks;
+  plan[1] = p.rows;
+  plan[2] = p.groups;
+  plan[3] = (int32_t)p.ws_bytes;
+  return ASM_OK;
+}
+
+extern "C" int asm_sk_gap_bn_ws(const void* y, const float* scale, const float* shift, void* s, int N, int HW, int F,
+                                void* workspace, size_t workspace_bytes, uint32_t* counters, void* stream) {
+  const ImagePassScratch sc = {workspace, workspace_bytes, counters};
+  return sk_gap_bn_impl(y, scale, shift, s, N, HW, F, nullptr, nullptr, nullptr, stream, &sc);
+}
+
+extern "C" int asm_sk_gap_bn_stats_ws(const void* y, const float* scale, const float* shift, const float* mean,
+                                      const float* invstd, void* s, float* mask_stats, int N, int HW, int F, void* workspace,
+                                      size_t workspace_bytes, uint32_t* counters, void* stream) {
+  ASM_REQUIRE(mean && invstd && mask_stats, "sk_gap_bn_stats_ws: null pointer");
+  const ImagePassScratch sc = {workspace, workspace_bytes, counters};
+  return sk_gap_bn_impl(y, scale, shift, s, N, HW, F, mean, invstd, mask_stats, stream, &sc);
 }
 
 extern "C" int asm_sk_gap_bn(const void* y, const float* scale, const float* shift, void* s, int N, int HW, int F,
@@ -710,16 +892,33 @@
 
 static int sk_att_impl(const void* y, const float* scale, const float* shift, const void* dv, const float* att, void* datt,
                        int N, int HW, int F, const float* mean, const float* invstd, float* stats, void* stream,
-                       const PoolGeom* pooled = nullptr) {
+                       const PoolGeom* pooled = nullptr, const ImagePassScratch* scratch = nullptr) {
   SKF_OK("sk_select_bn_bwd_att");
   ASM_REQUIRE(y && scale && shift && dv && att && datt, "sk_select_bn_bwd_att: null pointer");
+  hipStream_t st = (hipStream_t)stream;
+  const PoolGeom pg = pooled ? *pooled : PoolGeom{};
+  if (scratch) {
+    const ImagePassPlan p = image_pass_plan(N, HW, F);
+    SK_SCRATCH_OK("sk_select_bn_bwd_att_ws", scratch, p);
+    if (p.chunks > 1) {
+      const ChunkGeom cg = {p.rows, p.chunks, (float*)scratch->workspace, (unsigned)p.ws_bytes, scratch->counters};
+      const dim3 cgrid(p.chunks, N, p.groups);
+#define LAUNCH_ATT_CH(ST, PG)                                                                                            \
+  ASM_LAUNCH((sk_bn_bwd_att_kernel<256, ST, PG, true>), cgrid, dim3(256), 0, st, (const bf16_t*)y, scale, shift,           \
+                     (const bf16_t*)dv, att, (bf16_t*)datt, HW, F, p.vcb, mean, invstd, stats, pg, cg)
+      if (pooled) LAUNCH_ATT_CH(true, true);
+      else if (stats) LAUNCH_ATT_CH(true, false);
+      else LAUNCH_ATT_CH(false, false);
+#undef LAUNCH_ATT_CH
+      ASM_CHECK_LAUNCH("sk_select_bn_bwd_att_ws");
+      return ASM_OK;
+    }
+  }
   const int vcb = image_pass_vcb(N, F);
   const dim3 grid(cdiv(F / 8, vcb), N);
-  hipStream_t st = (hipStream_t)stream;
-  const PoolGeom pg = pooled ? *pooled : PoolGeom{};
 #define LAUNCH_ATT(NT, ST, PG)                                                                                          \
   ASM_LAUNCH((sk_bn_bwd_att_kernel<NT, ST, PG>), grid, dim3(NT), 0, st, (const bf16_t*)y, scale, shift, (const bf16_t*)dv, \
-                     att, (bf16_t*)datt, HW, F, vcb, mean, invstd, stats, pg)
+                     att, (bf16_t*)datt, HW, F, vcb, mean, invstd, stats, pg, ChunkGeom{})
   if (pooled) { if (HW >= 512) LAUNCH_ATT(1024, true, true); else LAUNCH_ATT(256, true, true); }
   else if (stats) { if (HW >= 512) LAUNCH_ATT(1024, true, false); else LAUNCH_ATT(256, true, false); }
   else { if (HW >= 512) LAUNCH_ATT(1024, false, false); else LAUNCH_ATT(256, false, false); }
@@ -748,6 +947,34 @@
   ASM_REQUIRE(mean && invstd && grad_stats, "sk_select_bn_bwd_att_stats_blur: null pointer");
   const PoolGeom pg = make_pool_geom(H, W);
   return sk_att_impl(y, scale, shift, dpool, att, datt, N, HW, F, mean, invstd, grad_stats, stream, &pg);
+}
+
+extern "C" int asm_sk_select_bn_bwd_att_ws(const void* y, const float* scale, const float* shift, const void* dv,
+                                           const float* att, void* datt, int N, int HW, int F, void* workspace,
+                                           size_t workspace_bytes, uint32_t* counters, void* stream) {
+  const ImagePassScratch sc = {workspace, workspace_bytes, counters};
+  return sk_att_impl(y, scale, shift, dv, att, datt, N, HW, F, nullptr, nullptr, nullptr, stream, nullptr, &sc);
+}
+
+extern "C" int asm_sk_select_bn_bwd_att_stats_ws(const void* y, const float* scale, const float* shift, const float* mean,
+                                                 const float* invstd, const void* dv, const float* att, void* datt,
+                                                 float* grad_stats, int N, int HW, int F, void* workspace,
+                                                 size_t workspace_bytes, uint32_t* counters, void* stream) {
+  ASM_REQUIRE(mean && invstd && grad_stats, "sk_select_bn_bwd_att_stats_ws: null pointer");
+  const ImagePassScratch sc = {workspace, workspace_bytes, counters};
+  return sk_att_impl(y, scale, shift, dv, att, datt, N, HW, F, mean, invstd, grad_stats, stream, nullptr, &sc);
+}
+
+extern "C" int asm_sk_select_bn_bwd_att_stats_blur_ws(const void* y, const float* scale, const float* shift,
+                                                      const float* mean, const float* invstd, const void* dpool,
+                                                      const float* att, void* datt, float* grad_stats, int N, int H, int W,
+                                                      int F, int k, int stride, void* workspace, size_t workspace_bytes,
+                                                      uint32_t* counters, void* stream) {
+  SKB_OK("sk_select_bn_bwd_att_stats_blur_ws");
+  ASM_REQUIRE(mean && invstd && grad_stats, "sk_select_bn_bwd_att_stats_blur_ws: null pointer");
+  const PoolGeom pg = make_pool_geom(H, W);
+  const ImagePassScratch sc = {workspace, workspace_bytes, counters};
+  return sk_att_impl(y, scale, shift, dpool, att, datt, N, HW, F, mean, invstd, grad_stats, stream, &pg, &sc);
 }
 
 extern "C" int asm_sk_bn_bwd_finalize(const float* grad_stats, const float* mask_stats, const float* att, const void* ds,
diff --git a/assembled_cnn_amd/lib.py b/assembled_cnn_amd/lib.py
--- a/assembled_cnn_amd/lib.py
+++ b/assembled_cnn_amd/lib.py
@@ -150,6 +150,8 @@
   check_code = lib.asm_set_tuning(C.byref(t))
   if check_code != ASM_OK:
     raise ValueError('asm_set_tuning rejected the ASM_* overrides: %s' % (lib.asm_last_error() or b'').decode())
+  if lib.asm_sk_image_pass_chunks(int(os.environ.get('ASM_SK_CHUNKS') or 0)) != ASM_OK:
+    raise ValueError('ASM_SK_CHUNKS rejected: %s' % (lib.asm_last_error() or b'').decode())
   return t
 
 
@@ -234,6 +236,14 @@
     'asm_sk_select_bn_bwd_att_stats': (_I, [_P, _P, _P, _P, _P, _P, _P, _P, _P, _I, _I, _I, _P]),
     'asm_sk_select_bn_bwd_att_stats_blur': (_I, [_P, _P, _P, _P, _P, _P, _P, _P, _P, _I, _I, _I, _I, _I, _I, _P]),
     'asm_sk_bn_bwd_finalize': (_I, [_P, _P, _P, _P, _I, _I, _I, _P, _P, _P, _P, _P, _P, _P, _P, _P]),
+    'asm_sk_image_pass_chunks': (_I, [_I]),
+    'asm_sk_image_pass_plan': (_I, [_I, _I, _I, C.POINTER(C.c_int32 * 4)]),
+    'asm_sk_gap_bn_ws': (_I, [_P, _P, _P, _P, _I, _I, _I, _P, _Z, _P, _P]),
+    'asm_sk_gap_bn_stats_ws': (_I, [_P, _P, _P, _P, _P, _P, _P, _I, _I, _I, _P, _Z, _P, _P]),
+    'asm_sk_select_bn_bwd_att_ws': (_I, [_P, _P, _P, _P, _P, _P, _I, _I, _I, _P, _Z, _P, _P]),
+    'asm_sk_select_bn_bwd_att_stats_ws': (_I, [_P, _P, _P, _P, _P, _P, _P, _P, _P, _I, _I, _I, _P, _Z, _P, _P]),
+    'asm_sk_select_bn_bwd_att_stats_blur_ws': (_I, [_P, _P, _P, _P, _P, _P, _P, _P, _P, _I, _I, _I, _I, _I, _I, _P, _Z, _P,
+                                                   _P]),
     'asm_se_scale_fwd': (_I, [_P, _P, _P, _I, _I, _I, _P]),
     'asm_se_scale_bwd_e': (_I, [_P, _P, _P, _P, _I, _I, _I, _P]),
     'asm_se_scale_bwd_x': (_I, [_P, _P, _P, _P, _I, _I, _I, _P]),
diff --git a/assembled_cnn_amd/ops.py b/assembled_cnn_amd/ops.py
--- a/assembled_cnn_amd/ops.py
+++ b/assembled_cnn_amd/ops.py
@@ -17,6 +17,7 @@
   global _L, _IS_DOUBLE
   _L = obj
   _IS_DOUBLE = is_double
+  _SK_PLANS.clear()
 
 
 def L():
@@ -42,6 +43,7 @@
 
 def refresh_tuning():
   _KNOBS.clear()
+  _SK_PLANS.clear()
   if _IS_DOUBLE:
     return None
   return _lib.apply_env_tuning(L())
@@ -600,15 +602,64 @@
   return df
 
 
+_SK_CHUNK_ENTRIES = ('asm_sk_image_pass_plan', 'asm_sk_gap_bn_ws', 'asm_sk_gap_bn_stats_ws', 'asm_sk_select_bn_bwd_att_ws',
+                     'asm_sk_select_bn_bwd_att_stats_ws', 'asm_sk_select_bn_bwd_att_stats_blur_ws')
+_SK_PLANS = {}
+_SK_COUNTERS = {}
+_SK_COUNTER_WORDS = 4096
+
+
+def _sk_image_scratch(y, N, HW, F_, stream):
+  plan = _SK_PLANS.get((N, HW, F_))
+  if plan is None:
+    lib = L()
+    if any(getattr(lib, e, None) is None for e in _SK_CHUNK_ENTRIES):
+      return None
+    p = (C.c_int32 * 4)()
+    check(lib.asm_sk_image_pass_plan(N, HW, F_, C.byref(p)), 'sk_image_pass_plan')
+    plan = _SK_PLANS[(N, HW, F_)] = (int(p[0]), int(p[3]), N * int(p[2]))
+  chunks, nbytes, words = plan
+  if chunks <= 1:
+    return None
+  key = (y.device.index, stream)
+  cnt = _SK_COUNTERS.get(key)
+  if cnt is None or cnt.numel() < words:
+    if y.is_cuda and torch.cuda.is_current_stream_capturing():
+      return None
+    cnt = _SK_COUNTERS[key] = torch.zeros(max(words, _SK_COUNTER_WORDS), dtype=torch.int32, device=y.device)
+  ws = empty((nbytes,), torch.uint8, y)
+  return ws, nbytes, _ptr(cnt)
+
+
+def sk_counters_for(stream: "torch.cuda.Stream"):
+  if _IS_DOUBLE:
+    return
+  dev = stream.device.index
+  words = max([_SK_COUNTER_WORDS] + [c.numel() for (d, _), c in _SK_COUNTERS.items() if d == dev])
+  key = (dev, stream.cuda_stream)
+  if key not in _SK_COUNTERS:
+    _SK_COUNTERS[key] = torch.zeros(words, dtype=torch.int32, device=stream.device)
+
+
 def sk_gap_bn(y, scale, shift, F_, mean=None, invstd=None):
   N, H, W, _ = y.shape
   s = empty((N, 1, 1, F_), BF16, y)
+  stream = _stream()
+  sc = _sk_image_scratch(y, N, H * W, F_, stream)
   if mean is not None:
     st = empty((N, 2, 2 * F_), F32, y)
+    if sc is not None:
+      check(L().asm_sk_gap_bn_stats_ws(_ptr(y), _ptr(scale), _ptr(shift), _ptr(mean), _ptr(invstd), _ptr(s), _ptr(st), N, H * W,
+                                       F_, _ptr(sc[0]), sc[1], sc[2], stream), 'sk_gap_bn_stats_ws')
+      return s, st
     check(L().asm_sk_gap_bn_stats(_ptr(y), _ptr(scale), _ptr(shift), _ptr(mean), _ptr(invstd), _ptr(s), _ptr(st), N, H * W,
-                                  F_, _stream()), 'sk_gap_bn_stats')
+                                  F_, stream), 'sk_gap_bn_stats')
     return s, st
-  check(L().asm_sk_gap_bn(_ptr(y), _ptr(scale), _ptr(shift), _ptr(s), N, H * W, F_, _stream()), 'sk_gap_bn')
+  if sc is not None:
+    check(L().asm_sk_gap_bn_ws(_ptr(y), _ptr(scale), _ptr(shift), _ptr(s), N, H * W, F_, _ptr(sc[0]), sc[1], sc[2], stream),
+          'sk_gap_bn_ws')
+    return s
+  check(L().asm_sk_gap_bn(_ptr(y), _ptr(scale), _ptr(shift), _ptr(s), N, H * W, F_, stream), 'sk_gap_bn')
   return s
 
 
@@ -639,19 +690,24 @@
 def sk_select_bn_bwd_att(y, scale, shift, dv, att, F_, mean=None, invstd=None, blur=None):
   N, H, W, _ = y.shape
   datt = empty((N, 1, 1, 2 * F_), BF16, y)
+  stream = _stream()
+  sc = _sk_image_scratch(y, N, H * W, F_, stream)
+  tail = (stream,) if sc is None else (_ptr(sc[0]), sc[1], sc[2], stream)
+  sfx = '' if sc is None else '_ws'
   if blur is not None:
     st = empty((N, 2, 2 * F_), F32, y)
-    check(L().asm_sk_select_bn_bwd_att_stats_blur(_ptr(y), _ptr(scale), _ptr(shift), _ptr(mean), _ptr(invstd), _ptr(dv),
-                                                  _ptr(att), _ptr(datt), _ptr(st), N, H, W, F_, blur[0], blur[1], _stream()),
-          'sk_select_bn_bwd_att_stats_blur')
+    name = 'asm_sk_select_bn_bwd_att_stats_blur' + sfx
+    check(getattr(L(), name)(_ptr(y), _ptr(scale), _ptr(shift), _ptr(mean), _ptr(invstd), _ptr(dv), _ptr(att), _ptr(datt),
+                             _ptr(st), N, H, W, F_, blur[0], blur[1], *tail), name[4:])
     return datt, st
   if mean is not None:
     st = empty((N, 2, 2 * F_), F32, y)
-    check(L().asm_sk_select_bn_bwd_att_stats(_ptr(y), _ptr(scale), _ptr(shift), _ptr(mean), _ptr(invstd), _ptr(dv), _ptr(att),
-                                             _ptr(datt), _ptr(st), N, H * W, F_, _stream()), 'sk_select_bn_bwd_att_stats')
+    name = 'asm_sk_select_bn_bwd_att_stats' + sfx
+    check(getattr(L(), name)(_ptr(y), _ptr(scale), _ptr(shift), _ptr(mean), _ptr(invstd), _ptr(dv), _ptr(att), _ptr(datt),
+                             _ptr(st), N, H * W, F_, *tail), name[4:])
     return datt, st
-  check(L().asm_sk_select_bn_bwd_att(_ptr(y), _ptr(scale), _ptr(shift), _ptr(dv), _ptr(att), _ptr(datt), N, H * W, F_,
-                                     _stream()), 'sk_select_bn_bwd_att')
+  name = 'asm_sk_select_bn_bwd_att' + sfx
+  check(getattr(L(), name)(_ptr(y), _ptr(scale), _ptr(shift), _ptr(dv), _ptr(att), _ptr(datt), N, H * W, F_, *tail), name[4:])
   return datt
 
 
diff --git a/assembled_cnn_amd/train.py b/assembled_cnn_amd/train.py
--- a/assembled_cnn_amd/train.py
+++ b/assembled_cnn_amd/train.py
@@ -507,6 +507,7 @@
         self._capturing = False
       if self._db is not None and not self._db.known:
         raise RuntimeError('capture with DropBlock needs one eager step first (warmup >= 1): it discovers the DropBlock calls')
+    ops.sk_counters_for(cap)
     torch.cuda.synchronize()
 
   def _record(self, static, cap, replay, capture_error_mode):
diff --git a/include/asm_hip.h b/include/asm_hip.h
--- a/include/asm_hip.h
+++ b/include/asm_hip.h
@@ -195,6 +195,24 @@
 int asm_sk_bn_bwd_apply_blur(const void* dpool, const float* att, const void* ds, const void* y, const float* scale,
                              const float* shift, const float* coefA, const float* coefB, const float* coefC, void* dy,
                              int N, int H, int W, int F, int k, int stride, void* stream);
+int asm_sk_image_pass_chunks(int n);
+int asm_sk_image_pass_plan(int N, int HW, int F, int32_t plan[4]);
+int asm_sk_gap_bn_ws(const void* y, const float* scale, const float* shift, void* s, int N, int HW, int F, void* workspace,
+                     size_t workspace_bytes, uint32_t* counters, void* stream);
+int asm_sk_gap_bn_stats_ws(const void* y, const float* scale, const float* shift, const float* mean, const float* invstd,
+                           void* s, float* mask_stats, int N, int HW, int F, void* workspace, size_t workspace_bytes,
+                           uint32_t* counters, void* stream);
+int asm_sk_select_bn_bwd_att_ws(const void* y, const float* scale, const float* shift, const void* dv, const float* att,
+                                void* datt, int N, int HW, int F, void* workspace, size_t workspace_bytes,
+                                uint32_t* counters, void* stream);
+int asm_sk_select_bn_bwd_att_stats_ws(const void* y, const float* scale, const float* shift, const float* mean,
+                                      const float* invstd, const void* dv, const float* att, void* datt, float* grad_stats,
+                                      int N, int HW, int F, void* workspace, size_t workspace_bytes, uint32_t* counters,
+                                      void* stream);
+int asm_sk_select_bn_bwd_att_stats_blur_ws(const void* y, const float* scale, const float* shift, const float* mean,
+                                           const float* invstd, const void* dpool, const float* att, void* datt,
+                                           float* grad_stats, int N, int H, int W, int F, int k, int stride,
+                                           void* workspace, size_t workspace_bytes, uint32_t* counters, void* stream);
 int asm_se_scale_fwd(const void* x, const float* e, void* y, int N, int HW, int C, void* stream);
 int asm_se_scale_bwd_e(const void* x, const void* dy, const float* e, void* de, int N, int HW, int C, void* stream);
 int asm_se_scale_bwd_x(const void* dy, const float* e, const void* dsq, void* dx, int N, int HW, int C, void* stream);
```

Result: no change. 10980 images/sec, median of 6 (+0.3%).
